# awslabs/crowd-coachable-recommendations

Hardware: AMD Instinct MI355X
Metric: queries/sec, exhaustive inner-product top-100 retrieval (NQ-shaped 2,681,468 x 768 bf16 corpus) (higher is better)
Workload: dtype bf16

## Files before the change

crowd-coachable-recommendations_amd/ccrec_amd/_lib.py:

```python
import ctypes
import os

_HERE = os.path.dirname(os.path.abspath(__file__))
LIB_PATH = os.path.join(os.path.dirname(_HERE), "lib", "libccr_hip.so")

CCR_OK = 0
CCR_ERR_INVALID, CCR_ERR_HIP, CCR_ERR_WORKSPACE, CCR_ERR_BLOCK_ID = -1, -2, -3, -4
DTYPE_F32, DTYPE_F16, DTYPE_BF16 = 0, 1, 2
SEARCH_DEFAULT, SEARCH_FORCE_DENSE, SEARCH_FORCE_FUSED, SEARCH_ASYNC = 0, 1, 2, 4
SCORES_CANONICAL, SCORES_MFMA = 0, 1

EXPORTS = [
    "ccr_last_error", "ccr_version", "ccr_pack_bf16", "ccr_pack_bf16_ex", "ccr_meanpool_pack_bf16", "ccr_meanpool_pack_bf16_ex", "ccr_index_create",
    "ccr_index_create_with_norms", "ccr_index_destroy",
    "ccr_index_rows", "ccr_index_dim", "ccr_search_workspace_bytes", "ccr_search", "ccr_search_last_stats",
    "ccr_merge_topk", "ccr_merge_topk_strided", "ccr_apply_block", "ccr_inbatch_ce_workspace_bytes", "ccr_inbatch_ce_fwd", "ccr_inbatch_ce_bwd", "ccr_inbatch_ce_bwd_dev", "ccr_rank_metrics",
    "ccr_search_finish", "ccr_scores", "ccr_search_blocked_workspace_bytes", "ccr_search_blocked",
    "ccr_search_sparse_prior_workspace_bytes", "ccr_search_sparse_prior", "ccr_colsum_bf16", "ccr_meanpool_bwd", "ccr_bm25_index_create", "ccr_bm25_index_destroy", "ccr_bm25_search_workspace_bytes",
    "ccr_bm25_search", "ccr_pack_bf16_padded", "ccr_shard_message_bytes", "ccr_search_shard", "ccr_shard_message_fill", "ccr_merge_shard_messages",
    "ccr_attention_bf16", "ccr_add_layernorm", "ccr_meanpool_pack_bf16_packed", "ccr_embed_layernorm", "ccr_gelu_bf16",
    "ccr_attention_half", "ccr_add_layernorm_half", "ccr_embed_layernorm_half", "ccr_gelu_half", "ccr_merge_short_lists",
    "ccr_bm25_search_workspace_bytes_k", "ccr_bm25_search_last_stats", "ccr_bm25_index_set_idf", "ccr_inbatch_pack3_bf16", "ccr_inbatch_ce_fwd_f32",
    "ccr_search_stream_wait_main_pass",
]

SHARD_HEADER_BYTES = 32
SHARD_MAGIC = 0x4D524343


class ShardHeader(ctypes.Structure):
    _fields_ = [("magic", ctypes.c_uint32), ("n_flagged", ctypes.c_uint32), ("k_valid", ctypes.c_uint32),
                ("n_covered", ctypes.c_uint32), ("row_offset", ctypes.c_int64), ("n_rows", ctypes.c_int64)]


class SearchStats(ctypes.Structure):
    _fields_ = [("path", ctypes.c_int32), ("n_fallback", ctypes.c_int32), ("sample_tiles", ctypes.c_int32),
                ("ranges", ctypes.c_int32), ("cap", ctypes.c_int32), ("sublists", ctypes.c_int32),
                ("n_candidates", ctypes.c_int64), ("ms_sample", ctypes.c_float), ("ms_threshold", ctypes.c_float),
                ("ms_main", ctypes.c_float), ("ms_select", ctypes.c_float), ("ms_fallback", ctypes.c_float),
                ("ms_total", ctypes.c_float), ("n_retried", ctypes.c_int32), ("n_dense", ctypes.c_int32),
                ("main_launches", ctypes.c_int32), ("opt_rank", ctypes.c_int32), ("main_tile_queries", ctypes.c_int32),
                ("reserved0", ctypes.c_int32)]


class CcrError(RuntimeError):
    pass


_lib = None


def load():
    global _lib
    if _lib is not None:
        return _lib
    if not os.path.isfile(LIB_PATH):
        raise CcrError(f"{LIB_PATH} not built: run `python -c 'import __graft_entry__ as g; g.build()'` "
                       f"(or make -C crowd-coachable-recommendations_amd/csrc)")
    lib = ctypes.CDLL(LIB_PATH)
    vp, i32, i64, f32, sz = ctypes.c_void_p, ctypes.c_int, ctypes.c_int64, ctypes.c_float, ctypes.c_size_t
    lib.ccr_last_error.restype = ctypes.c_char_p
    lib.ccr_last_error.argtypes = []
    lib.ccr_version.restype = i32
    lib.ccr_pack_bf16.argtypes = [vp, vp, vp, i64, i32, i32, vp]
    lib.ccr_pack_bf16_ex.argtypes = [vp, vp, vp, vp, i64, i32, i32, vp]
    lib.ccr_index_create_with_norms.argtypes = [vp, i64, i32, i64, vp, vp, ctypes.POINTER(vp)]
    lib.ccr_meanpool_pack_bf16.argtypes = [vp, i32, vp, vp, vp, i32, i32, i32, i32, vp]
    lib.ccr_meanpool_pack_bf16_ex.argtypes = [vp, i32, vp, vp, vp, vp, vp, i32, i32, i32, i32, vp]
    lib.ccr_index_create.argtypes = [vp, i64, i32, i64, vp, ctypes.POINTER(vp)]
    lib.ccr_index_destroy.argtypes = [vp]
    lib.ccr_index_rows.argtypes = [vp]
    lib.ccr_index_rows.restype = i64
    lib.ccr_index_dim.argtypes = [vp]
    lib.ccr_search_workspace_bytes.argtypes = [vp, i32, i32]
    lib.ccr_search_workspace_bytes.restype = sz
    lib.ccr_search.argtypes = [vp, vp, i32, i32, vp, vp, vp, sz, i32, vp]
    lib.ccr_search_last_stats.argtypes = [vp, ctypes.POINTER(SearchStats)]
    lib.ccr_merge_topk.argtypes = [vp, vp, i32, i32, i32, vp, vp, vp]
    lib.ccr_merge_topk_strided.argtypes = [vp, vp, i64, i64, i32, i32, i32, vp, vp, vp]
    lib.ccr_apply_block.argtypes = [vp, vp, i32, i32, vp, vp, i64, vp, vp, i32, vp]
    lib.ccr_inbatch_ce_workspace_bytes.argtypes = [i32, i32]
    lib.ccr_inbatch_ce_workspace_bytes.restype = sz
    lib.ccr_inbatch_ce_fwd.argtypes = [vp, vp, vp, i32, i32, f32, vp, vp, vp, sz, vp]
    lib.ccr_inbatch_ce_bwd.argtypes = [vp, vp, vp, vp, i32, i32, f32, f32, vp, vp, vp, vp, sz, vp]
    lib.ccr_inbatch_ce_bwd_dev.argtypes = [vp, vp, vp, vp, i32, i32, f32, vp, vp, vp, vp, vp, sz, vp]
    lib.ccr_inbatch_pack3_bf16.argtypes = [vp, vp, vp, i32, i32, vp, vp]
    lib.ccr_inbatch_ce_fwd_f32.argtypes = [vp, vp, vp, i32, i32, f32, vp, vp, vp, vp, sz, vp]
    lib.ccr_rank_metrics.argtypes = [vp, i32, i32, vp, vp, vp, i32, vp, vp, vp]
    lib.ccr_search_finish.argtypes = [vp]
    lib.ccr_search_stream_wait_main_pass.argtypes = [vp, vp]
    lib.ccr_scores.argtypes = [vp, vp, i32, i32, vp, vp]
    lib.ccr_search_blocked_workspace_bytes.argtypes = [vp, i32, i32, vp]
    lib.ccr_search_blocked_workspace_bytes.restype = sz
    lib.ccr_search_blocked.argtypes = [vp, vp, i32, i32, vp, vp, vp, vp, vp, sz, i32, vp]
    lib.ccr_search_sparse_prior_workspace_bytes.argtypes = [vp, i32, i32, vp]
    lib.ccr_search_sparse_prior_workspace_bytes.restype = sz
    lib.ccr_search_sparse_prior.argtypes = [vp, vp, i32, i32, vp, vp, vp, vp, vp, vp, sz, i32, vp]
    lib.ccr_colsum_bf16.argtypes = [vp, i64, i32, vp, vp]
    lib.ccr_meanpool_bwd.argtypes = [vp, vp, vp, i32, i32, i32, i32, vp]
    lib.ccr_bm25_index_create.argtypes = [vp, vp, vp, vp, i64, i64, ctypes.c_double, ctypes.POINTER(vp)]
    lib.ccr_bm25_index_destroy.argtypes = [vp]
    lib.ccr_bm25_search_workspace_bytes.argtypes = [vp, i32, i32]
    lib.ccr_bm25_search_workspace_bytes.restype = sz
    lib.ccr_bm25_search_workspace_bytes_k.argtypes = [vp, i32, i32, i32]
    lib.ccr_bm25_search_workspace_bytes_k.restype = sz
    lib.ccr_bm25_search_last_stats.argtypes = [vp, vp]
    lib.ccr_bm25_index_set_idf.argtypes = [vp, vp, vp, vp]
    lib.ccr_bm25_search.argtypes = [vp, vp, vp, vp, i32, i32, vp, vp, vp, sz, vp]
    lib.ccr_pack_bf16_padded.argtypes = [vp, i64, i32, vp, i32, vp, vp, i32, vp]
    lib.ccr_attention_bf16.argtypes = [vp, vp, vp, vp, i32, i32, i32, i32, ctypes.c_float, vp]
    lib.ccr_add_layernorm.argtypes = [vp, vp, vp, vp, ctypes.c_float, vp, vp, i64, i32, vp]
    lib.ccr_embed_layernorm.argtypes = [vp, i64, vp, i64, vp, i64, vp, vp, vp, vp, vp, ctypes.c_float, vp, vp, i64, i32, vp]
    lib.ccr_gelu_bf16.argtypes = [vp, vp, i64, vp]
    lib.ccr_attention_half.argtypes = [vp, vp, vp, vp, i32, i32, i32, i32, ctypes.c_float, i32, vp]
    lib.ccr_add_layernorm_half.argtypes = [vp, vp, vp, vp, ctypes.c_float, vp, vp, i64, i32, i32, vp]
    lib.ccr_embed_layernorm_half.argtypes = [vp, i64, vp, i64, vp, i64, vp, vp, vp, vp, vp, ctypes.c_float, vp, vp, i64, i32, i32, vp]
    lib.ccr_gelu_half.argtypes = [vp, vp, i64, i32, vp]
    lib.ccr_meanpool_pack_bf16_packed.argtypes = [vp, i32, vp, vp, vp, vp, vp, vp, i32, i32, i32, vp]
    lib.ccr_shard_message_bytes.argtypes = [i32, i32]
    lib.ccr_shard_message_bytes.restype = sz
    lib.ccr_search_shard.argtypes = [vp, vp, i32, i32, vp, vp, sz, i32, vp]
    lib.ccr_shard_message_fill.argtypes = [vp, i32, i32, i32, vp, vp, i64, i64, vp]
    lib.ccr_merge_shard_messages.argtypes = [vp, i64, i32, i32, i32, vp, vp, vp]
    lib.ccr_merge_short_lists.argtypes = [vp, i64, i32, i32, i32, i32, vp, vp, vp, vp, vp]
    for name in EXPORTS:
        fn = getattr(lib, name)
        if fn.restype is ctypes.c_int and name not in ("ccr_version", "ccr_index_dim"):
            fn.restype = i32
    _lib = lib
    return lib


def check(rc, what=""):
    if rc != CCR_OK:
        msg = load().ccr_last_error().decode("utf-8", "replace")
        if rc == CCR_ERR_BLOCK_ID:
            raise AssertionError("block id not found")
        raise CcrError(f"{what} failed ({rc}): {msg}")
```

crowd-coachable-recommendations_amd/csrc/ccr_api.hip:

```cpp
#include <stdarg.h>
#include <stdlib.h>
#include <string.h>

#include <math.h>

#include <algorithm>
#include <mutex>
#include <vector>

#include "ccr_index.h"
#include "ccr_narrow.h"
#include "ccr_topk_device.h"

namespace ccr {

static thread_local char g_err[512] = "";
void set_error(const char *fmt, ...) {
    va_list ap;
    va_start(ap, fmt);
    vsnprintf(g_err, sizeof(g_err), fmt, ap);
    va_end(ap);
}

static int env_int(const char *name, int dflt) {
    const char *e = getenv(name);
    return e ? atoi(e) : dflt;
}

Knobs read_knobs() {
    Knobs kn;
    kn.qgroups = env_int("CCR_QGROUPS", 0);
    kn.progressive = env_int("CCR_PROGRESSIVE", 1);
    kn.max_phases = env_int("CCR_PHASES", 3);
    kn.mfma16 = env_int("CCR_MFMA16", -1);
    kn.sample_div = env_int("CCR_SAMPLE_DIV", 0);
    kn.max_lists = env_int("CCR_MAX_LISTS", 0);
    kn.ranges = env_int("CCR_RANGES", 0);
    kn.optimistic = env_int("CCR_OPTIMISTIC", -1);
    kn.opt_rank = env_int("CCR_OPT_RANK", 0);
    kn.narrow = env_int("CCR_NARROW", -1);
    kn.wide = env_int("CCR_WIDE", -1);
    kn.narrow_grid = env_int("CCR_NARROW_GRID", 0);
    kn.narrow_groups = env_int("CCR_NARROW_GROUPS", NARROW_MAX_GROUPS);
    return kn;
}

static int pick_qgroups(int qblocks, int dim, const Knobs &kn, int tile_q = TILE_Q) {
    {
        const int v = kn.qgroups;
        if ((v == 1 || v == 2 || v == 4 || v == 8) && qblocks % v == 0) return v;
    }
    const size_t block_bytes = (size_t)tile_q * dim * 2;
    int best = 1;
    for (int gq = 1; gq <= NUM_XCD; gq *= 2) {
        if (qblocks % gq) continue;
        best = gq;
        if ((size_t)(qblocks / gq) * block_bytes <= (size_t)3 << 20) break;
    }
    return best;
}

static inline int64_t round_up(int64_t v, int64_t m) { return (v + m - 1) / m * m; }

static int best_sample_ranges(int64_t n_vt, int qblocks, int qgroups, int grid) {
    const int nrc = NUM_XCD / qgroups, qb_per = qblocks / qgroups, per_x = std::max(1, grid / NUM_XCD);
    int best_r = NUM_XCD;
    double best = 1e300;
    const int64_t r_max = round_up(std::min<int64_t>(n_vt, 1024), NUM_XCD);
    std::vector<double> load((size_t)per_x);
    for (int64_t R = NUM_XCD; R <= r_max; R += NUM_XCD) {
        double worst = 0.0;
        for (int rc = 0; rc < nrc; ++rc) {
            std::fill(load.begin(), load.end(), 0.0);
            const int64_t items = R / nrc * qb_per;
            for (int64_t item = 0; item < items; ++item) {
                const int64_t r = rc + nrc * (item / qb_per);
                const int64_t ntile = (n_vt - r + R - 1) / R;
                if (ntile > 0) load[(size_t)(item % per_x)] += (double)ntile + 0.15;
            }
            worst = std::max(worst, *std::max_element(load.begin(), load.end()));
        }
        if (worst < best - 1e-9) {
            best = worst;
            best_r = (int)R;
        }
    }
    return best_r;
}

constexpr size_t DENSE_SCRATCH_TARGET = (size_t)1 << 30;

struct MainPassChoice {
    int64_t sample, ranges;
    int item_a, item_b;
    int opt_rank;
};

static int optimistic_rank(int k, int64_t sample, int64_t tiles, const Knobs &kn) {
    if (kn.opt_rank > 0) return kn.opt_rank;
    const double need = (double)k * (double)sample / (double)tiles;
    int r = 40;
    for (; r < 1 << 20; ++r) {
        const double a = 1.0 / (9.0 * r), t = 1.0 - a - 5.2 * sqrt(a);
        if (t > 0.0 && (double)r * t * t * t >= need) break;
    }
    return r;
}

static MainPassChoice choose_main_pass(const Plan &p, int k, int64_t sample_a, int64_t sample_b, int64_t sample_c, const Knobs &kn,
                                       bool single_only = false) {
    const int nrc = NUM_XCD / p.main_qgroups, qb_per = p.main_qblocks / p.main_qgroups, per_x = p.grid / NUM_XCD;
    const double tile_cost = p.tile_q == WIDE_Q ? 1.37 : 1.0;
    int64_t max_lists = p.rescore_cap > 512 ? 2048 : 1024;
    if ((max_lists / p.sublists) * p.main_qblocks < p.grid) max_lists = 2048;
    if (kn.max_lists >= 64 && kn.max_lists < max_lists) max_lists = kn.max_lists;
    const int64_t r_hi = std::min<int64_t>(max_lists / p.sublists, round_up(std::max<int64_t>(1, p.tiles / 8), NUM_XCD));
    const int64_t target = std::min<int64_t>(r_hi, round_up(std::max<int64_t>(NUM_XCD, (int64_t)p.grid * 6 / p.main_qblocks), NUM_XCD));
    const bool prog_on = kn.progressive != 0 && !single_only;
    const int max_phases = kn.max_phases;
    const double qscale = (double)p.nq_pad / 3584.0;
    const double select_per_range = 0.1 * qscale, hit_w = 0.014 * qscale, phase_w = 3.0;
    auto sample_cost = [&](int64_t smp) -> double {
        return (double)((smp * p.qblocks + p.grid - 1) / p.grid) + 0.015 * (double)smp * std::max(1.0, qscale);
    };

    MainPassChoice best_choice = {sample_a, target, 0, 0, 0};
    double best = 1e300;
    for (int pass = 0; pass < 3; ++pass) {
        const int64_t smp = pass == 0 ? sample_a : (pass == 1 ? sample_b : sample_c);
        if ((pass >= 1 && smp == sample_a) || (pass == 2 && smp == sample_b)) continue;
        const double fs = (double)smp / (double)p.tiles;
        const double smp_cost = sample_cost(smp);
        auto survivors = [&](double fa, double fb) -> double {
            if (fa <= 0.0) return (double)k / fs;
            if (fb <= 0.0) return (double)k * (fa / fs + (1.0 - fa) / fa);
            return (double)k * (fa / fs + fb / fa + (1.0 - fa - fb) / (fa + fb));
        };
        const int64_t r_lo = std::max<int64_t>(NUM_XCD, target / 2 / NUM_XCD * NUM_XCD);
        for (int64_t R = r_lo; R <= std::min(r_hi, target * 2); R += NUM_XCD) {
            if (kn.ranges > 0 && R != std::min<int64_t>(r_hi, std::max<int64_t>(r_lo, round_up(kn.ranges, NUM_XCD)))) continue;
            const int64_t items = R / nrc * qb_per;
            const double item_cost = ((double)((p.tiles + R - 1) / R) + 0.15) * tile_cost;
            auto rounds = [&](int64_t n) { return (double)((n + per_x - 1) / per_x); };
            const double common = smp_cost + select_per_range * (double)R + 1e-3 * std::abs((double)(R - target));
            const double single = rounds(items) * item_cost + hit_w * survivors(0.0, 0.0) + common;
            if (single < best && kn.optimistic != 1) {
                best = single;
                best_choice = {smp, R, 0, 0, 0};
            }
            if (kn.optimistic != 0 && smp * GROUPS_PER_TILE >= 4 * 40) {
                const int rank = optimistic_rank(k, smp, p.tiles, kn);
                if ((int64_t)rank * 4 <= smp * GROUPS_PER_TILE) {
                    const double pass = std::max((double)rank / fs, (double)k);
                    const double opt = rounds(items) * item_cost + hit_w * pass + common - (kn.optimistic == 1 ? 1e9 : 0.0);
                    if (opt < best) {
                        best = opt;
                        best_choice = {smp, R, 0, 0, rank};
                    }
                }
            }
            if (!(prog_on && items > per_x && (double)p.tiles / (double)R >= 8.0)) continue;
            const double fa = (double)per_x / (double)items;
            const double two = (1.0 + rounds(items - per_x)) * item_cost + phase_w + hit_w * survivors(fa, 0.0) + common;
            if (two < best) {
                best = two;
                best_choice = {smp, R, per_x, 0, 0};
            }
            if (max_phases < 3) continue;
            for (int m = 1; m <= 3; ++m) {
                const int64_t ib = (int64_t)per_x * (1 + m);
                if (ib >= items) break;
                const double fb = (double)m * per_x / (double)items;
                const double three = (1.0 + m + rounds(items - ib)) * item_cost + 2.0 * phase_w + hit_w * survivors(fa, fb) + common;
                if (three < best) {
                    best = three;
                    best_choice = {smp, R, per_x, (int)ib, 0};
                }
            }
        }
    }
    return best_choice;
}

static CandLayout one_segment(int cap) {
    CandLayout L;
    memset(&L, 0, sizeof(L));
    L.nseg = 1;
    L.seg_end[0] = L.seg_end[1] = L.seg_end[2] = INT32_MAX;
    L.cap[0] = L.cap[1] = L.cap[2] = cap;
    return L;
}

static Plan make_plan_for(int64_t n_rows, int dim, int n_q, int k, int flags, int num_cu, const Knobs &kn, int mfma16) {
    Plan p;
    memset(&p, 0, sizeof(p));
    p.nq_pad = (int)round_up(n_q, TILE_Q);
    p.qblocks = p.nq_pad / TILE_Q;
    p.tile_q = TILE_Q;
    p.main_qblocks = p.qblocks;
    p.main_qgroups = 1;
    p.tiles = (n_rows + TILE_DOCS - 1) / TILE_DOCS;
    p.full_tiles = n_rows / TILE_DOCS;
    p.grid = std::max(NUM_XCD, num_cu / NUM_XCD * NUM_XCD);
    {
        p.mfma16 = mfma16;
        p.sublists = p.mfma16 ? 8 : 4;
    }
    p.rescore_cap = std::min(8192, std::max(256, 2 * pow2_ceil(k)));

    const int64_t min_sample = (2 * (int64_t)k + GROUPS_PER_TILE - 1) / GROUPS_PER_TILE;
    int64_t sample_div = 32;
    bool sample_div_forced = false;
    {
        if (kn.sample_div >= 4 && kn.sample_div <= 256) {
            sample_div = kn.sample_div;
            sample_div_forced = true;
        }
    }
    auto sample_for = [&](int64_t div) { return std::max<int64_t>({(p.tiles + div - 1) / div, min_sample, 4}); };
    int64_t sample = sample_for(sample_div);
    bool fused = (dim % 8 == 0) && dim >= 8 && (sample * 4 <= p.full_tiles) && k <= MAX_K;
    if ((flags & CCR_SEARCH_FORCE_FUSED) && (dim % 8 == 0) && p.full_tiles >= 1) {
        if (!fused) sample = std::min<int64_t>(std::max<int64_t>(sample, 1), p.full_tiles);
        fused = sample * GROUPS_PER_TILE >= k;
    }
    if (flags & CCR_SEARCH_FORCE_DENSE) fused = false;
    p.fused = fused ? 1 : 0;

    if (p.fused) {
        p.qgroups = pick_qgroups(p.qblocks, dim, kn);
        const bool pinned = sample_div_forced || (flags & CCR_SEARCH_FORCE_FUSED);
        const int64_t sample_alt = pinned ? sample : sample_for(2 * sample_div);
        int64_t sample_big = pinned ? sample : sample_for(sample_div / 2);
        if (sample_big * 4 > p.full_tiles) sample_big = sample;
        int nqt = n_q <= 16 ? 1 : (n_q <= 32 ? 2 : 4);
        int ngroups = n_q <= NARROW_MAX_Q ? 1 : 2;
        if (n_q > NARROW_MAX_Q && n_q <= 96 && kn.narrow_groups >= 2 && dim % TILE_K == 0 && narrow_lds_bytes(6, dim) <= (size_t)160 * 1024)
            nqt = 6, ngroups = 1;
        const bool narrow = kn.narrow != 0 && n_q <= NARROW_MAX_Q * std::min(std::max(kn.narrow_groups, 1), NARROW_MAX_GROUPS) && dim % TILE_K == 0 &&
                            narrow_lds_bytes(nqt, dim) <= (size_t)160 * 1024 && (ngroups == 1 || num_cu >= 16);
        p.narrow = narrow ? nqt : 0;
        p.narrow_groups = narrow ? ngroups : 1;
        p.tile_q = TILE_Q;
        p.main_qblocks = p.qblocks;
        if (!narrow && p.mfma16 && dim % 32 == 0 && kn.wide != 0) {
            const int wb = (n_q + WIDE_Q - 1) / WIDE_Q;
            const double per_xcd = (double)(wb / pick_qgroups(wb, dim, kn, WIDE_Q)) * WIDE_Q * dim * 2.0;
            const double per_flop = per_xcd <= 3.2 * 1048576.0 ? 0.95 : (per_xcd <= 5.5 * 1048576.0 ? 0.97 : 1.04);
            if (kn.wide == 1 || (double)wb * WIDE_Q * per_flop < (double)p.qblocks * TILE_Q) {
                p.tile_q = WIDE_Q;
                p.main_qblocks = wb;
                p.nq_pad = (int)round_up(std::max<int64_t>(n_q, (int64_t)wb * WIDE_Q), TILE_Q);
                p.qblocks = p.nq_pad / TILE_Q;
                p.qgroups = pick_qgroups(p.qblocks, dim, kn);
            }
        }
        p.main_qgroups = pick_qgroups(p.main_qblocks, dim, kn, p.tile_q);
        const MainPassChoice choice = choose_main_pass(p, k, sample, sample_alt, sample_big, kn, narrow);
        sample = choice.sample;
        const int64_t R = choice.ranges;
        p.sample_tiles = (int)sample;
        p.sample_stride = std::max<int64_t>(1, p.full_tiles / sample);
        p.sample_ranges = best_sample_ranges(sample, p.qblocks, p.qgroups, p.grid);
        p.ranges = (int)R;
        p.item_a = choice.item_a;
        p.item_b = choice.item_b;
        p.opt_rank = choice.opt_rank;
        const int nrc_p = NUM_XCD / p.main_qgroups, qb_per_p = p.main_qblocks / p.main_qgroups;
        const int64_t RA = p.item_a ? std::min<int64_t>(R, (int64_t)nrc_p * ((p.item_a + qb_per_p - 1) / qb_per_p)) : 0;
        const int64_t RB = p.item_b ? std::min<int64_t>(R, (int64_t)nrc_p * ((p.item_b + qb_per_p - 1) / qb_per_p)) : 0;
        const double ratio = (double)p.tiles / (double)sample;
        const double expect = (double)k * ratio * 1.3 + 64.0;
        const double fs = 1.0 / ratio, nlists = (double)R * p.sublists;
        const double xk = 1.25 * ((double)k + 4.75 * sqrt((double)k) + 8.0) / (double)k;
        const int64_t tile_rows = TILE_DOCS / p.sublists;
        const double xr = p.opt_rank ? 1.25 * ((double)p.opt_rank + 4.75 * sqrt((double)p.opt_rank) + 8.0) / (double)p.opt_rank : 0.0;
        auto cap_for = [&](double g) -> int {
            const double mean = p.opt_rank ? xr * std::max((double)p.opt_rank / fs, (double)k) / nlists : xk * (double)k / (g * nlists);
            const int64_t c = (int64_t)(mean + 6.0 * sqrt(mean)) + 16 + tile_rows;
            return (int)round_up(std::min<int64_t>(std::max<int64_t>(c, 16), 8192), 4);
        };
        const double fa = p.item_a ? (double)(p.item_a / qb_per_p) * nrc_p / (double)R : 0.0;
        const double fb = p.item_b ? std::max(0.0, (double)(p.item_b / qb_per_p) * nrc_p / (double)R - fa) : 0.0;
        const double upd_compact = std::min(32768.0, std::max(4096.0, 8.0 * pow2_ceil(k)));
        auto seen = [&](double g, double found) { return found > upd_compact ? g * upd_compact / found : g; };
        const double found_a = (double)k * fa / fs;
        CandLayout &L = p.cand;
        memset(&L, 0, sizeof(L));
        const int seg_end_v[3] = {RA ? (int)RA : (int)R, RB > RA ? (int)RB : (int)R, (int)R};
        int64_t recs = 0;
        L.nseg = 0;
        int prev_end = 0;
        for (int g = 0; g < 3; ++g) {
            L.seg_end[g] = INT32_MAX;
            L.cap[g] = 16;
            L.base[g] = recs;
        }
        for (int g = 0; g < 3; ++g) {
            if (seg_end_v[g] <= prev_end) continue;
            const int sg = L.nseg++;
            double frac_seen = fs;
            if (sg == 1) frac_seen = fa >= 2.0 * fs ? seen(fa, found_a) : fs;
            if (sg == 2) frac_seen = fa >= 2.0 * fs ? seen(fa + fb, found_a + (double)k * fb / fa) : fs;
            L.seg_end[sg] = seg_end_v[g];
            L.cap[sg] = cap_for(std::min(1.0, std::max(frac_seen, fs)));
            L.base[sg] = recs;
            recs += (int64_t)(seg_end_v[g] - prev_end) * p.nq_pad * p.sublists * L.cap[sg];
            recs = round_up(recs, 32);
            prev_end = seg_end_v[g];
        }
        L.seg_end[L.nseg - 1] = INT32_MAX;
        p.cap = L.cap[0];
        const double want_opt = std::max(xr * std::max((double)p.opt_rank / fs, (double)k) + 512.0, k > 256 ? 18.0 * k : 0.0);
        p.select_compact = select_compact_entries(dim, p.ranges * p.sublists, p.rescore_cap,
                                                  (int64_t)((p.opt_rank ? want_opt : (RA ? 16.0 * k + 512.0 : expect)) * 1.25));
        p.first_nsub = p.ranges * p.sublists;
        p.first_sp = p.sublists;
        p.first_lay = p.cand;
        if (p.narrow) {
            const double pass = p.opt_rank ? xr * std::max((double)p.opt_rank / fs, (double)k) : expect;
            int64_t capn = std::max<int64_t>(recs / ((int64_t)NARROW_SUBLISTS * std::max(1, n_q)), (int64_t)(8.0 * pass) + 4096);
            capn = std::min<int64_t>(capn, (int64_t)1 << 22) / 4 * 4;
            recs = std::max<int64_t>(recs, capn * NARROW_SUBLISTS * n_q);
            p.first_lay = one_segment((int)capn);
            p.first_nsub = NARROW_SUBLISTS;
            p.first_sp = NARROW_SUBLISTS;
        }
        p.cand_recs = recs;
        p.dense_rows_per_chunk = FALLBACK_ROWS;
    } else {
        int64_t rows = (int64_t)(DENSE_SCRATCH_TARGET / ((size_t)n_rows * 4));
        rows = std::min<int64_t>(std::max<int64_t>(rows, 1), n_q);
        if (rows >= 64) rows = rows / 64 * 64;
        p.dense_rows_per_chunk = rows;
    }
    const SearchWs w = search_ws(p, n_rows, dim, n_q, k, nullptr);
    p.off_qnorm = (size_t)w.qnorm, p.off_thr = (size_t)w.thr, p.off_gmax = (size_t)w.gmax, p.off_cnt = (size_t)w.cnt, p.off_cand = (size_t)w.cand;
    p.off_flag = (size_t)w.flag_count, p.off_dense = (size_t)w.dense, p.off_retry = (size_t)w.Q2, p.off_top = (size_t)w.top, p.off_safe = (size_t)w.thr_safe;
    p.total = w.total;
    return p;
}

SearchWs search_ws(const Plan &p, int64_t n_rows, int dim, int n_q, int k, char *base) {
    SearchWs w;
    memset(&w, 0, sizeof(w));
    Bump b = {0};
    auto at = [&](size_t off) { return (char *)((uintptr_t)base + off); };
    auto take = [&](size_t bytes) { return at(b.take(bytes)); };
    if (!p.fused) {
        w.flag_count = (uint32_t *)take(64 + (size_t)n_q * 4);
        w.flag_list = w.flag_count + 16;
        w.dense_bytes = (size_t)p.dense_rows_per_chunk * (n_rows + 3) * 4;
        w.dense = (float *)take(w.dense_bytes);
        w.total = b.off;
        return w;
    }
    const size_t nq_pad = p.nq_pad;
    w.qnorm = (float *)take(nq_pad * 4);
    w.thr = (float *)take(nq_pad * 8);
    w.cq = w.thr + nq_pad;
    w.gmax = (float *)take((size_t)p.sample_tiles * GROUPS_PER_TILE * nq_pad * 4);
    w.cnt = (uint32_t *)take((size_t)p.ranges * nq_pad * p.sublists * 4);
    w.cand = (uint2 *)take((size_t)p.cand_recs * 8);
    w.flag_count = (uint32_t *)take(64 + (size_t)n_q * 4);
    w.stat_cand = (unsigned long long *)(w.flag_count + 2);
    w.flag_list = w.flag_count + 16;
    w.cand_bytes = (char *)w.flag_count - (char *)w.cand;
    w.top = (uint32_t *)take(p.item_b ? (nq_pad + (size_t)n_q * k) * 4 : 0);
    w.thr_safe = (float *)take(p.opt_rank ? nq_pad * 8 : 0);
    w.cq_safe = w.thr_safe + nq_pad;
    w.dense_bytes = (size_t)p.dense_rows_per_chunk * n_rows * 4;
    w.dense = (float *)take(w.dense_bytes);
    w.retry_bytes = nq_pad * dim * 2 + nq_pad * 8 + (size_t)n_q * 16 + 64 + 64 + (size_t)n_q * 4 + 256 * 10;
    Bump r = {b.take(w.retry_bytes)};
    w.Q2 = (uint16_t *)at(r.take(nq_pad * dim * 2));
    w.thr2 = (float *)at(r.take(nq_pad * 4));
    w.cq2 = (float *)at(r.take(nq_pad * 4));
    w.retry_list = (uint32_t *)at(r.take((size_t)n_q * 4));
    w.dense_list = (uint32_t *)at(r.take((size_t)n_q * 4));
    w.counts = (uint32_t *)at(r.take(64));
    w.flag2 = (uint32_t *)at(r.take(64 + (size_t)n_q * 4));
    w.list_b = (uint32_t *)at(r.take((size_t)n_q * 4));
    w.list_c = (uint32_t *)at(r.take((size_t)n_q * 4));
    w.total = b.off;
    return w;
}

Plan make_plan(int64_t n_rows, int dim, int n_q, int k, int flags, int num_cu, const Knobs &kn) {
    if (kn.mfma16 >= 0) return make_plan_for(n_rows, dim, n_q, k, flags, num_cu, kn, kn.mfma16 ? 1 : 0);
    if (k <= 512) return make_plan_for(n_rows, dim, n_q, k, flags, num_cu, kn, 1);
    const Plan p32 = make_plan_for(n_rows, dim, n_q, k, flags, num_cu, kn, 0);
    if (p32.fused && p32.ranges * 8 <= 2048) return make_plan_for(n_rows, dim, n_q, k, flags, num_cu, kn, 1);
    return p32;
}

}

using namespace ccr;

namespace {
constexpr int SLAB_SLOTS = 1024, SLAB_SLOT_BYTES = 256, MAX_DEVICES = 64;
struct Slab {
    char *base = nullptr;
    char *host = nullptr;
    std::vector<int> free_slots;
};
constexpr int SLAB_HOST_BYTES = 64;
std::mutex g_slab_mutex;
Slab g_slabs[MAX_DEVICES];

int slab_take(int device, uint32_t **out, volatile uint32_t **host_out) {
    std::lock_guard<std::mutex> lock(g_slab_mutex);
    CCR_REQUIRE(device >= 0 && device < MAX_DEVICES, "device ordinal %d out of range", device);
    Slab &sl = g_slabs[device];
    if (!sl.base) {
        CCR_HIP_CHECK(hipMalloc((void **)&sl.base, (size_t)SLAB_SLOTS * SLAB_SLOT_BYTES));
        if (hipHostMalloc((void **)&sl.host, (size_t)SLAB_SLOTS * SLAB_HOST_BYTES, hipHostMallocDefault) != hipSuccess) {
            (void)hipFree(sl.base);
            sl.base = nullptr;
            set_error("ccr_index_create: hipHostMalloc of the pinned flag lines failed");
            return CCR_ERR_HIP;
        }
        for (int i = SLAB_SLOTS - 1; i >= 0; --i) sl.free_slots.push_back(i);
    }
    if (sl.free_slots.empty()) {
        set_error("ccr_index_create: more than %d live indices on device %d", SLAB_SLOTS, device);
        return CCR_ERR_INVALID;
    }
    *out = reinterpret_cast<uint32_t *>(sl.base + (size_t)sl.free_slots.back() * SLAB_SLOT_BYTES);
    *host_out = reinterpret_cast<volatile uint32_t *>(sl.host + (size_t)sl.free_slots.back() * SLAB_HOST_BYTES);
    sl.free_slots.pop_back();
    return CCR_OK;
}

void slab_give(int device, uint32_t *p) {
    if (!p || device < 0 || device >= MAX_DEVICES) return;
    std::lock_guard<std::mutex> lock(g_slab_mutex);
    Slab &sl = g_slabs[device];
    sl.free_slots.push_back((int)((reinterpret_cast<char *>(p) - sl.base) / SLAB_SLOT_BYTES));
}
}

extern "C" const char *ccr_last_error(void) { return g_err; }
extern "C" int ccr_version(void) { return 100; }

extern "C" int ccr_index_destroy(ccr_index *ix);

namespace {
struct CachedBlock {
    void *p;
    size_t bytes;
};
std::vector<CachedBlock> g_blocks[MAX_DEVICES];
constexpr size_t BLOCK_CACHE_ENTRIES = 8;

int block_take(int device, size_t bytes, void **out, size_t *got) {
    CCR_REQUIRE(device >= 0 && device < MAX_DEVICES, "device ordinal %d out of range", device);
    bytes = (bytes + 4095) / 4096 * 4096;
    {
        std::lock_guard<std::mutex> lock(g_slab_mutex);
        auto &v = g_blocks[device];
        for (size_t i = 0; i < v.size(); ++i)
            if (v[i].bytes >= bytes && v[i].bytes <= 2 * bytes) {
                *out = v[i].p;
                *got = v[i].bytes;
                v.erase(v.begin() + i);
                return CCR_OK;
            }
    }
    CCR_HIP_CHECK(hipMalloc(out, bytes));
    *got = bytes;
    return CCR_OK;
}

void block_give(int device, void *p, size_t bytes) {
    if (!p) return;
    void *drop = nullptr;
    if (device >= 0 && device < MAX_DEVICES && bytes <= ((size_t)64 << 20)) {
        std::lock_guard<std::mutex> lock(g_slab_mutex);
        auto &v = g_blocks[device];
        v.push_back({p, bytes});
        if (v.size() > BLOCK_CACHE_ENTRIES) {
            drop = v.front().p;
            v.erase(v.begin());
        }
    } else {
        drop = p;
    }
    if (drop) (void)hipFree(drop);
}
}

static int index_create_impl(const uint16_t *D_bf16, int64_t n_rows, int dim, int64_t global_row_offset, const float *row_bounds,
                             void *stream, ccr_index **out) {
    CCR_REQUIRE(D_bf16 && out, "ccr_index_create: null pointer");
    CCR_REQUIRE(n_rows >= 1 && n_rows < ((int64_t)1 << 32), "ccr_index_create: n_rows=%lld out of range [1, 2^32)",
                (long long)n_rows);
    CCR_REQUIRE(dim >= 8 && dim % 8 == 0 && dim <= 4096, "ccr_index_create: dim=%d must be a multiple of 8 in [8, 4096]", dim);
    CCR_REQUIRE((uintptr_t)D_bf16 % 16 == 0, "ccr_index_create: corpus pointer must be 16-byte aligned");
    hipStream_t s = (hipStream_t)stream;
    ccr_index *ix = new ccr_index();
    memset(ix, 0, sizeof(*ix));
    ix->D = D_bf16;
    ix->n_rows = n_rows;
    ix->dim = dim;
    ix->offset = ix->id_out = global_row_offset;
    ix->knobs = read_knobs();
    auto build = [&]() -> int {
        CCR_HIP_CHECK(hipGetDevice(&ix->device));
        CCR_HIP_CHECK(hipDeviceGetAttribute(&ix->num_cu, hipDeviceAttributeMultiprocessorCount, ix->device));
        int rc = slab_take(ix->device, &ix->dmax_bits, &ix->host_flags);
        if (rc != CCR_OK) return rc;
        const int64_t tiles = (n_rows + TILE_DOCS - 1) / TILE_DOCS;
        void *tn = nullptr;
        rc = block_take(ix->device, (size_t)tiles * 4, &tn, &ix->tile_bytes);
        if (rc != CCR_OK) return rc;
        ix->tile_norm = (float *)tn;
        uint32_t *tile_bits = reinterpret_cast<uint32_t *>(ix->tile_norm);
        if (row_bounds) {
            ix->row_norm = row_bounds;
            rc = launch_tile_norms(row_bounds, n_rows, tile_bits, ix->dmax_bits, s);
            if (rc != CCR_OK) return rc;
        } else {
            void *rn = nullptr;
            rc = block_take(ix->device, (size_t)n_rows * 4, &rn, &ix->row_bytes);
            if (rc != CCR_OK) return rc;
            ix->row_norm = ix->row_norm_own = (float *)rn;
            CCR_HIP_CHECK(hipMemsetAsync(ix->dmax_bits, 0, 4, s));
            CCR_HIP_CHECK(hipMemsetAsync(tile_bits, 0, (size_t)tiles * 4, s));
            rc = launch_row_norms_bf16(D_bf16, n_rows, dim, ix->row_norm_own, ix->dmax_bits, tile_bits, s);
            if (rc != CCR_OK) return rc;
            CCR_HIP_CHECK(hipStreamSynchronize(s));
        }
        return CCR_OK;
    };
    const int rc = build();
    if (rc != CCR_OK) {
        ccr_index_destroy(ix);
        return rc;
    }
    *out = ix;
    return CCR_OK;
}

extern "C" int ccr_index_create(const uint16_t *D_bf16, int64_t n_rows, int dim, int64_t global_row_offset, void *stream,
                                ccr_index **out) {
    return index_create_impl(D_bf16, n_rows, dim, global_row_offset, nullptr, stream, out);
}

extern "C" int ccr_index_create_with_norms(const uint16_t *D_bf16, int64_t n_rows, int dim, int64_t global_row_offset,
                                           const float *row_norm_bounds, void *stream, ccr_index **out) {
    CCR_REQUIRE(row_norm_bounds, "ccr_index_create_with_norms: null row_norm_bounds");
    return index_create_impl(D_bf16, n_rows, dim, global_row_offset, row_norm_bounds, stream, out);
}

extern "C" int ccr_index_destroy(ccr_index *ix) {
    if (!ix) return CCR_OK;
    if (ix->pending.active && ix->have_events) (void)hipEventSynchronize(ix->ev[EV_ASYNC_END]);
    ix->pending.active = false;
    slab_give(ix->device, ix->dmax_bits);
    block_give(ix->device, ix->tile_norm, ix->tile_bytes);
    block_give(ix->device, ix->row_norm_own, ix->row_bytes);
    if (ix->have_events)
        for (int i = 0; i < EV_COUNT; ++i)
            if (ix->ev[i]) (void)hipEventDestroy(ix->ev[i]);
    delete ix;
    return CCR_OK;
}

extern "C" int64_t ccr_index_rows(const ccr_index *ix) { return ix ? ix->n_rows : -1; }
extern "C" int ccr_index_dim(const ccr_index *ix) { return ix ? ix->dim : -1; }

extern "C" size_t ccr_search_workspace_bytes(const ccr_index *ix, int n_q, int k) {
    if (!ix || n_q <= 0 || k <= 0) return 0;
    Plan a = make_plan(ix->n_rows, ix->dim, n_q, k, CCR_SEARCH_DEFAULT, ix->num_cu, ix->knobs);
    Plan b = make_plan(ix->n_rows, ix->dim, n_q, k, CCR_SEARCH_FORCE_DENSE, ix->num_cu, ix->knobs);
    Plan c = make_plan(ix->n_rows, ix->dim, n_q, k, CCR_SEARCH_FORCE_FUSED, ix->num_cu, ix->knobs);
    return std::max({a.total, b.total, c.total}) + 256;
}

extern "C" int ccr_search_stream_wait_main_pass(const ccr_index *ix, void *stream) {
    CCR_REQUIRE(ix, "ccr_search_stream_wait_main_pass: null index");
    if (!ix->main_pass_recorded) return CCR_OK;
    CCR_HIP_CHECK(hipStreamWaitEvent((hipStream_t)stream, ix->ev[EV_MAIN_END], 0));
    return CCR_OK;
}

extern "C" int ccr_search_last_stats(const ccr_index *ix, ccr_search_stats *stats) {
    CCR_REQUIRE(ix && stats, "ccr_search_last_stats: null pointer");
    CCR_REQUIRE(!ix->pending.active, "ccr_search_last_stats: an asynchronous search is pending (call ccr_search_finish first)");
    *stats = ix->stats;
    return CCR_OK;
}

static int dense_for_list(const ccr_index *ix, const uint16_t *Q, const uint32_t *d_qlist, int n, int k, float *scratch, int64_t rows_per_chunk,
                          float *out_scores, int64_t *out_ids, hipStream_t s) {
    for (int lo = 0; lo < n; lo += (int)rows_per_chunk) {
        const int m = std::min<int64_t>(rows_per_chunk, n - lo);
        int rc = launch_dense_scores(ix->D, ix->n_rows, ix->dim, Q, d_qlist ? d_qlist + lo : nullptr, lo, m, nullptr, scratch, s);
        if (rc != CCR_OK) return rc;
        rc = launch_dense_select(scratch, ix->n_rows, k, d_qlist ? d_qlist + lo : nullptr, lo, m, nullptr, ix->id_out, out_scores, out_ids, s);
        if (rc != CCR_OK) return rc;
    }
    return CCR_OK;
}

static bool margin_path_ok(const ccr_index *ix, int k) { return ix->dim % 8 == 0 && k <= MAX_K; }
static int64_t tiles_of(const ccr_index *ix) { return (ix->n_rows + TILE_DOCS - 1) / TILE_DOCS; }

static GemmArgs gemm_args(const ccr_index *ix, const uint16_t *Q, int n_q, int nq_pad) {
    GemmArgs g;
    memset(&g, 0, sizeof(g));
    g.D = ix->D;
    g.n_rows = ix->n_rows;
    g.dim = ix->dim;
    g.Q = Q;
    g.n_q = n_q;
    g.nq_pad = nq_pad;
    g.qblocks = nq_pad / TILE_Q;
    g.item_end = INT32_MAX;
    return g;
}

static GemmArgs filter_args(const ccr_index *ix, const Plan &p, const SearchWs &w, const uint16_t *Q, int n_q, int nq_pad, int qblocks,
                            int qgroups, const float *thr, const float *cq, const CandLayout &lay) {
    GemmArgs g = gemm_args(ix, Q, n_q, nq_pad);
    g.qblocks = qblocks;
    g.qgroups = qgroups;
    g.n_vt = p.tiles;
    g.tile_stride = 1;
    g.ranges = p.ranges;
    g.thr = thr;
    g.cq = cq;
    g.tile_norm = ix->tile_norm;
    g.cnt = w.cnt;
    g.cand = w.cand;
    g.lay = lay;
    return g;
}

static int store_scores(const ccr_index *ix, const uint16_t *Q, int n_q, int ranges, float *out, int64_t pitch, hipStream_t s) {
    GemmArgs g = gemm_args(ix, Q, n_q, (int)round_up(n_q, TILE_Q));
    g.n_vt = tiles_of(ix);
    g.tile_stride = 1;
    g.ranges = ranges;
    g.qgroups = 1;
    g.store = out;
    g.store_pitch = pitch;
    return launch_gemm(g, ix->knobs.mfma16 != 0 ? MAIN_16X16 : MAIN_32X32, EPI_STORE, std::max(NUM_XCD, ix->num_cu / NUM_XCD * NUM_XCD), s);
}

static int margin_for_rows(const ccr_index *ix, const uint16_t *Qc, const float *hint, const uint32_t *out_rows, int n, int k, float *scratch,
                           size_t scratch_bytes, float *out_scores, int64_t *out_ids, uint32_t *flag_count, uint32_t *flag_list, hipStream_t s) {
    const int64_t pitch = round_up(ix->n_rows, 4);
    int64_t chunk = (int64_t)(scratch_bytes / ((size_t)pitch * 4));
    CCR_REQUIRE(chunk >= 1, "margin path: no room for one score row");
    if (chunk > TILE_Q) chunk = chunk / TILE_Q * TILE_Q;
    const int ranges = (int)round_up(std::min<int64_t>(std::max<int64_t>(1, tiles_of(ix) / 4), 1024), NUM_XCD);
    for (int lo = 0; lo < n; lo += (int)chunk) {
        const int m = std::min<int64_t>(chunk, n - lo);
        const uint16_t *Q = Qc + (int64_t)lo * ix->dim;
        int rc = store_scores(ix, Q, m, ranges, scratch, pitch, s);
        if (rc != CCR_OK) return rc;
        rc = launch_margin_select(scratch, pitch, ix->n_rows, k, ix->dim, Q, ix->D, ix->tile_norm, ix->row_norm, ix->dmax_bits,
                                  hint ? hint + lo : nullptr, out_rows ? out_rows + lo : nullptr, lo, m, ix->id_out, out_scores, out_ids, flag_count, flag_list, s);
        if (rc != CCR_OK) return rc;
    }
    return CCR_OK;
}

static int run_main_pass(const ccr_index *ix, const Plan &p, const SearchWs &w, const uint16_t *Q, int n_q, int k, hipStream_t s) {
    GemmArgs gm = filter_args(ix, p, w, Q, n_q, p.nq_pad, p.main_qblocks, p.main_qgroups, w.thr, w.cq, p.cand);
    const int nrc = NUM_XCD / gm.qgroups, qb_per = gm.qblocks / gm.qgroups, items = p.ranges / nrc * qb_per;
    const int bounds[4] = {0, p.item_a, p.item_b, items};
    int done = 0, updates = 0, prev_full = 0, prev_part = 0, prev_blocks = 0;
    for (int ph = 1; ph < 4; ++ph) {
        if (bounds[ph] <= done) continue;
        if (done > 0) {
            const int rl_full = done / qb_per, part = done % qb_per;
            const int full = rl_full * nrc * p.sublists, partial = part ? (rl_full + 1) * nrc * p.sublists : 0;
            const bool more = bounds[ph] < items && ph < 3;
            const int rc = launch_threshold_update(w.cand, w.cnt, full, partial, part, prev_full, prev_part, prev_blocks, qb_per, p.sublists, n_q,
                                                   p.nq_pad, p.cand, k, w.cq, ix->tile_norm, p.item_b ? w.top : nullptr, updates > 0, more, w.thr, s, p.tile_q);
            if (rc != CCR_OK) return rc;
            prev_full = full;
            prev_part = partial;
            prev_blocks = part;
            ++updates;
        }
        gm.item_begin = done;
        gm.item_end = bounds[ph];
        const MainKernel kind = p.tile_q == WIDE_Q ? MAIN_WIDE : p.mfma16 ? MAIN_16X16 : MAIN_32X32;
        const int rc = launch_gemm(gm, kind, EPI_FILTER, p.grid, s);
        if (rc != CCR_OK) return rc;
        done = bounds[ph];
    }
    return CCR_OK;
}

static int run_narrow_pass(const ccr_index *ix, const Plan &p, const SearchWs &w, const uint16_t *Q, int n_q, hipStream_t s) {
    NarrowArgs na;
    memset(&na, 0, sizeof(na));
    na.D = ix->D;
    na.n_rows = ix->n_rows;
    na.dim = ix->dim;
    na.Q = Q;
    na.n_q = n_q;
    na.q_stride = narrow_query_stride(ix->dim);
    na.thr = w.thr;
    na.cq = w.cq;
    na.tile_norm = ix->tile_norm;
    na.cand = w.cand;
    na.cnt = w.cnt;
    na.cap = p.first_lay.cap[0];
    na.groups = p.narrow_groups;
    int ngrid = ix->knobs.narrow_grid > 0 ? ix->knobs.narrow_grid : ix->num_cu;
    const int64_t blocks = (ix->n_rows + 16 * NARROW_WAVES - 1) / (16 * NARROW_WAVES);
    if ((int64_t)ngrid > blocks) ngrid = (int)std::max<int64_t>(1, blocks);
    if (p.narrow_groups == 2) ngrid = std::max(16, ngrid / 16 * 16);
    return launch_narrow_filter(na, p.narrow, ngrid, s);
}

static int read_words(void *host, const void *dev, int n, hipStream_t s) {
    CCR_HIP_CHECK(hipMemcpyAsync(host, dev, (size_t)n * 4, hipMemcpyDeviceToHost, s));
    CCR_HIP_CHECK(hipStreamSynchronize(s));
    return CCR_OK;
}


static int fused_stats(ccr_index *ix, uint32_t nflag, unsigned long long ncand) {
    const Plan &p = ix->plan;
    ccr_search_stats &st = ix->stats;
    float a = 0, b = 0;
    CCR_HIP_CHECK(hipEventElapsedTime(&st.ms_sample, ix->ev[EV_SAMPLE_BEGIN], ix->ev[EV_SAMPLE_END]));
    CCR_HIP_CHECK(hipEventElapsedTime(&a, ix->ev[EV_BEGIN], ix->ev[EV_SAMPLE_BEGIN]));
    CCR_HIP_CHECK(hipEventElapsedTime(&b, ix->ev[EV_SAMPLE_END], ix->ev[EV_MAIN_BEGIN]));
    st.ms_threshold = a + b;
    CCR_HIP_CHECK(hipEventElapsedTime(&st.ms_main, ix->ev[EV_MAIN_BEGIN], ix->ev[EV_MAIN_END]));
    CCR_HIP_CHECK(hipEventElapsedTime(&st.ms_select, ix->ev[EV_MAIN_END], ix->ev[EV_SELECT_END]));
    CCR_HIP_CHECK(hipEventElapsedTime(&st.ms_total, ix->ev[EV_BEGIN], ix->ev[EV_SELECT_END]));
    st.path = 1;
    st.n_fallback = (int32_t)nflag;
    st.sample_tiles = p.sample_tiles;
    st.ranges = p.narrow ? 1 : p.ranges;
    st.cap = p.narrow ? p.first_lay.cap[0] : p.cap;
    st.sublists = p.narrow ? p.first_sp : p.sublists;
    st.main_launches = 1 + (p.item_a ? 1 : 0) + (p.item_b ? 1 : 0);
    st.opt_rank = p.opt_rank;
    st.main_tile_queries = p.narrow ? 0 : p.tile_q;
    st.n_candidates = (int64_t)ncand;
    return CCR_OK;
}

static int recover_thresholds(const ccr_index *ix, const SearchWs &w, int nflag) {
    const auto &pd = ix->pending;
    const int rc = launch_threshold(w.gmax, (int64_t)ix->plan.sample_tiles * GROUPS_PER_TILE, pd.n_q, ix->plan.nq_pad, pd.k, w.qnorm, ix->dmax_bits,
                                    ix->dim, ix->tile_norm, ix->plan.sample_stride, w.thr_safe, w.cq_safe, pd.stream);
    if (rc != CCR_OK) return rc;
    return launch_underfilled_to_retry(w.flag_list, 0, nflag, w.thr_safe, w.thr, pd.stream);
}

static int to_dense(const SearchWs &w, const uint32_t *list, int n, int &n_dense, hipStream_t s) {
    CCR_HIP_CHECK(hipMemcpyAsync(w.dense_list + n_dense, list, (size_t)n * 4, hipMemcpyDeviceToDevice, s));
    n_dense += n;
    return CCR_OK;
}

static int retry_group(ccr_index *ix, const SearchWs &w, const uint32_t *cur, int n_cur, int &n_dense) {
    const Plan &p = ix->plan;
    const auto &pd = ix->pending;
    hipStream_t s = pd.stream;
    const int nsub_all = p.ranges * p.sublists;
    for (int round = 0;; ++round) {
        int rc = launch_gather_queries(pd.Q, ix->dim, cur, n_cur, w.thr, w.cq, w.Q2, w.thr2, w.cq2, s);
        if (rc != CCR_OK) return rc;
        const int pad2 = (int)round_up(n_cur, TILE_Q);
        const int64_t cap2 = std::min<int64_t>(8192, (int64_t)(w.cand_bytes / 8) / ((int64_t)nsub_all * pad2) / 4 * 4);
        if (cap2 < 16) break;
        const CandLayout lay2 = one_segment((int)cap2);
        CCR_HIP_CHECK(hipMemsetAsync(w.cnt, 0, (size_t)nsub_all * pad2 * 4, s));
        CCR_HIP_CHECK(hipMemsetAsync(w.flag2, 0, 64, s));
        const GemmArgs g = filter_args(ix, p, w, w.Q2, n_cur, pad2, pad2 / TILE_Q, pick_qgroups(pad2 / TILE_Q, ix->dim, ix->knobs), w.thr2, w.cq2, lay2);
        rc = launch_gemm(g, p.mfma16 ? MAIN_16X16 : MAIN_32X32, EPI_FILTER, p.grid, s);
        if (rc != CCR_OK) return rc;
        rc = launch_select_rescore(w.cand, w.cnt, nsub_all, p.sublists, n_cur, pad2, lay2, pd.k, p.rescore_cap, p.select_compact, ix->n_rows,
                                   w.thr2, w.cq2, ix->tile_norm, ix->row_norm, ix->dmax_bits, w.Q2, ix->D, ix->dim, ix->id_out, pd.out_scores, pd.out_ids,
                                   w.flag2, w.flag2 + 16, nullptr, cur, s);
        if (rc != CCR_OK) return rc;
        ix->stats.n_retried += n_cur;
        uint32_t again = 0;
        rc = read_words(&again, w.flag2, 1, s);
        if (rc != CCR_OK || again == 0) return rc;
        uint32_t *next = (cur == w.list_b) ? w.list_c : w.list_b;
        rc = launch_partition_flags(w.flag2 + 16, 0, (int)again, next, w.dense_list + n_dense, w.counts, s);
        if (rc != CCR_OK) return rc;
        uint32_t hc[2] = {0, 0};
        rc = read_words(hc, w.counts, 2, s);
        if (rc != CCR_OK) return rc;
        n_dense += (int)hc[1];
        const uint32_t *list = cur;
        const int n = n_cur;
        cur = next;
        n_cur = (int)hc[0];
        if (n_cur == 0 || round == 2 || n_cur >= n) break;
        rc = launch_threshold_update(w.cand, w.cnt, nsub_all, 0, 0, 0, 0, 0, 1, p.sublists, n, pad2, lay2, pd.k, w.cq2, ix->tile_norm, nullptr,
                                     false, false, w.thr2, s);
        if (rc != CCR_OK) return rc;
        rc = launch_scatter_thresholds(list, n, w.thr2, w.thr, s);
        if (rc != CCR_OK) return rc;
    }
    return n_cur > 0 ? to_dense(w, cur, n_cur, n_dense, s) : CCR_OK;
}

static int retry_flagged(ccr_index *ix, const SearchWs &w, int n_retry, int &n_dense) {
    const Plan &p = ix->plan;
    const auto &pd = ix->pending;
    const int nsub_all = p.ranges * p.sublists;
    if (nsub_all > 2048) return to_dense(w, w.retry_list, n_retry, n_dense, pd.stream);
    int rc = launch_threshold_update(w.cand, w.cnt, p.first_nsub, 0, 0, 0, 0, 0, 1, p.first_sp, pd.n_q, p.nq_pad, p.first_lay, pd.k, w.cq,
                                     ix->tile_norm, nullptr, false, false, w.thr, pd.stream);
    if (rc != CCR_OK) return rc;
    const int64_t want_cap = std::min<int64_t>(8192, 4 * (int64_t)p.cap);
    int64_t group = (int64_t)(w.cand_bytes / 8) / ((int64_t)nsub_all * want_cap) / TILE_Q * TILE_Q;
    group = std::max<int64_t>(TILE_Q, std::min<int64_t>(group, round_up(n_retry, TILE_Q)));
    for (int g0 = 0; g0 < n_retry && rc == CCR_OK; g0 += (int)group)
        rc = retry_group(ix, w, w.retry_list + g0, std::min<int>((int)group, n_retry - g0), n_dense);
    return rc;
}

static int complete_dense(ccr_index *ix, const SearchWs &w, int n_dense) {
    const Plan &p = ix->plan;
    const auto &pd = ix->pending;
    hipStream_t s = pd.stream;
    const bool margin_in_cand = w.cand_bytes > w.dense_bytes;
    const int64_t fit = (int64_t)(w.cand_bytes / ((size_t)ix->n_rows * 4)) / 64 * 64;
    const bool fp64_in_cand = n_dense > p.dense_rows_per_chunk && fit >= 64;
    const int64_t chunk = fp64_in_cand ? std::min<int64_t>(fit, 256) : p.dense_rows_per_chunk;
    float *fp64_scr = fp64_in_cand ? (float *)w.cand : w.dense;
    if (!margin_path_ok(ix, pd.k))
        return dense_for_list(ix, pd.Q, w.dense_list, n_dense, pd.k, fp64_scr, chunk, pd.out_scores, pd.out_ids, s);
    CCR_HIP_CHECK(hipMemsetAsync(w.flag2, 0, 64, s));
    for (int lo = 0; lo < n_dense; lo += p.nq_pad) {
        const int m = std::min(p.nq_pad, n_dense - lo);
        int rc = launch_gather_queries(pd.Q, ix->dim, w.dense_list + lo, m, w.thr, w.cq, w.Q2, w.thr2, w.cq2, s);
        if (rc != CCR_OK) return rc;
        rc = margin_for_rows(ix, w.Q2, w.thr2, w.dense_list + lo, m, pd.k, margin_in_cand ? (float *)w.cand : w.dense,
                             margin_in_cand ? w.cand_bytes : w.dense_bytes, pd.out_scores, pd.out_ids, w.flag2, w.flag2 + 16, s);
        if (rc != CCR_OK) return rc;
    }
    uint32_t left = 0;
    const int rc = read_words(&left, w.flag2, 1, s);
    if (rc != CCR_OK || left == 0) return rc;
    return dense_for_list(ix, pd.Q, w.flag2 + 16, (int)left, pd.k, fp64_scr, chunk, pd.out_scores, pd.out_ids, s);
}

static int search_complete(ccr_index *ix) {
    auto &pd = ix->pending;
    hipStream_t s = pd.stream;
    const bool was_async = pd.active;
    pd.active = false;
    const SearchWs w = search_ws(ix->plan, ix->n_rows, ix->dim, pd.n_q, pd.k, pd.ws);
    struct { uint32_t nflag, pad; unsigned long long ncand; } host;
    int rc = CCR_OK;
    if (was_async) {
        CCR_HIP_CHECK(hipEventSynchronize(ix->ev[EV_ASYNC_END]));
        host.nflag = ix->host_flags[0];
        host.ncand = *reinterpret_cast<volatile unsigned long long *>(ix->host_flags + 2);
    } else {
        rc = read_words(&host, w.flag_count, 4, s);
        if (rc != CCR_OK) return rc;
    }
    rc = fused_stats(ix, host.nflag, host.ncand);
    if (rc != CCR_OK || host.nflag == 0) return rc;
    rc = ix->plan.opt_rank ? recover_thresholds(ix, w, (int)host.nflag) : CCR_OK;
    if (rc != CCR_OK) return rc;
    rc = launch_partition_flags(w.flag_list, 0, (int)host.nflag, w.retry_list, w.dense_list, w.counts, s);
    if (rc != CCR_OK) return rc;
    uint32_t hc[2] = {0, 0};
    rc = read_words(hc, w.counts, 2, s);
    if (rc != CCR_OK) return rc;
    int n_dense = (int)hc[1];
    if (hc[0] > 0) rc = retry_flagged(ix, w, (int)hc[0], n_dense);
    if (rc == CCR_OK && n_dense > 0) rc = complete_dense(ix, w, n_dense);
    if (rc != CCR_OK) return rc;
    ix->stats.n_dense += n_dense;
    CCR_HIP_CHECK(hipEventRecord(ix->ev[EV_DONE], s));
    CCR_HIP_CHECK(hipStreamSynchronize(s));
    CCR_HIP_CHECK(hipEventElapsedTime(&ix->stats.ms_fallback, ix->ev[EV_SELECT_END], ix->ev[EV_DONE]));
    ix->stats.ms_total += ix->stats.ms_fallback;
    return CCR_OK;
}

extern "C" int ccr_search_finish(ccr_index *ix) {
    CCR_REQUIRE(ix, "ccr_search_finish: null index");
    return ix->pending.active ? search_complete(ix) : CCR_OK;
}

static int search_dense(ccr_index *ix, const SearchWs &w, const uint16_t *Q, int n_q, int k, float *out_scores, int64_t *out_ids,
                        int flags, hipStream_t s) {
    const bool async = (flags & CCR_SEARCH_ASYNC) != 0;
    const int64_t chunk = ix->plan.dense_rows_per_chunk;
    int rc;
    if (!async && !(flags & CCR_SEARCH_FORCE_DENSE) && margin_path_ok(ix, k)) {
        CCR_HIP_CHECK(hipMemsetAsync(w.flag_count, 0, 64, s));
        rc = margin_for_rows(ix, Q, nullptr, nullptr, n_q, k, w.dense, w.dense_bytes, out_scores, out_ids, w.flag_count, w.flag_list, s);
        if (rc != CCR_OK) return rc;
        uint32_t nf = 0;
        rc = read_words(&nf, w.flag_count, 1, s);
        if (rc != CCR_OK) return rc;
        ix->stats.n_fallback = ix->stats.n_dense = (int32_t)nf;
        if (nf > 0) rc = dense_for_list(ix, Q, w.flag_list, (int)nf, k, w.dense, chunk, out_scores, out_ids, s);
    } else {
        rc = dense_for_list(ix, Q, nullptr, n_q, k, w.dense, chunk, out_scores, out_ids, s);
    }
    if (rc != CCR_OK) return rc;
    CCR_HIP_CHECK(hipEventRecord(ix->ev[EV_DONE], s));
    if (async) return CCR_OK;
    CCR_HIP_CHECK(hipStreamSynchronize(s));
    CCR_HIP_CHECK(hipEventElapsedTime(&ix->stats.ms_total, ix->ev[EV_BEGIN], ix->ev[EV_DONE]));
    ix->stats.ms_fallback = ix->stats.ms_total;
    return CCR_OK;
}

static int search_impl(ccr_index *ix, const uint16_t *Q_bf16, int n_q, int k, float *out_scores, int64_t *out_ids, int64_t id_out,
                       uint32_t *flagged_out, void *workspace, size_t ws_bytes, int flags, void *stream) {
    CCR_REQUIRE(ix && Q_bf16 && out_scores && out_ids, "ccr_search: null pointer");
    CCR_REQUIRE(n_q >= 0, "ccr_search: n_q=%d", n_q);
    CCR_REQUIRE(k >= 1 && k <= MAX_K && (int64_t)k <= ix->n_rows, "ccr_search: k=%d must be in [1, min(n_rows=%lld, %d)]", k,
                (long long)ix->n_rows, MAX_K);
    CCR_REQUIRE((uintptr_t)Q_bf16 % 16 == 0, "ccr_search: query pointer must be 16-byte aligned");
    CCR_REQUIRE(!ix->pending.active, "ccr_search: an asynchronous search is pending on this index (call ccr_search_finish first)");
    memset(&ix->stats, 0, sizeof(ix->stats));
    ix->main_pass_recorded = false;
    if (n_q == 0) return CCR_OK;
    hipStream_t s = (hipStream_t)stream;
    ix->id_out = id_out;
    const bool async = (flags & CCR_SEARCH_ASYNC) != 0;
    const int plan_flags = flags & ~CCR_SEARCH_ASYNC;
    if (!(ix->plan_nq == n_q && ix->plan_k == k && ix->plan_flags == plan_flags)) {
        ix->plan = make_plan(ix->n_rows, ix->dim, n_q, k, plan_flags, ix->num_cu, ix->knobs);
        ix->plan_nq = n_q;
        ix->plan_k = k;
        ix->plan_flags = plan_flags;
    }
    const Plan p = ix->plan;
    if (!workspace || ws_bytes < p.total || (uintptr_t)workspace % 256 != 0) {
        set_error("ccr_search: workspace %zu bytes (256-byte aligned) required, got %zu at %p", p.total, ws_bytes, workspace);
        return CCR_ERR_WORKSPACE;
    }
    const SearchWs w = search_ws(p, ix->n_rows, ix->dim, n_q, k, (char *)workspace);

    if (!ix->have_events) {
        for (int i = 0; i < EV_COUNT; ++i) CCR_HIP_CHECK(hipEventCreate(&ix->ev[i]));
        ix->have_events = true;
    }
    CCR_HIP_CHECK(hipEventRecord(ix->ev[EV_BEGIN], s));
    if (!p.fused) return search_dense(ix, w, Q_bf16, n_q, k, out_scores, out_ids, flags, s);

    CCR_HIP_CHECK(hipMemsetAsync(w.flag_count, 0, 64, s));
    if ((int64_t)p.ranges > p.tiles) CCR_HIP_CHECK(hipMemsetAsync(w.cnt, 0, (size_t)p.ranges * p.nq_pad * p.sublists * 4, s));
    int rc = launch_row_norms_bf16(Q_bf16, n_q, ix->dim, w.qnorm, nullptr, nullptr, s);
    if (rc != CCR_OK) return rc;

    GemmArgs gs = gemm_args(ix, Q_bf16, n_q, p.nq_pad);
    gs.qgroups = p.qgroups;
    gs.n_vt = p.sample_tiles;
    gs.tile_stride = p.sample_stride;
    gs.ranges = p.sample_ranges;
    gs.gmax = w.gmax;
    CCR_HIP_CHECK(hipEventRecord(ix->ev[EV_SAMPLE_BEGIN], s));
    rc = launch_gemm(gs, MAIN_32X32, EPI_GMAX, p.grid, s);
    if (rc != CCR_OK) return rc;
    CCR_HIP_CHECK(hipEventRecord(ix->ev[EV_SAMPLE_END], s));
    rc = launch_threshold(w.gmax, (int64_t)p.sample_tiles * GROUPS_PER_TILE, n_q, p.nq_pad, p.opt_rank ? p.opt_rank : k, w.qnorm, ix->dmax_bits,
                          ix->dim, ix->tile_norm, p.sample_stride, w.thr, w.cq, s, p.narrow ? w.cnt : nullptr, p.narrow ? NARROW_SUBLISTS : 0);
    if (rc != CCR_OK) return rc;

    CCR_HIP_CHECK(hipEventRecord(ix->ev[EV_MAIN_BEGIN], s));
    rc = p.narrow ? run_narrow_pass(ix, p, w, Q_bf16, n_q, s) : run_main_pass(ix, p, w, Q_bf16, n_q, k, s);
    if (rc != CCR_OK) return rc;
    CCR_HIP_CHECK(hipEventRecord(ix->ev[EV_MAIN_END], s));
    ix->main_pass_recorded = true;
    rc = launch_select_rescore(w.cand, w.cnt, p.first_nsub, p.first_sp, n_q, p.nq_pad, p.first_lay, k, p.rescore_cap, p.select_compact, ix->n_rows, w.thr,
                               w.cq, ix->tile_norm, ix->row_norm, ix->dmax_bits, Q_bf16, ix->D, ix->dim, ix->id_out, out_scores, out_ids,
                               w.flag_count, w.flag_list, w.stat_cand, nullptr, s);
    if (rc != CCR_OK) return rc;
    CCR_HIP_CHECK(hipEventRecord(ix->ev[EV_SELECT_END], s));

    ix->pending = {false, Q_bf16, n_q, k, out_scores, out_ids, (char *)workspace, s};
    if (!async) return search_complete(ix);
    if (flagged_out) CCR_HIP_CHECK(hipMemcpyAsync(flagged_out, w.flag_count, 4, hipMemcpyDeviceToDevice, s));
    CCR_HIP_CHECK(hipMemcpyAsync((void *)ix->host_flags, w.flag_count, 16, hipMemcpyDeviceToHost, s));
    CCR_HIP_CHECK(hipEventRecord(ix->ev[EV_ASYNC_END], s));
    ix->pending.active = true;
    return CCR_OK;
}

extern "C" int ccr_search(ccr_index *ix, const uint16_t *Q_bf16, int n_q, int k, float *out_scores, int64_t *out_ids,
                          void *workspace, size_t ws_bytes, int flags, void *stream) {
    CCR_REQUIRE(ix, "ccr_search: null index");
    return search_impl(ix, Q_bf16, n_q, k, out_scores, out_ids, ix->offset, nullptr, workspace, ws_bytes, flags, stream);
}

static inline size_t shard_rows_at(int n_q, int k) { return (sizeof(ccr_shard_header) + (size_t)n_q * k * 4 + 15) / 16 * 16; }

extern "C" size_t ccr_shard_message_bytes(int n_q, int k) {
    if (n_q < 0 || k < 1) return 0;
    return (shard_rows_at(n_q, k) + (size_t)n_q * k * 4 + 15) / 16 * 16;
}

extern "C" int ccr_search_shard(ccr_index *ix, const uint16_t *Q_bf16, int n_q, int k, void *message, void *workspace, size_t ws_bytes,
                                int flags, void *stream) {
    CCR_REQUIRE(ix && message, "ccr_search_shard: null pointer");
    CCR_REQUIRE((uintptr_t)message % 16 == 0, "ccr_search_shard: message must be 16-byte aligned");
    CCR_REQUIRE(n_q >= 0 && k >= 1, "ccr_search_shard: bad shape n_q=%d k=%d", n_q, k);
    hipStream_t s = (hipStream_t)stream;
    ccr_shard_header h;
    memset(&h, 0, sizeof(h));
    h.magic = CCR_SHARD_MAGIC;
    h.k_valid = (uint32_t)k;
    h.n_covered = 0u;
    h.row_offset = ix->offset;
    h.n_rows = ix->n_rows;
    int rc = launch_shard_header(h, message, s);
    if (rc != CCR_OK) return rc;
    if (n_q == 0) return CCR_OK;
    char *m = (char *)message;
    uint32_t *flagged = reinterpret_cast<uint32_t *>(m + offsetof(ccr_shard_header, n_flagged));
    return search_impl(ix, Q_bf16, n_q, k, reinterpret_cast<float *>(m + sizeof(ccr_shard_header)),
                       reinterpret_cast<int64_t *>(m + shard_rows_at(n_q, k)), ID_LOCAL_U32, flagged, workspace, ws_bytes, flags, stream);
}

extern "C" int ccr_scores(const ccr_index *ix, const uint16_t *Q_bf16, int n_q, int mode, float *out, void *stream) {
    CCR_REQUIRE(ix && Q_bf16 && out && n_q > 0, "ccr_scores: bad argument");
    CCR_REQUIRE((uintptr_t)Q_bf16 % 16 == 0, "ccr_scores: query pointer must be 16-byte aligned");
    if (mode == CCR_SCORES_CANONICAL)
        return launch_dense_scores(ix->D, ix->n_rows, ix->dim, Q_bf16, nullptr, 0, n_q, nullptr, out, (hipStream_t)stream);
    CCR_REQUIRE(mode == CCR_SCORES_MFMA, "ccr_scores: unknown mode %d", mode);
    CCR_REQUIRE(ix->dim % 8 == 0, "ccr_scores: CCR_SCORES_MFMA needs dim %% 8 == 0 (dim=%d)", ix->dim);
    return store_scores(ix, Q_bf16, n_q, (int)round_up(std::min<int64_t>(64, tiles_of(ix)), NUM_XCD), out, 0, (hipStream_t)stream);
}
```

crowd-coachable-recommendations_amd/csrc/ccr_common.h:

```cpp
#pragma once
#include <hip/hip_runtime.h>
#include <stdint.h>
#include <stdio.h>

#include "ccr_retrieval.h"

namespace ccr {

void set_error(const char *fmt, ...);

#define CCR_HIP_CHECK(expr)                                                                   \
    do {                                                                                      \
        hipError_t _e = (expr);                                                               \
        if (_e != hipSuccess) {                                                               \
            ccr::set_error("%s failed: %s (%s:%d)", #expr, hipGetErrorString(_e), __FILE__, __LINE__); \
            return CCR_ERR_HIP;                                                               \
        }                                                                                     \
    } while (0)

#define CCR_REQUIRE(cond, ...)            \
    do {                                  \
        if (!(cond)) {                    \
            ccr::set_error(__VA_ARGS__);  \
            return CCR_ERR_INVALID;       \
        }                                 \
    } while (0)

#define CCR_LAUNCH_CHECK()                                                              \
    do {                                                                                \
        hipError_t _e = hipGetLastError();                                              \
        if (_e != hipSuccess) {                                                         \
            ccr::set_error("kernel launch failed: %s (%s:%d)", hipGetErrorString(_e), __FILE__, __LINE__); \
            return CCR_ERR_HIP;                                                         \
        }                                                                               \
    } while (0)

constexpr int TILE_DOCS = 256;
constexpr int TILE_Q = 256;
constexpr int WIDE_Q = 384;
constexpr int TILE_K = 32;
constexpr int GEMM_THREADS = 512;
constexpr int GROUPS_PER_TILE = 16;
constexpr int MAX_K = 4096;
constexpr uint32_t FLAG_DENSE = 0x80000000u;
constexpr int NUM_XCD = 8;

struct CandLayout {
    int nseg;
    int seg_end[3];
    int cap[3];
    long long base[3];
};
__host__ __device__ __forceinline__ void cand_segment(const CandLayout &L, int r, int &cap, int &r0, long long &base) {
    const int g = (r >= L.seg_end[0] ? 1 : 0) + (r >= L.seg_end[1] ? 1 : 0);
    r0 = g ? L.seg_end[g - 1] : 0;
    cap = L.cap[g];
    base = L.base[g];
}
__host__ __device__ __forceinline__ long long cand_sublist(const CandLayout &L, int r, int q, int s, int nq_pad, int sp, int &cap) {
    const int g = (r >= L.seg_end[0] ? 1 : 0) + (r >= L.seg_end[1] ? 1 : 0);
    const int r0 = g ? L.seg_end[g - 1] : 0;
    cap = L.cap[g];
    return L.base[g] + (((long long)(r - r0) * nq_pad + q) * sp) * (long long)cap + s;
}

struct Plan {
    int fused;
    int nq_pad;
    int qblocks;
    int tile_q;
    int main_qblocks;
    int main_qgroups;
    int64_t tiles;
    int64_t full_tiles;
    int sample_tiles;
    int64_t sample_stride;
    int sample_ranges;
    int ranges;
    int item_a;
    int item_b;
    int opt_rank;
    int qgroups;
    int cap;
    CandLayout cand;
    int grid;
    int rescore_cap;
    int select_compact;
    int mfma16;
    int sublists;
    int narrow;
    int narrow_groups;
    int first_nsub;
    int first_sp;
    CandLayout first_lay;
    int64_t cand_recs;
    size_t off_qnorm, off_thr, off_gmax, off_cnt, off_cand, off_flag, off_dense, off_retry, off_top, off_safe, total;
    int64_t dense_rows_per_chunk;
};

enum { EPI_FILTER = 0, EPI_GMAX = 1, EPI_STORE = 2 };

struct GemmArgs {
    const uint16_t *D;
    int64_t n_rows;
    int dim;
    const uint16_t *Q;
    int n_q;
    int nq_pad;
    int qblocks;
    int64_t n_vt;
    int64_t tile_stride;
    int ranges;
    int qgroups;
    int item_begin, item_end;
    const float *thr;
    const float *cq;
    const float *tile_norm;
    uint2 *cand;
    uint32_t *cnt;
    CandLayout lay;
    float *gmax;
    float *store;
    int64_t store_pitch;
};


__device__ __forceinline__ float bf16_bits_to_f32(uint16_t h) { return __uint_as_float(((uint32_t)h) << 16); }

__device__ __forceinline__ uint32_t f32_orderable(float f) {
    uint32_t u = __float_as_uint(f);
    return (u & 0x80000000u) ? ~u : (u | 0x80000000u);
}
__device__ __forceinline__ float orderable_to_f32(uint32_t u) {
    return __uint_as_float((u & 0x80000000u) ? (u & 0x7fffffffu) : ~u);
}

constexpr int64_t ID_LOCAL_U32 = INT64_MIN;
__device__ __forceinline__ void store_id(int64_t *out_ids, int64_t pos, int64_t id_offset, uint32_t row) {
    if (id_offset == ID_LOCAL_U32)
        reinterpret_cast<uint32_t *>(out_ids)[pos] = row;
    else
        out_ids[pos] = id_offset + (int64_t)row;
}

__host__ __device__ __forceinline__ float mfma_gamma(int dim) { return (float)dim * 1.1920929e-7f * 1.02f; }

}
```

crowd-coachable-recommendations_amd/csrc/ccr_fused.hip:

```cpp
#include <stdlib.h>

#include <mutex>
#include <set>
#include <type_traits>
#include <utility>

#include "ccr_gemm_common.h"
#include "ccr_index.h"
#include "ccr_topk_device.h"

namespace ccr {

__device__ __attribute__((aligned(16))) uint32_t g_zero_chunk[4];

__device__ __forceinline__ float load_uniform_f32(const float *p) {
    float v;
    asm volatile("s_load_dword %0, %1, 0x0\n\ts_waitcnt lgkmcnt(0)" : "=s"(v) : "s"(p) : "memory");
    return v;
}

template <int N>
__device__ __forceinline__ void wait_vm() {
    asm volatile("s_waitcnt vmcnt(%0)" ::"n"(N) : "memory");
}

typedef float f32x4v __attribute__((ext_vector_type(4)));

__device__ __forceinline__ float max4_asm(const f32x4v &c) {
    float m;
    asm("v_max3_f32 %0, %1, %2, %3\n\tv_max_f32 %0, %0, %4" : "=&v"(m) : "v"(c[0]), "v"(c[1]), "v"(c[2]), "v"(c[3]));
    return m;
}
__device__ __forceinline__ float max3_asm(float a, float b, float c) {
    float m;
    asm("v_max3_f32 %0, %1, %2, %3" : "=v"(m) : "v"(a), "v"(b), "v"(c));
    return m;
}

struct ItemWalk {
    int jx, step, qg, rc, nrc, qb_per, end;
    __device__ __forceinline__ explicit ItemWalk(const GemmArgs &a) {
        const int xcd = blockIdx.x & (NUM_XCD - 1);
        jx = blockIdx.x >> 3;
        step = gridDim.x >> 3;
        qg = xcd % a.qgroups;
        rc = xcd / a.qgroups;
        nrc = NUM_XCD / a.qgroups;
        qb_per = a.qblocks / a.qgroups;
        const int count_x = (a.ranges / nrc) * qb_per;
        end = a.item_end < count_x ? a.item_end : count_x;
    }
    __device__ __forceinline__ int first(const GemmArgs &a) const { return a.item_begin + jx; }
    __device__ __forceinline__ int64_t item(const GemmArgs &a, int i, int &r, int &qb) const {
        const int rl = i / qb_per;
        const int b = qg * qb_per + i % qb_per;
        const int ri = rc + nrc * rl;
        const int64_t ntile = (a.n_vt - ri + a.ranges - 1) / a.ranges;
        r = ri;
        qb = b;
        return ntile;
    }
};


struct Mfma32 {
    typedef f32x16 Acc;
    static constexpr int TILE = 32, REGS = 16, DT = 4, QT = 2, SUBLISTS = 4;
    struct Frags { bf16x8 a[2][4], b[2][2]; };

    static __device__ __forceinline__ int src_swizzle(int row) { return (row >> 2) & 3; }

    int a_base, b_base, cofs[2];
    __device__ __forceinline__ Mfma32(int lane, int wd, int wq) {
        const int swz = (lane >> 2) & 3;
#pragma unroll
        for (int ks = 0; ks < 2; ++ks) cofs[ks] = (((2 * ks + (lane >> 5)) ^ swz) << 4);
        a_base = (wd * 128 + (lane & 31)) * 64;
        b_base = SUB_Q_REGION + (wq * 64 + (lane & 31)) * 64;
    }
    __device__ __forceinline__ void read(const char *buf, Frags &f) const {
#pragma unroll
        for (int ks = 0; ks < 2; ++ks) {
#pragma unroll
            for (int dt = 0; dt < 4; ++dt) f.a[ks][dt] = *reinterpret_cast<const bf16x8 *>(buf + a_base + dt * 2048 + cofs[ks]);
#pragma unroll
            for (int qt = 0; qt < 2; ++qt) f.b[ks][qt] = *reinterpret_cast<const bf16x8 *>(buf + b_base + qt * 2048 + cofs[ks]);
        }
    }
    static __device__ __forceinline__ void mma(Acc (&acc)[4][2], const Frags &f, bool first) {
        if (first) {
            const f32x16 z = {0.f, 0.f, 0.f, 0.f, 0.f, 0.f, 0.f, 0.f, 0.f, 0.f, 0.f, 0.f, 0.f, 0.f, 0.f, 0.f};
#pragma unroll
            for (int dt = 0; dt < 4; ++dt)
#pragma unroll
                for (int qt = 0; qt < 2; ++qt) acc[dt][qt] = __builtin_amdgcn_mfma_f32_32x32x16_bf16(f.a[0][dt], f.b[0][qt], z, 0, 0, 0);
        } else {
#pragma unroll
            for (int dt = 0; dt < 4; ++dt)
#pragma unroll
                for (int qt = 0; qt < 2; ++qt) acc[dt][qt] = __builtin_amdgcn_mfma_f32_32x32x16_bf16(f.a[0][dt], f.b[0][qt], acc[dt][qt], 0, 0, 0);
        }
#pragma unroll
        for (int dt = 0; dt < 4; ++dt)
#pragma unroll
            for (int qt = 0; qt < 2; ++qt) acc[dt][qt] = __builtin_amdgcn_mfma_f32_32x32x16_bf16(f.a[1][dt], f.b[1][qt], acc[dt][qt], 0, 0, 0);
    }

    static __device__ __forceinline__ void tile_max(const Acc (&acc)[4][2], int qt, float (&sub)[4][4], float (&mdt)[4]) {
#pragma unroll
        for (int dt = 0; dt < 4; ++dt) {
#pragma unroll
            for (int g = 0; g < 4; ++g)
                sub[dt][g] = fmaxf(fmaxf(acc[dt][qt][4 * g], acc[dt][qt][4 * g + 1]), fmaxf(acc[dt][qt][4 * g + 2], acc[dt][qt][4 * g + 3]));
            mdt[dt] = fmaxf(fmaxf(sub[dt][0], sub[dt][1]), fmaxf(sub[dt][2], sub[dt][3]));
        }
    }
    static __device__ __forceinline__ void gmax(const Acc (&acc)[4][2], const GemmArgs &a, int64_t vt, int q0, int wd, int wq, int lane) {
        const int h = lane >> 5;
#pragma unroll
        for (int qt = 0; qt < 2; ++qt) {
            float sub[4][4], mdt[4];
            tile_max(acc, qt, sub, mdt);
            const int ql = wq * 64 + qt * 32 + (lane & 31);
#pragma unroll
            for (int dt = 0; dt < 4; ++dt) a.gmax[(vt * GROUPS_PER_TILE + wd * 8 + dt * 2 + h) * a.nq_pad + q0 + ql] = mdt[dt];
        }
    }
    static __device__ __forceinline__ void filter(const Acc (&acc)[4][2], const float (&thr)[2], const float (&cqv)[2], float nt,
                                                  int64_t row_base, const GemmArgs &a, uint2 *const (&clist)[2], uint32_t (&ncand)[2],
                                                  int cap) {
        const uint32_t row32 = (uint32_t)row_base;
        const int64_t left = a.n_rows - row_base;
        const uint32_t rows_left = left <= 0 ? 0u : (left > 128 ? 128u : (uint32_t)left);
#pragma unroll
        for (int qt = 0; qt < 2; ++qt) {
            float sub[4][4], mdt[4];
            tile_max(acc, qt, sub, mdt);
            const float t = fmaf(-cqv[qt], nt, thr[qt]);
            const float mall = fmaxf(fmaxf(mdt[0], mdt[1]), fmaxf(mdt[2], mdt[3]));
            if (__ballot(mall >= t) == 0ull) continue;
#pragma unroll
            for (int dt = 0; dt < 4; ++dt) {
                if (__ballot(mdt[dt] >= t) == 0ull) continue;
#pragma unroll
                for (int g = 0; g < 4; ++g) {
                    if (sub[dt][g] >= t) {
#pragma unroll
                        for (int e2 = 0; e2 < 4; ++e2) {
                            const float v = acc[dt][qt][4 * g + e2];
                            const uint32_t off = (uint32_t)(dt * 32 + 8 * g + e2);
                            if (v >= t && off < rows_left) {
                                if (ncand[qt] < (uint32_t)cap) clist[qt][ncand[qt] * 4] = make_uint2(__float_as_uint(v), row32 + off);
                                ++ncand[qt];
                            }
                        }
                    }
                }
            }
        }
    }
};

struct Mfma16 {
    typedef f32x4v Acc;
    static constexpr int TILE = 16, REGS = 4, DT = 8, QT = 4, SUBLISTS = 8;
    struct Frags { bf16x8 a[8], b[4]; };

    static __device__ __forceinline__ int src_swizzle(int row) { return ((row >> 2) & 1) << 1; }

    int a_base, b_base;
    __device__ __forceinline__ Mfma16(int lane, int wd, int wq) {
        const int cofs = (((lane >> 4) ^ (((lane >> 2) & 1) << 1)) << 4);
        a_base = (wd * 128 + (lane & 15)) * 64 + cofs;
        b_base = SUB_Q_REGION + (wq * 64 + (lane & 15)) * 64 + cofs;
    }
    __device__ __forceinline__ void read(const char *buf, Frags &f) const {
#pragma unroll
        for (int dt = 0; dt < 8; ++dt) f.a[dt] = *reinterpret_cast<const bf16x8 *>(buf + a_base + dt * 1024);
#pragma unroll
        for (int qt = 0; qt < 4; ++qt) f.b[qt] = *reinterpret_cast<const bf16x8 *>(buf + b_base + qt * 1024);
    }
    static __device__ __forceinline__ void mma(Acc (&acc)[8][4], const Frags &f, bool first) {
        if (first) {
            const f32x4v z = {0.f, 0.f, 0.f, 0.f};
#pragma unroll
            for (int dt = 0; dt < 8; ++dt)
#pragma unroll
                for (int qt = 0; qt < 4; ++qt) acc[dt][qt] = __builtin_amdgcn_mfma_f32_16x16x32_bf16(f.a[dt], f.b[qt], z, 0, 0, 0);
            return;
        }
#pragma unroll
        for (int dt = 0; dt < 8; ++dt)
#pragma unroll
            for (int qt = 0; qt < 4; ++qt) acc[dt][qt] = __builtin_amdgcn_mfma_f32_16x16x32_bf16(f.a[dt], f.b[qt], acc[dt][qt], 0, 0, 0);
    }

    static __device__ __forceinline__ void filter(const Acc (&acc)[8][4], const float (&thr)[4], const float (&cqv)[4], float nt,
                                                  int64_t row_base, const GemmArgs &a, uint2 *const (&clist)[4], uint32_t (&ncand)[4],
                                                  int cap) {
#pragma unroll
        for (int qt = 0; qt < 4; ++qt) {
            float sub[8];
#pragma unroll
            for (int dt = 0; dt < 8; ++dt) sub[dt] = max4_asm(acc[dt][qt]);
            const float t = fmaf(-cqv[qt], nt, thr[qt]);
            float mall = max3_asm(sub[0], sub[1], sub[2]);
            mall = max3_asm(mall, sub[3], sub[4]);
            mall = max3_asm(mall, sub[5], sub[6]);
            mall = fmaxf(mall, sub[7]);
            if (__ballot(mall >= t) == 0ull) continue;
#pragma unroll
            for (int dt = 0; dt < 8; ++dt) {
                if (sub[dt] >= t) {
#pragma unroll
                    for (int e = 0; e < 4; ++e) {
                        const float v = acc[dt][qt][e];
                        const int64_t doc = row_base + dt * 16 + e;
                        if (v >= t && doc < a.n_rows) {
                            if (ncand[qt] < (uint32_t)cap) clist[qt][ncand[qt] * 8] = make_uint2(__float_as_uint(v), (uint32_t)doc);
                            ++ncand[qt];
                        }
                    }
                }
            }
        }
    }
};

template <class S, int EPI, bool TAIL>
__device__ __forceinline__ void main_pass_256(const GemmArgs &a) {
    static_assert(EPI != EPI_GMAX || std::is_same<S, Mfma32>::value, "EPI_GMAX exists on the 32x32 shape only");
    extern __shared__ __attribute__((aligned(16))) char smem[];

    const int tid = threadIdx.x & (GEMM_THREADS - 1);
    const int lane = tid & 63;
    const int wv = __builtin_amdgcn_readfirstlane(tid >> 6);
    const int wd = wv >> 2;
    const int wq = wv & 3;
    const int lc = lane & (S::TILE - 1);
    const int lh = lane / S::TILE;
    const int cell = wd * (S::SUBLISTS / 2) + lh;
    const bool g1 = (wv >= 4);
    const int KS2 = TAIL ? (a.dim + SUB_K - 1) / SUB_K : a.dim / SUB_K;

    const int srow = wv * 16 + (lane >> 2);
    const int schunk = (lane & 3) ^ S::src_swizzle(srow);
    const S mfma(lane, wd, wq);

    const ItemWalk walk(a);
    for (int item = walk.first(a); item < walk.end; item += walk.step) {
        int r, qb;
        const int64_t ntile = walk.item(a, item, r, qb);
        if (ntile <= 0) continue;
        const int q0 = qb * TILE_Q;

        float thr[S::QT] = {}, cqv[S::QT] = {};
        uint32_t ncand[S::QT] = {};
        uint2 *clist[S::QT] = {};
        int cap = 0;
        if (EPI == EPI_FILTER) {
            int seg_r0;
            long long seg_base;
            cand_segment(a.lay, r, cap, seg_r0, seg_base);
#pragma unroll
            for (int qt = 0; qt < S::QT; ++qt) {
                const int q = q0 + wq * 64 + qt * S::TILE + lc;
                thr[qt] = (q < a.n_q) ? a.thr[q] : __builtin_nanf("");
                cqv[qt] = (q < a.n_q) ? a.cq[q] : 0.f;
                clist[qt] = a.cand + seg_base + ((int64_t)(r - seg_r0) * a.nq_pad + q) * S::SUBLISTS * cap + cell;
            }
#pragma unroll
            for (int qt = 0; qt < S::QT; ++qt) asm volatile("" : "+v"(thr[qt]), "+v"(cqv[qt]));
        }
        float *dst[S::QT] = {};
        if (EPI == EPI_STORE) {
            const int64_t pitch = a.store_pitch ? a.store_pitch : a.n_rows;
#pragma unroll
            for (int qt = 0; qt < S::QT; ++qt) {
                const int q = q0 + wq * 64 + qt * S::TILE + lc;
                if (q < a.n_q) dst[qt] = a.store + (int64_t)q * pitch;
            }
        }
        const uint16_t *qsrc[2];
#pragma unroll
        for (int i = 0; i < 2; ++i) {
            int qrow = q0 + i * 128 + srow;
            if (qrow > a.n_q - 1) qrow = a.n_q - 1;
            qsrc[i] = a.Q + (int64_t)qrow * a.dim + schunk * 8;
        }

        typename S::Acc acc[S::DT][S::QT];
        const int64_t U = ntile * KS2;

        int64_t iu = 0, it = 0;
        int iks = 0;
        const uint16_t *dsrc[2];
        auto tile_ptrs = [&]() {
            const int64_t row0 = (r + it * a.ranges) * a.tile_stride * TILE_DOCS;
#pragma unroll
            for (int i = 0; i < 2; ++i) {
                int64_t drow = row0 + (i * 128 + srow);
                if (drow > a.n_rows - 1) drow = a.n_rows - 1;
                dsrc[i] = a.D + drow * a.dim + schunk * 8;
            }
        };
        tile_ptrs();
        auto issue = [&]() {
            char *buf = smem + (int)(iu & (RING - 1)) * SUB_BYTES;
            const int k0 = iks * SUB_K;
            if (TAIL && iks == KS2 - 1) {
                const bool in = k0 + schunk * 8 < a.dim;
#pragma unroll
                for (int i = 0; i < 2; ++i)
                    glds16(in ? (const void *)(dsrc[i] + k0) : (const void *)g_zero_chunk, buf + (i * 512 + wv * 64) * 16);
#pragma unroll
                for (int i = 0; i < 2; ++i)
                    glds16(in ? (const void *)(qsrc[i] + k0) : (const void *)g_zero_chunk, buf + SUB_Q_REGION + (i * 512 + wv * 64) * 16);
            } else {
#pragma unroll
                for (int i = 0; i < 2; ++i) glds16(dsrc[i] + k0, buf + (i * 512 + wv * 64) * 16);
#pragma unroll
                for (int i = 0; i < 2; ++i) glds16(qsrc[i] + k0, buf + SUB_Q_REGION + (i * 512 + wv * 64) * 16);
            }
            ++iu;
            if (++iks == KS2) {
                iks = 0;
                ++it;
                tile_ptrs();
            }
        };

        auto epilogue = [&](int64_t vt, float nt) {
            const int64_t row_base = vt * a.tile_stride * TILE_DOCS + wd * 128 + 4 * lh;
            if constexpr (EPI == EPI_GMAX) {
                S::gmax(acc, a, vt, q0, wd, wq, lane);
            } else if constexpr (EPI == EPI_FILTER) {
                S::filter(acc, thr, cqv, nt, row_base, a, clist, ncand, cap);
            } else {
                const int64_t pitch = a.store_pitch ? a.store_pitch : a.n_rows;
#pragma unroll
                for (int qt = 0; qt < S::QT; ++qt) {
                    if (!dst[qt]) continue;
#pragma unroll
                    for (int dt = 0; dt < S::DT; ++dt)
#pragma unroll
                        for (int g = 0; g < S::REGS / 4; ++g) {
                            const int64_t doc = row_base + dt * S::TILE + 8 * g;
                            if ((pitch & 3) == 0 && doc + 3 < a.n_rows) {
                                *reinterpret_cast<float4 *>(dst[qt] + doc) = make_float4(acc[dt][qt][4 * g], acc[dt][qt][4 * g + 1],
                                                                                             acc[dt][qt][4 * g + 2], acc[dt][qt][4 * g + 3]);
                            } else {
#pragma unroll
                                for (int e2 = 0; e2 < 4; ++e2)
                                    if (doc + e2 < a.n_rows) dst[qt][doc + e2] = acc[dt][qt][4 * g + e2];
                            }
                        }
                }
            }
        };

        const int npro = U < 3 ? (int)U : 3;
        for (int i = 0; i < npro; ++i) issue();
        if (npro == 3)
            CCR_WAIT_VM(8);
        else if (npro == 2)
            CCR_WAIT_VM(4);
        else
            CCR_WAIT_VM(0);
        CCR_BARRIER();
        if (g1) CCR_BARRIER();

        int cks = 0;
        int64_t ct = 0;
        bool pending = false;
        int64_t pending_vt = 0;
        float pending_nt = 0.f;
        for (int64_t u = 0; u < U; ++u) {
            if (pending) {
                epilogue(pending_vt, pending_nt);
                pending = false;
            }
            if (u + 1 < U) {
                if (u + 2 < U)
                    CCR_WAIT_VM(4);
                else
                    CCR_WAIT_VM(0);
            }
            typename S::Frags f;
            mfma.read(smem + (int)(u & (RING - 1)) * SUB_BYTES, f);
            if (u + 3 < U) issue();
            CCR_WAIT_LGKM0();
            CCR_BARRIER();
            S::mma(acc, f, cks == 0);
            if (++cks == KS2) {
                cks = 0;
                const int64_t vt_done = r + ct * a.ranges;
                const float nt_done = EPI == EPI_FILTER ? load_uniform_f32(a.tile_norm + vt_done * a.tile_stride) : 0.f;
                if (g1) {
                    epilogue(vt_done, nt_done);
                } else {
                    pending = true;
                    pending_vt = vt_done;
                    pending_nt = nt_done;
                }
                ++ct;
            }
            CCR_BARRIER();
        }
        if (pending) epilogue(pending_vt, pending_nt);
        if (!g1) CCR_BARRIER();

        if (EPI == EPI_FILTER) {
#pragma unroll
            for (int qt = 0; qt < S::QT; ++qt)
                a.cnt[((int64_t)r * a.nq_pad + q0 + wq * 64 + qt * S::TILE + lc) * S::SUBLISTS + cell] = ncand[qt];
        }
        __syncthreads();
    }
}

template <int EPI, bool TAIL = false>
__global__ __launch_bounds__(GEMM_THREADS, 2) void gemm_topk_kernel(const GemmArgs a) { main_pass_256<Mfma32, EPI, TAIL>(a); }
template <int EPI, bool TAIL = false>
__global__ __launch_bounds__(GEMM_THREADS, 2) void gemm_topk16_kernel(const GemmArgs a) { main_pass_256<Mfma16, EPI, TAIL>(a); }


__device__ __forceinline__ int fresh_lane() {
    int l;
    asm volatile("v_mbcnt_lo_u32_b32 %0, -1, 0\n\tv_mbcnt_hi_u32_b32 %0, -1, %0" : "=v"(l));
    return l;
}
__device__ __forceinline__ uint32_t lds_offset(const void *p) {
    return (uint32_t)(uintptr_t)(const __attribute__((address_space(3))) void *)p;
}
__device__ __forceinline__ float2 lds_read_f2(uint32_t addr) {
    uint64_t v;
    asm volatile("ds_read_b64 %0, %1\n\ts_waitcnt lgkmcnt(0)" : "=v"(v) : "v"(addr) : "memory");
    return make_float2(__uint_as_float((uint32_t)v), __uint_as_float((uint32_t)(v >> 32)));
}
__device__ __forceinline__ uint32_t lds_add_rtn(uint32_t addr, uint32_t x) {
    uint32_t r;
    asm volatile("ds_add_rtn_u32 %0, %1, %2\n\ts_waitcnt lgkmcnt(0)" : "=v"(r) : "v"(addr), "v"(x) : "memory");
    return r;
}
constexpr int WIDE_SUB_BYTES = (TILE_DOCS + WIDE_Q) * SUB_K * 2;
constexpr int WIDE_Q_REGION = TILE_DOCS * SUB_K * 2;
constexpr int WIDE_RING = 3;
constexpr int WIDE_PIECES = 5;
constexpr int WIDE_QT = 6;
#ifndef WIDE_BFR
#define WIDE_BFR 6
#endif
constexpr int WIDE_RING_BYTES = WIDE_RING * WIDE_SUB_BYTES;
constexpr size_t WIDE_LDS = (size_t)WIDE_RING_BYTES + WIDE_Q * 8 + (size_t)(GEMM_THREADS / 64) * WIDE_QT * 64 * 4;

__global__ __launch_bounds__(GEMM_THREADS, 2) void gemm_topk16w_kernel(const GemmArgs a) {
    extern __shared__ __attribute__((aligned(16))) char smem[];
    float2 *s_tc = reinterpret_cast<float2 *>(smem + WIDE_RING_BYTES);
    uint32_t *s_cnt = reinterpret_cast<uint32_t *>(smem + WIDE_RING_BYTES + WIDE_Q * 8);
    const int wv = __builtin_amdgcn_readfirstlane((int)threadIdx.x >> 6);
    const int wd = wv >> 2;
    const int wq = wv & 3;
    const bool g1 = (wv >= 4);
    const int KS2 = a.dim / SUB_K;
    const uint32_t pitch = (uint32_t)a.dim * 2u;
    uint32_t lane_src, lane_lds;
    {
        const int ln = fresh_lane();
        const int pr = ln >> 2;
        lane_src = (uint32_t)pr * pitch + (uint32_t)(((ln & 3) ^ (((pr >> 2) & 1) << 1)) << 4);
        lane_lds = (uint32_t)((ln & 15) * 64 + (((ln >> 4) ^ (((ln >> 2) & 1) << 1)) << 4));
    }

    const ItemWalk walk(a);
    for (int item = walk.first(a); item < walk.end; item += walk.step) {
        int r, qb;
        const int64_t ntile = walk.item(a, item, r, qb);
        if (ntile <= 0) continue;
        const int q0 = qb * WIDE_Q;

        int cap, seg_r0;
        long long seg_base;
        cand_segment(a.lay, r, cap, seg_r0, seg_base);
        {
            const int ln = fresh_lane();
            const int tid = wv * 64 + ln;
            if (tid < WIDE_Q) {
                const int q = q0 + tid;
                s_tc[tid] = make_float2((q < a.n_q) ? a.thr[q] : __builtin_nanf(""), (q < a.n_q) ? a.cq[q] : 0.f);
            }
#pragma unroll
            for (int qt = 0; qt < WIDE_QT; ++qt) s_cnt[(wv * WIDE_QT + qt) * 64 + ln] = 0u;
        }
        CCR_WAIT_VM(0);

        const int qlimit = (a.n_q - 1 - q0 < WIDE_Q - 1) ? a.n_q - 1 - q0 : WIDE_Q - 1;
        const char *qblk = reinterpret_cast<const char *>(a.Q) + (int64_t)q0 * pitch;

        f32x4v acc[8][WIDE_QT];
        const int U = (int)(ntile * KS2);
        int islot = 0, iks = 0;
        int64_t it = 0;
        const char *dtile = nullptr;
        int dlimit = 0;
        auto tile_base = [&]() __attribute__((always_inline)) {
            const int64_t row0 = (r + it * a.ranges) * a.tile_stride * TILE_DOCS;
            dlimit = (a.n_rows - 1 - row0 < TILE_DOCS - 1) ? (int)(a.n_rows - 1 - row0) : TILE_DOCS - 1;
            dtile = reinterpret_cast<const char *>(a.D) + row0 * pitch;
        };
        tile_base();
        const bool q_whole = g1 ? ((wv - 4) * 96 + 95 <= qlimit) : (wv * 96 + 15 <= qlimit);
        auto issue = [&]() __attribute__((always_inline)) {
            char *buf = smem + islot * WIDE_SUB_BYTES;
            const uint32_t kb = (uint32_t)iks * (SUB_K * 2);
            if (q_whole && (g1 || dlimit == TILE_DOCS - 1)) {
                const uint32_t voff = lane_src + kb;
                if (!g1) {
                    const char *rows = dtile + (size_t)(wv * 64) * pitch;
#pragma unroll
                    for (int i = 0; i < 4; ++i) glds16(rows + (size_t)(i * 16) * pitch + voff, buf + (wv * 4 + i) * 1024);
                    glds16(qblk + (size_t)(wv * 96) * pitch + voff, buf + WIDE_Q_REGION + wv * 96 * 64);
                } else {
                    const char *rows = qblk + (size_t)((wv - 4) * 96 + 16) * pitch;
                    char *dst = buf + WIDE_Q_REGION + ((wv - 4) * 96 + 16) * 64;
#pragma unroll
                    for (int i = 0; i < WIDE_PIECES; ++i) glds16(rows + (size_t)(i * 16) * pitch + voff, dst + i * 1024);
                }
            } else {
                const int iln = fresh_lane();
                const int pr = iln >> 2;
                const uint32_t co = (uint32_t)(((iln & 3) ^ (((pr >> 2) & 1) << 1)) << 4) + kb;
                auto piece = [&](const char *rows, int row0, int limit, char *dst) __attribute__((always_inline)) {
                    int row = row0 + pr;
                    row = row < limit ? row : limit;
                    glds16(rows + ((uint32_t)row * pitch + co), dst);
                };
                if (!g1) {
#pragma unroll
                    for (int i = 0; i < 4; ++i) piece(dtile, (wv * 4 + i) * 16, dlimit, buf + (wv * 4 + i) * 1024);
                    piece(qblk, wv * 96, qlimit, buf + WIDE_Q_REGION + wv * 96 * 64);
                } else {
#pragma unroll
                    for (int i = 0; i < WIDE_PIECES; ++i)
                        piece(qblk, (wv - 4) * 96 + 16 * (1 + i), qlimit, buf + WIDE_Q_REGION + ((wv - 4) * 96 + 16 * (1 + i)) * 64);
                }
            }
            islot = islot == WIDE_RING - 1 ? 0 : islot + 1;
            if (++iks == KS2) {
                iks = 0;
                ++it;
                if (!g1) tile_base();
            }
        };

        auto epilogue = [&](int64_t vt, float nt) __attribute__((always_inline)) {
            const int eln = fresh_lane();
            const int l15o = eln & 15, lqo = eln >> 4;
            char *const cbase = reinterpret_cast<char *>(a.cand + seg_base + ((int64_t)(r - seg_r0) * a.nq_pad + q0) * 8 * cap + wd * 4);
            const uint32_t row_lo = (uint32_t)(wd * 128 + 4 * lqo);
            const uint32_t tc_addr = lds_offset(s_tc) + (uint32_t)l15o * 8u;
            const uint32_t cnt_addr = lds_offset(s_cnt) + (uint32_t)(lqo * 16 + l15o) * 4u;
            const int64_t tile_row0 = vt * a.tile_stride * TILE_DOCS;
            const uint32_t rows_left = a.n_rows - tile_row0 < TILE_DOCS ? (uint32_t)(a.n_rows - tile_row0) : (uint32_t)TILE_DOCS;
#pragma unroll
            for (int qt = 0; qt < WIDE_QT; ++qt) {
                float sub[8];
#pragma unroll
                for (int dt = 0; dt < 8; ++dt) sub[dt] = max4_asm(acc[dt][qt]);
                const float2 tc = lds_read_f2(tc_addr + (uint32_t)(wq * 96 + qt * 16) * 8u);
                const float t = fmaf(-tc.y, nt, tc.x);
                float mall = max3_asm(sub[0], sub[1], sub[2]);
                mall = max3_asm(mall, sub[3], sub[4]);
                mall = max3_asm(mall, sub[5], sub[6]);
                mall = fmaxf(mall, sub[7]);
                if (__ballot(mall >= t) != 0ull) {
                    const uint32_t ql = (uint32_t)(wq * 96 + qt * 16 + l15o);
                    const uint32_t cell = (ql * 8u * (uint32_t)cap + (uint32_t)lqo) * 8u;
                    const uint32_t cn = cnt_addr + (uint32_t)((wv * WIDE_QT + qt) * 64) * 4u;
#pragma unroll
                    for (int dt = 0; dt < 8; ++dt) {
                        if (sub[dt] >= t) {
#pragma unroll
                            for (int e = 0; e < 4; ++e) {
                                const float v = acc[dt][qt][e];
                                const uint32_t row = row_lo + dt * 16 + e;
                                if (v >= t && row < rows_left) {
                                    const uint32_t n = lds_add_rtn(cn, 1u);
                                    if (n < (uint32_t)cap)
                                        *reinterpret_cast<uint2 *>(cbase + (cell + n * 64u)) = make_uint2(__float_as_uint(v), (uint32_t)tile_row0 + row);
                                }
                            }
                        }
                    }
                }
            }
        };

        const int npro = U < 2 ? U : 2;
        for (int i = 0; i < npro; ++i) issue();
        if (npro == 2)
            wait_vm<WIDE_PIECES>();
        else
            CCR_WAIT_VM(0);
        CCR_BARRIER();
        if (g1) CCR_BARRIER();

        int cks = 0;
        int64_t ct = 0;
        bool pending = false;
        int64_t pending_vt = 0;
        float pending_nt = 0.f;
        int uslot = 0;
        for (int u = 0; u < U; ++u) {
            if (u + 2 < U) issue();
            __builtin_amdgcn_sched_barrier(0);
            if (pending) {
                epilogue(pending_vt, pending_nt);
                pending = false;
            }
            const char *abuf = smem + uslot * WIDE_SUB_BYTES;
            const char *bbuf = abuf + WIDE_Q_REGION;
            uslot = uslot == WIDE_RING - 1 ? 0 : uslot + 1;
            const int a_base = wd * 128 * 64 + (int)lane_lds;
            const int b_base = wq * 96 * 64 + (int)lane_lds;
            bf16x8 af[8], bfr[WIDE_BFR];
#pragma unroll
            for (int dt = 0; dt < 8; ++dt) af[dt] = *reinterpret_cast<const bf16x8 *>(abuf + a_base + dt * 1024);
#pragma unroll
            for (int qt = 0; qt < WIDE_BFR; ++qt) bfr[qt] = *reinterpret_cast<const bf16x8 *>(bbuf + b_base + qt * 1024);
            if (u + 2 < U)
                wait_vm<WIDE_PIECES>();
            else
                CCR_WAIT_VM(0);
            CCR_WAIT_LGKM0();
            CCR_BARRIER();
            if (cks == 0) {
                const f32x4v z = {0.f, 0.f, 0.f, 0.f};
#pragma unroll
                for (int qt = 0; qt < WIDE_QT; ++qt) {
#pragma unroll
                    for (int dt = 0; dt < 8; ++dt) acc[dt][qt] = __builtin_amdgcn_mfma_f32_16x16x32_bf16(af[dt], bfr[qt % WIDE_BFR], z, 0, 0, 0);
                    if (WIDE_BFR == 3 && qt < 3) {
                        __builtin_amdgcn_sched_barrier(0);
                        bfr[qt] = *reinterpret_cast<const bf16x8 *>(bbuf + b_base + (qt + 3) * 1024);
                        __builtin_amdgcn_sched_barrier(0);
                    }
                }
            } else {
#pragma unroll
                for (int qt = 0; qt < WIDE_QT; ++qt) {
#pragma unroll
                    for (int dt = 0; dt < 8; ++dt)
                        acc[dt][qt] = __builtin_amdgcn_mfma_f32_16x16x32_bf16(af[dt], bfr[qt % WIDE_BFR], acc[dt][qt], 0, 0, 0);
                    if (WIDE_BFR == 3 && qt < 3) {
                        __builtin_amdgcn_sched_barrier(0);
                        bfr[qt] = *reinterpret_cast<const bf16x8 *>(bbuf + b_base + (qt + 3) * 1024);
                        __builtin_amdgcn_sched_barrier(0);
                    }
                }
            }
            if (++cks == KS2) {
                cks = 0;
                const int64_t vt_done = r + ct * a.ranges;
                const float nt_done = load_uniform_f32(a.tile_norm + vt_done * a.tile_stride);
                if (g1) {
                    epilogue(vt_done, nt_done);
                } else {
                    pending = true;
                    pending_vt = vt_done;
                    pending_nt = nt_done;
                }
                ++ct;
            }
            CCR_WAIT_LGKM0();
            CCR_BARRIER();
        }
        if (pending) epilogue(pending_vt, pending_nt);
        if (!g1) CCR_BARRIER();

        {
            const int ln = fresh_lane();
#pragma unroll
            for (int qt = 0; qt < WIDE_QT; ++qt)
                a.cnt[((int64_t)r * a.nq_pad + q0 + wq * 96 + qt * 16 + (ln & 15)) * 8 + wd * 4 + (ln >> 4)] = s_cnt[(wv * WIDE_QT + qt) * 64 + ln];
        }
        __syncthreads();
    }
}

__global__ __launch_bounds__(256) void row_norms_bf16_kernel(const uint16_t *__restrict__ X, int64_t rows, int dim,
                                                            float *__restrict__ norms, uint32_t *__restrict__ max_bits,
                                                            uint32_t *__restrict__ tile_bits) {
    const int lane = threadIdx.x & 63;
    const int64_t wave = ((int64_t)blockIdx.x * blockDim.x + threadIdx.x) >> 6;
    const int64_t nwaves = ((int64_t)gridDim.x * blockDim.x) >> 6;
    const int chunk = tile_bits ? 64 : 1;
    uint32_t wbits = 0u;
    for (int64_t r0 = wave * chunk; r0 < rows; r0 += nwaves * chunk) {
        uint32_t cbits = 0u;
        const int64_t r1 = r0 + chunk < rows ? r0 + chunk : rows;
        for (int64_t r = r0; r < r1; ++r) {
            const uint16_t *x = X + r * dim;
            float s = 0.f;
            for (int c = lane * 8; c < dim; c += 64 * 8) {
                const uint4 v = *reinterpret_cast<const uint4 *>(x + c);
                const uint32_t w[4] = {v.x, v.y, v.z, v.w};
#pragma unroll
                for (int e = 0; e < 4; ++e) {
                    const float lo = __uint_as_float(w[e] << 16), hi = __uint_as_float(w[e] & 0xffff0000u);
                    s = fmaf(lo, lo, s);
                    s = fmaf(hi, hi, s);
                }
            }
#pragma unroll
            for (int off = 32; off >= 1; off >>= 1) s += __shfl_xor(s, off, 64);
            const float n = sqrtf(s);
            if (norms && lane == 0) norms[r] = n;
            const uint32_t nb = __float_as_uint(n) & 0x7fffffffu;
            cbits = nb > cbits ? nb : cbits;
        }
        if (tile_bits && lane == 0) atomicMax(tile_bits + r0 / TILE_DOCS, cbits);
        wbits = cbits > wbits ? cbits : wbits;
    }
    if (max_bits && lane == 0 && wbits > __hip_atomic_load(max_bits, __ATOMIC_RELAXED, __HIP_MEMORY_SCOPE_AGENT)) atomicMax(max_bits, wbits);
}

__global__ __launch_bounds__(256) void tile_norms_kernel(const float *__restrict__ row_bounds, int64_t rows,
                                                        uint32_t *__restrict__ tile_bits) {
    __shared__ uint32_t s_w[4];
    const int64_t r = (int64_t)blockIdx.x * TILE_DOCS + threadIdx.x;
    uint32_t b = r < rows ? (__float_as_uint(row_bounds[r]) & 0x7fffffffu) : 0u;
#pragma unroll
    for (int off = 32; off >= 1; off >>= 1) {
        const uint32_t o = __shfl_xor(b, off, 64);
        b = o > b ? o : b;
    }
    if ((threadIdx.x & 63) == 0) s_w[threadIdx.x >> 6] = b;
    __syncthreads();
    if (threadIdx.x == 0) {
        const uint32_t m01 = s_w[0] > s_w[1] ? s_w[0] : s_w[1], m23 = s_w[2] > s_w[3] ? s_w[2] : s_w[3];
        tile_bits[blockIdx.x] = m01 > m23 ? m01 : m23;
    }
}

__global__ __launch_bounds__(1024) void max_tile_norm_kernel(const uint32_t *__restrict__ tile_bits, int64_t tiles,
                                                            uint32_t *__restrict__ max_bits) {
    __shared__ uint32_t s_w[16];
    uint32_t b = 0u;
    for (int64_t t = threadIdx.x; t < tiles; t += 1024) {
        const uint32_t v = tile_bits[t];
        b = v > b ? v : b;
    }
#pragma unroll
    for (int off = 32; off >= 1; off >>= 1) {
        const uint32_t o = __shfl_xor(b, off, 64);
        b = o > b ? o : b;
    }
    if ((threadIdx.x & 63) == 0) s_w[threadIdx.x >> 6] = b;
    __syncthreads();
    if (threadIdx.x == 0) {
        uint32_t m = 0u;
        for (int w = 0; w < 16; ++w) m = s_w[w] > m ? s_w[w] : m;
        *max_bits = m;
    }
}

__global__ __launch_bounds__(256) void threshold_kernel(const float *__restrict__ gmax, int64_t n_groups, int n_q, int nq_pad,
                                                       int k, const float *__restrict__ qnorm,
                                                       const uint32_t *__restrict__ dmax_bits, float gamma,
                                                       const float *__restrict__ tile_norm, int64_t sample_stride,
                                                       float *__restrict__ thr, float *__restrict__ cq) {
    __shared__ uint32_t s_hist[16][256];
    __shared__ uint32_t s_prefix[16], s_remaining[16];
    const int tid = threadIdx.x;
    const int ql = tid & 15, ph = tid >> 4;
    const int q = blockIdx.x * 16 + ql;
    if (tid < 16) {
        s_prefix[tid] = 0;
        s_remaining[tid] = (uint32_t)k;
    }
    const float dmax = __uint_as_float(*dmax_bits);
    const float c = (q < n_q) ? ((dmax < INFINITY) ? gamma * (qnorm[q] * 1.001f) * 1.001f : __builtin_nanf("")) : 0.f;
    auto tile_of = [&](int64_t g) { return tile_norm[(g / GROUPS_PER_TILE) * sample_stride]; };
    uint32_t mask = 0;
    for (int shift = 24; shift >= 0; shift -= 8) {
        for (int b = tid; b < 16 * 256; b += 256) (&s_hist[0][0])[b] = 0;
        __syncthreads();
        const uint32_t prefix = s_prefix[ql];
        int64_t i = ph;
        for (; i + 240 < n_groups; i += 256) {
            float v[16], tn[16];
#pragma unroll
            for (int j = 0; j < 16; ++j) {
                v[j] = gmax[(i + 16 * j) * nq_pad + q];
                tn[j] = tile_of(i + 16 * j);
            }
#pragma unroll
            for (int j = 0; j < 16; ++j) {
                const uint32_t o = f32_orderable(fmaf(-c, tn[j], v[j]));
                if ((o & mask) == prefix) atomicAdd(&s_hist[ql][(o >> shift) & 255u], 1u);
            }
        }
        for (; i < n_groups; i += 16) {
            const uint32_t o = f32_orderable(fmaf(-c, tile_of(i), gmax[i * nq_pad + q]));
            if ((o & mask) == prefix) atomicAdd(&s_hist[ql][(o >> shift) & 255u], 1u);
        }
        __syncthreads();
        {
            const int qi = tid >> 4, part = tid & 15;
            const uint32_t remaining = s_remaining[qi];
            uint32_t hb[16];
            uint32_t own = 0;
#pragma unroll
            for (int j = 0; j < 16; ++j) {
                hb[j] = s_hist[qi][16 * part + j];
                own += hb[j];
            }
            uint32_t incl = own;
#pragma unroll
            for (int off = 1; off < 16; off <<= 1) {
                const uint32_t t = __shfl_down(incl, off, 16);
                if (part + off < 16) incl += t;
            }
            const uint32_t above = incl - own;
            const uint32_t total = __shfl(incl, 0, 16);
            __syncthreads();
            if (above < remaining && remaining <= incl) {
                uint32_t cum = above;
                int d = 16 * part;
#pragma unroll
                for (int j = 15; j >= 1; --j) {
                    if (cum + hb[j] >= remaining) {
                        d = 16 * part + j;
                        break;
                    }
                    cum += hb[j];
                }
                s_prefix[qi] |= (uint32_t)d << shift;
                s_remaining[qi] = remaining - cum;
            } else if (part == 0 && total < remaining) {
                s_remaining[qi] = remaining - (total - hb[0]);
            }
        }
        mask |= 0xffu << shift;
        __syncthreads();
    }
    if (tid < 16) {
        const int qq = blockIdx.x * 16 + tid;
        if (qq < n_q) {
            const float tau = orderable_to_f32(s_prefix[tid]);
            cq[qq] = c;
            thr[qq] = (c < INFINITY) ? tau : __builtin_nanf("");
        }
    }
}


template <int THREADS, int BATCH, class At, class Want, class Put>
__device__ __forceinline__ void sweep_sublists(int tid, int n_lists, int first, int longest, const uint32_t *s_cnt, At at,
                                               Want want, Put put) {
    if (longest <= first) return;
    int lw = 0;
    while ((1 << lw) < longest - first) ++lw;
    const int sweep = n_lists << lw;
    for (int i0 = tid; i0 < sweep; i0 += THREADS * BATCH) {
        uint2 e[BATCH];
        int jj[BATCH], ss[BATCH];
#pragma unroll
        for (int u = 0; u < BATCH; ++u) {
            const int i = i0 + u * THREADS;
            const int j = i >> lw, sl = first + (i & ((1 << lw) - 1));
            jj[u] = -1;
            ss[u] = sl;
            if (i < sweep && (uint32_t)sl < s_cnt[j] && want(j, sl)) {
                jj[u] = j;
                e[u] = at(j, sl);
            }
        }
#pragma unroll
        for (int u = 0; u < BATCH; ++u)
            if (jj[u] >= 0) put(jj[u], ss[u], e[u]);
    }
}

__global__ __launch_bounds__(256) void threshold_update_kernel(const uint2 *__restrict__ cand, const uint32_t *__restrict__ cnt,
                                                              int nsub_full, int nsub_part, int part_blocks, int prev_full,
                                                              int prev_part, int prev_blocks, int qb_per, int sp, int nq_pad,
                                                              const CandLayout lay, int k, int compact,
                                                              const float *__restrict__ cq, const float *__restrict__ tile_norm,
                                                              uint32_t *__restrict__ top, int top_in, int top_out,
                                                              float *__restrict__ thr, int tile_q) {
    extern __shared__ __attribute__((aligned(16))) uint32_t s_val[];
    __shared__ uint32_t s_hist[256];
    __shared__ uint32_t s_ctl[4];
    __shared__ uint32_t s_cnt[2048];
    __shared__ uint32_t s_total, s_maxc, s_fill, s_eq;
    const int tid = threadIdx.x;
    const int q = blockIdx.x;
    const int qpos = (q / tile_q) % qb_per;
    const int nsub = qpos < part_blocks ? nsub_part : nsub_full;
    uint32_t *top_n = top;
    uint32_t *top_v = top ? top + nq_pad + (int64_t)q * k : nullptr;
    const bool have_prev = top_in && top_n[q] == (uint32_t)k;
    const int j0 = have_prev ? (qpos < prev_blocks ? prev_part : prev_full) : 0;
    if (tid == 0) {
        s_total = have_prev ? (uint32_t)k : 0u;
        s_maxc = 0;
        s_fill = 0;
    }
    __syncthreads();
    uint32_t my = 0, mymax = 0;
    for (int j = j0 + tid; j < nsub; j += blockDim.x) {
        uint32_t c = cnt[((int64_t)(j / sp) * nq_pad + q) * sp + (j % sp)];
        int cap;
        (void)cand_sublist(lay, j / sp, q, j % sp, nq_pad, sp, cap);
        if (c > (uint32_t)cap) c = (uint32_t)cap;
        s_cnt[j - j0] = c;
        my += c;
        mymax = c > mymax ? c : mymax;
    }
    if (my) {
        atomicAdd(&s_total, my);
        atomicMax(&s_maxc, mymax);
    }
    __syncthreads();
    if (s_total < (uint32_t)k) {
        if (top_out && tid == 0) top_n[q] = 0u;
        return;
    }
    auto sub_base = [&](int j) -> int64_t {
        int cap;
        return cand_sublist(lay, (j0 + j) / sp, q, (j0 + j) % sp, nq_pad, sp, cap);
    };
    uint32_t kth = 0;
    int need_eq = 0, M = 0;
    bool selected = false;
    {
        const int maxc = (int)s_maxc;
        const float c = cq[q];
        uint32_t keep = 0u;
        auto append = [&](uint32_t o) {
            if (o >= keep) {
                const uint32_t p = atomicAdd(&s_fill, 1u);
                if (p < (uint32_t)compact) s_val[p] = o;
            }
        };
        for (int round = 0; round < 4; ++round) {
            __syncthreads();
            if (tid == 0) s_fill = 0;
            __syncthreads();
            selected = false;
            if (have_prev)
                for (int i = tid; i < k; i += blockDim.x) append(top_v[i]);
            sweep_sublists<256, 8>(
                tid, nsub - j0, 0, maxc, s_cnt, [&](int j, int sl) -> uint2 { return cand[sub_base(j) + (int64_t)sl * sp]; },
                [](int, int) { return true; },
                [&](int, int, uint2 e) { append(f32_orderable(fmaf(-c, tile_norm[e.y / TILE_DOCS], __uint_as_float(e.x)))); });
            __syncthreads();
            const uint32_t filled = s_fill;
            M = (int)(filled < (uint32_t)compact ? filled : (uint32_t)compact);
            if (M < k) break;
            block_radix_select(
                [&](int64_t i, bool &skip) -> uint32_t {
                    (void)skip;
                    return s_val[i];
                },
                (int64_t)M, k, s_hist, s_ctl, kth, need_eq);
            selected = true;
            if (filled <= (uint32_t)compact || kth <= keep) break;
            keep = kth;
        }
    }
    if (top_out) {
        if (!selected) {
            if (tid == 0) top_n[q] = 0u;
        } else {
            __syncthreads();
            if (tid == 0) s_fill = s_eq = 0u;
            __syncthreads();
            for (int i = tid; i < M; i += blockDim.x) {
                const uint32_t v = s_val[i];
                bool take = v > kth;
                if (v == kth) take = atomicAdd(&s_eq, 1u) < (uint32_t)need_eq;
                if (take) top_v[atomicAdd(&s_fill, 1u)] = v;
            }
            if (tid == 0) top_n[q] = (uint32_t)k;
        }
    }
    if (tid == 0) {
        const float t1 = orderable_to_f32(kth);
        if (t1 > thr[q]) thr[q] = t1;
    }
}

template <int THREADS>
__global__ __launch_bounds__(THREADS) void select_rescore_kernel(const uint2 *__restrict__ cand, const uint32_t *__restrict__ cnt,
                                                            int ranges, int sp, int nq_pad, const CandLayout lay, int k, int rescore_cap, int compact,
                                                            int64_t n_rows, float *__restrict__ thr, const float *__restrict__ cq,
                                                            const float *__restrict__ tile_norm, const float *__restrict__ row_norm,
                                                            const uint32_t *__restrict__ dmax_bits,
                                                            const uint16_t *__restrict__ Q, const uint16_t *__restrict__ D,
                                                            int dim, int64_t id_offset, float *__restrict__ out_scores,
                                                            int64_t *__restrict__ out_ids, uint32_t *__restrict__ flag_count,
                                                            uint32_t *__restrict__ flag_list,
                                                            unsigned long long *__restrict__ stat_cand,
                                                            const uint32_t *__restrict__ out_rows) {
    extern __shared__ __attribute__((aligned(16))) char sm[];
    const size_t cnt_bytes = ((size_t)(ranges + 1) * 4 + 15) & ~(size_t)15;
    uint16_t *s_q = reinterpret_cast<uint16_t *>(sm);
    uint32_t *s_cnt = reinterpret_cast<uint32_t *>(sm + (((size_t)dim * 2 + 15) & ~(size_t)15));
    uint32_t *s_off = reinterpret_cast<uint32_t *>(reinterpret_cast<char *>(s_cnt) + cnt_bytes);
    unsigned long long *s_keys = reinterpret_cast<unsigned long long *>(reinterpret_cast<char *>(s_off) + cnt_bytes);
    uint2 *s_comp = reinterpret_cast<uint2 *>(s_keys + rescore_cap);
    __shared__ uint32_t s_hist[256];
    __shared__ uint32_t s_ctl[4];
    __shared__ uint32_t s_wsum[THREADS / 64];
    __shared__ int s_flag;
    __shared__ uint32_t s_total, s_maxc, s_fill;
    __shared__ uint32_t s_ncoll;

    const int tid = threadIdx.x;
    const int q = blockIdx.x;
    if (tid == 0) {
        s_flag = 0;
        s_total = 0;
        s_ncoll = 0;
        s_maxc = 0;
        s_fill = 0;
    }
    __syncthreads();
    const int per = (ranges + THREADS - 1) / THREADS;
    uint32_t my = 0, mymax = 0;
    for (int j = tid * per; j < min(ranges, tid * per + per); ++j) {
        uint32_t c = cnt[((int64_t)(j / sp) * nq_pad + q) * sp + (j % sp)];
        int cap;
        (void)cand_sublist(lay, j / sp, q, j % sp, nq_pad, sp, cap);
        if (c > (uint32_t)cap) {
            s_flag = 1;
            c = (uint32_t)cap;
        }
        s_cnt[j] = c;
        my += c;
        mymax = c > mymax ? c : mymax;
    }
    {
        const int lane = tid & 63, wid = tid >> 6;
        uint32_t incl = my;
#pragma unroll
        for (int off = 1; off < 64; off <<= 1) {
            const uint32_t t = __shfl_up(incl, off, 64);
            if (lane >= off) incl += t;
        }
        if (lane == 63) s_wsum[wid] = incl;
        if (my) atomicMax(&s_maxc, mymax);
        for (int c = tid; c < dim / 8; c += THREADS)
            reinterpret_cast<uint4 *>(s_q)[c] = reinterpret_cast<const uint4 *>(Q + (int64_t)q * dim)[c];
        __syncthreads();
        uint32_t base = incl - my;
        for (int w = 0; w < wid; ++w) base += s_wsum[w];
        for (int j = tid * per; j < min(ranges, tid * per + per); ++j) {
            s_off[j] = base;
            base += s_cnt[j];
        }
        if (tid == THREADS - 1) s_total = base;
        __syncthreads();
    }
    if (tid == 0 && stat_cand) atomicAdd(stat_cand, (unsigned long long)s_total);
    bool bad = (s_flag != 0) || (s_total < (uint32_t)k);
    bool dense_only = (s_flag == 0) && bad;
    if (dense_only && thr && tid == 0) thr[q] = -INFINITY;

    auto sub_base = [&](int j) -> int64_t {
        int cap;
        return cand_sublist(lay, j / sp, q, j % sp, nq_pad, sp, cap);
    };
    auto at = [&](int j, int sl) -> uint2 { return cand[sub_base(j) + (int64_t)sl * sp]; };
    const int coll_cap = rescore_cap;
    uint32_t kth = 0;
    int need_eq = 0;
    int n_lds = 0;
    const float c = cq[q];
    bool row_lb = false;

    if (!bad && s_total <= (uint32_t)compact) {
        constexpr int FIRST = THREADS >= 1024 ? 8 : 4, MAXL = 8;
        {
            const int per_cell = FIRST * sp / 2;
            const int nload = (ranges / sp) * per_cell;
            uint4 v[MAXL];
#pragma unroll
            for (int t = 0; t < MAXL; ++t) {
                const int x = tid + t * THREADS;
                if (x < nload) {
                    const int cell = x / per_cell, w = x - cell * per_cell;
                    int cap;
                    v[t] = *reinterpret_cast<const uint4 *>(cand + cand_sublist(lay, cell, q, 0, nq_pad, sp, cap) + 2 * w);
                }
            }
#pragma unroll
            for (int t = 0; t < MAXL; ++t) {
                const int x = tid + t * THREADS;
                if (x < nload) {
                    const int cell = x / per_cell, w = x - cell * per_cell;
                    const int slot = (2 * w) / sp, part = (2 * w) % sp;
                    const int j = cell * sp + part;
                    if ((uint32_t)slot < s_cnt[j]) s_comp[s_off[j] + slot] = make_uint2(v[t].x, v[t].y);
                    if ((uint32_t)slot < s_cnt[j + 1]) s_comp[s_off[j + 1] + slot] = make_uint2(v[t].z, v[t].w);
                }
            }
        }
        sweep_sublists<THREADS, 8>(tid, ranges, FIRST, (int)s_maxc, s_cnt, at, [](int, int) { return true; },
                                   [&](int j, int sl, uint2 e) { s_comp[s_off[j] + sl] = e; });
        __syncthreads();
        n_lds = (int)s_total;
        for (int i0 = tid; i0 < n_lds; i0 += 4 * THREADS) {
            uint2 e[4];
            float rn[4];
#pragma unroll
            for (int u = 0; u < 4; ++u) {
                const int i = i0 + u * THREADS;
                e[u] = s_comp[i < n_lds ? i : i0];
                rn[u] = tile_norm[e[u].y / TILE_DOCS];
            }
#pragma unroll
            for (int u = 0; u < 4; ++u) {
                const int i = i0 + u * THREADS;
                if (i < n_lds) s_comp[i] = make_uint2(__float_as_uint(fmaf(-c, rn[u], __uint_as_float(e[u].x))), e[u].y);
            }
        }
        __syncthreads();
    } else if (!bad && compact < k) {
        bad = dense_only = true;
    } else if (!bad) {
        float keep = -INFINITY;
        bool fits = false;
        row_lb = true;
        for (int round = 0; round < 4 && !fits; ++round) {
            __syncthreads();
            if (tid == 0) s_fill = 0u;
            __syncthreads();
            sweep_sublists<THREADS, 8>(tid, ranges, 0, (int)s_maxc, s_cnt, at, [](int, int) { return true; },
                                       [&](int, int, uint2 e) {
                                           const float cn = c * row_norm[e.y];
                                           if (__uint_as_float(e.x) + cn >= keep) {
                                               const uint32_t p = atomicAdd(&s_fill, 1u);
                                               if (p < (uint32_t)compact) s_comp[p] = make_uint2(__float_as_uint(__uint_as_float(e.x) - cn), e.y);
                                           }
                                       });
            __syncthreads();
            if (s_fill <= (uint32_t)compact) {
                fits = true;
            } else {
                uint32_t kth0 = 0;
                int eq0 = 0;
                block_radix_select(
                    [&](int64_t i, bool &skip) -> uint32_t {
                        (void)skip;
                        return f32_orderable(__uint_as_float(s_comp[i].x));
                    },
                    compact, k, s_hist, s_ctl, kth0, eq0);
                keep = orderable_to_f32(kth0);
            }
        }
        if (fits)
            n_lds = (int)s_fill;
        else
            bad = dense_only = true;
    }
    if (!bad) {
        const int M = n_lds;
        block_radix_select(
            [&](int64_t i, bool &skip) -> uint32_t {
                (void)skip;
                return f32_orderable(__uint_as_float(s_comp[i].x));
            },
            M, k, s_hist, s_ctl, kth, need_eq);
        const float low = orderable_to_f32(kth);
        if (thr && low < thr[q]) {
            __syncthreads();
            if (tid == 0) {
                thr[q] = low;
                const uint32_t p = atomicAdd(flag_count, 1u);
                flag_list[p] = (out_rows ? out_rows[q] : (uint32_t)q);
            }
            return;
        }
        const float loose = fmaf(-2.f * c, __uint_as_float(*dmax_bits), low);
        for (int i = tid; i < M; i += THREADS) {
            const uint2 e = s_comp[i];
            const float lb = __uint_as_float(e.x);
            if (lb >= loose && fmaf(c, row_norm[e.y], fmaf(c, row_lb ? row_norm[e.y] : tile_norm[e.y / TILE_DOCS], lb)) >= low) {
                const uint32_t p = atomicAdd(&s_ncoll, 1u);
                if (p < (uint32_t)coll_cap) s_keys[p] = (unsigned long long)e.y;
            }
        }
        __syncthreads();
        if (s_ncoll > (uint32_t)coll_cap) bad = dense_only = true;
    }
    if (bad) {
        if (tid == 0) {
            const uint32_t p = atomicAdd(flag_count, 1u);
            flag_list[p] = (out_rows ? out_rows[q] : (uint32_t)q) | (dense_only ? FLAG_DENSE : 0u);
        }
        return;
    }
    const int ncoll = (int)s_ncoll;
    const int np2 = pow2_ceil(ncoll);
    const size_t stage_bytes = (size_t)compact * 8;
    int SB = (size_t)ncoll * 144 <= stage_bytes ? 128 : ((size_t)ncoll * 80 <= stage_bytes ? 64 : 0);
    constexpr int PRE = 8;
    if (SB == 128 && ncoll * 8 > PRE * THREADS) SB = 64;
    if (SB != 0 && ncoll <= 2 * THREADS && ncoll * (SB / 16) <= PRE * THREADS) {
        char *stage = reinterpret_cast<char *>(s_comp);
        const int stride = SB + 16;
        const int lpr = SB / 16;
        const int row_bytes = dim * 2;
        const char *Dbytes = reinterpret_cast<const char *>(D);
        const int col = (tid % lpr) * 16;
#define CCR_PIECES(X) X(0) X(1) X(2) X(3) X(4) X(5) X(6) X(7)
        const int acol = col < row_bytes ? col : 0;
        const char *Dcol = Dbytes + acol;
        const int npiece = ncoll * lpr;
#define CCR_DECL(j)                                                                                              \
    const int idx##j = tid + j * THREADS;                                                                        \
    const char *src##j = Dcol + (int64_t)(uint32_t)s_keys[idx##j < npiece ? idx##j / lpr : 0] * row_bytes;      \
    uint4 pre##j = *reinterpret_cast<const uint4 *>(src##j);
        CCR_PIECES(CCR_DECL)
#undef CCR_DECL
        double acc[2] = {0.0, 0.0};
        for (int k0 = 0; k0 < row_bytes; k0 += SB) {
            __syncthreads();
            const bool col_in = k0 + col < row_bytes;
#define CCR_PUT(j) \
    if (col_in && idx##j < npiece) *reinterpret_cast<uint4 *>(stage + (idx##j / lpr) * stride + col) = pre##j;
            CCR_PIECES(CCR_PUT)
#undef CCR_PUT
            __syncthreads();
            {
                const int kn = (k0 + SB + col < row_bytes) ? k0 + SB : -acol;
#define CCR_GET(j) pre##j = *reinterpret_cast<const uint4 *>(src##j + kn);
                CCR_PIECES(CCR_GET)
#undef CCR_GET
            }
#undef CCR_PIECES
#pragma unroll
            for (int j = 0; j < 2; ++j) {
                const int i = tid + j * THREADS;
                if (i < ncoll) {
                    double a = acc[j];
                    for (int c = 0; c < lpr && k0 + c * 16 < row_bytes; ++c) {
                        const uint4 dv = *reinterpret_cast<const uint4 *>(stage + (size_t)i * stride + c * 16);
                        const uint4 qv = *reinterpret_cast<const uint4 *>(reinterpret_cast<const char *>(s_q) + k0 + c * 16);
                        const uint32_t dw[4] = {dv.x, dv.y, dv.z, dv.w};
                        const uint32_t qw[4] = {qv.x, qv.y, qv.z, qv.w};
#pragma unroll
                        for (int e = 0; e < 4; ++e) {
                            a = fma((double)__uint_as_float(qw[e] << 16), (double)__uint_as_float(dw[e] << 16), a);
                            a = fma((double)__uint_as_float(qw[e] & 0xffff0000u), (double)__uint_as_float(dw[e] & 0xffff0000u), a);
                        }
                    }
                    acc[j] = a;
                }
            }
        }
        __syncthreads();
#pragma unroll
        for (int j = 0; j < 2; ++j) {
            const int i = tid + j * THREADS;
            if (i < np2) s_keys[i] = i < ncoll ? make_key((float)acc[j], (uint32_t)s_keys[i]) : 0ull;
        }
    } else {
        for (int i = tid; i < np2; i += blockDim.x) {
            unsigned long long key = 0ull;
            if (i < ncoll) {
                const uint32_t row = (uint32_t)s_keys[i];
                key = make_key(canonical_dot(s_q, D + (int64_t)row * dim, dim), row);
            }
            s_keys[i] = key;
        }
    }
    block_bitonic_sort_desc(s_keys, np2);
    const int64_t orow = out_rows ? (int64_t)out_rows[q] : (int64_t)q;
    for (int i = tid; i < k; i += blockDim.x) {
        const unsigned long long key = s_keys[i];
        out_scores[orow * k + i] = key_score(key);
        store_id(out_ids, orow * k + i, id_offset, key_idx(key));
    }
}

__global__ __launch_bounds__(256) void partition_flags_kernel(const uint32_t *__restrict__ flags, int begin, int n,
                                                             uint32_t *__restrict__ retry_list, uint32_t *__restrict__ dense_list,
                                                             uint32_t *__restrict__ counts) {
    __shared__ uint32_t s_n[2];
    if (threadIdx.x == 0) s_n[0] = s_n[1] = 0;
    __syncthreads();
    for (int i = begin + threadIdx.x; i < n; i += blockDim.x) {
        const uint32_t f = flags[i];
        if (f & FLAG_DENSE)
            dense_list[atomicAdd(&s_n[1], 1u)] = f & ~FLAG_DENSE;
        else
            retry_list[atomicAdd(&s_n[0], 1u)] = f;
    }
    __syncthreads();
    if (threadIdx.x < 2) counts[threadIdx.x] = s_n[threadIdx.x];
}

__global__ __launch_bounds__(256) void underfilled_to_retry_kernel(uint32_t *__restrict__ flags, int begin, int n,
                                                                  const float *__restrict__ thr_safe, float *__restrict__ thr) {
    const int i = begin + blockIdx.x * blockDim.x + threadIdx.x;
    if (i >= n) return;
    const uint32_t f = flags[i];
    const uint32_t q = f & ~FLAG_DENSE;
    if ((f & FLAG_DENSE) && thr[q] == -INFINITY && thr_safe[q] > -INFINITY) {
        thr[q] = thr_safe[q];
        flags[i] = q;
    }
}

__global__ __launch_bounds__(256) void scatter_thresholds_kernel(const uint32_t *__restrict__ list, int n, const float *__restrict__ thr2,
                                                                float *__restrict__ thr) {
    const int i = blockIdx.x * blockDim.x + threadIdx.x;
    if (i < n) thr[list[i]] = thr2[i];
}

__global__ __launch_bounds__(256) void gather_queries_kernel(const uint16_t *__restrict__ Q, int dim, const uint32_t *__restrict__ list,
                                                            int n, const float *__restrict__ thr, const float *__restrict__ delta,
                                                            uint16_t *__restrict__ Q2, float *__restrict__ thr2,
                                                            float *__restrict__ delta2) {
    const int i = blockIdx.x;
    if (i >= n) return;
    const uint32_t q = list[i];
    for (int c = threadIdx.x; c < dim / 8; c += blockDim.x)
        reinterpret_cast<uint4 *>(Q2 + (int64_t)i * dim)[c] = reinterpret_cast<const uint4 *>(Q + (int64_t)q * dim)[c];
    if (threadIdx.x == 0) {
        thr2[i] = thr[q];
        delta2[i] = delta[q];
    }
}

int ensure_dynamic_lds(const void *kernel, size_t lds) {
    static std::mutex mu;
    static std::set<std::pair<const void *, int>> done;
    int dev = 0;
    CCR_HIP_CHECK(hipGetDevice(&dev));
    std::lock_guard<std::mutex> lock(mu);
    if (done.count({kernel, dev})) return CCR_OK;
    CCR_HIP_CHECK(hipFuncSetAttribute(kernel, hipFuncAttributeMaxDynamicSharedMemorySize, (int)lds));
    done.insert({kernel, dev});
    return CCR_OK;
}

template <class K>
static int launch_kernel(K kernel, size_t lds, const GemmArgs &a, int grid, hipStream_t s) {
    const int rc = ensure_dynamic_lds(reinterpret_cast<const void *>(kernel), lds);
    if (rc != CCR_OK) return rc;
    hipLaunchKernelGGL(kernel, dim3(grid), dim3(GEMM_THREADS), lds, s, a);
    CCR_LAUNCH_CHECK();
    return CCR_OK;
}

int launch_gemm(const GemmArgs &a, MainKernel kind, int epi, int grid, hipStream_t s) {
    if (epi != EPI_FILTER && epi != EPI_GMAX && epi != EPI_STORE) {
        set_error("launch_gemm: unknown epilogue %d", epi);
        return CCR_ERR_INVALID;
    }
    if (kind == MAIN_WIDE) {
        if (epi != EPI_FILTER || a.dim % SUB_K != 0 || a.dim < SUB_K) {
            set_error("launch_gemm: the 256 x 384 kernel takes EPI_FILTER and dim %% %d == 0 only (epi %d, dim %d)", SUB_K, epi, a.dim);
            return CCR_ERR_INVALID;
        }
        return launch_kernel(&gemm_topk16w_kernel, WIDE_LDS, a, grid, s);
    }
    typedef void (*Kernel)(const GemmArgs);
    static const Kernel k256[2][3][2] = {
        {{gemm_topk_kernel<EPI_FILTER>, gemm_topk_kernel<EPI_FILTER, true>},
         {gemm_topk_kernel<EPI_GMAX>, gemm_topk_kernel<EPI_GMAX, true>},
         {gemm_topk_kernel<EPI_STORE>, gemm_topk_kernel<EPI_STORE, true>}},
        {{gemm_topk16_kernel<EPI_FILTER>, gemm_topk16_kernel<EPI_FILTER, true>},
         {nullptr, nullptr},
         {gemm_topk16_kernel<EPI_STORE>, gemm_topk16_kernel<EPI_STORE, true>}},
    };
    const Kernel k = k256[kind == MAIN_16X16][epi][a.dim % SUB_K != 0];
    if (!k) {
        set_error("launch_gemm: the 16x16x32 kernel has no EPI_GMAX");
        return CCR_ERR_INVALID;
    }
    return launch_kernel(k, RING * (size_t)SUB_BYTES, a, grid, s);
}

int launch_row_norms_bf16(const uint16_t *X, int64_t rows, int dim, float *norms, uint32_t *max_bits, uint32_t *tile_bits,
                          hipStream_t s) {
    if (rows <= 0) return CCR_OK;
    int64_t blocks = tile_bits ? (rows + 255) / 256 : (rows + 3) / 4;
    if (blocks > 2048) blocks = 2048;
    hipLaunchKernelGGL(row_norms_bf16_kernel, dim3((unsigned)blocks), dim3(256), 0, s, X, rows, dim, norms, max_bits, tile_bits);
    CCR_LAUNCH_CHECK();
    return CCR_OK;
}

int launch_tile_norms(const float *row_bounds, int64_t rows, uint32_t *tile_bits, uint32_t *max_bits, hipStream_t s) {
    if (rows <= 0) return CCR_OK;
    const int64_t tiles = (rows + TILE_DOCS - 1) / TILE_DOCS;
    hipLaunchKernelGGL(tile_norms_kernel, dim3((unsigned)tiles), dim3(256), 0, s, row_bounds, rows, tile_bits);
    hipLaunchKernelGGL(max_tile_norm_kernel, dim3(1), dim3(1024), 0, s, tile_bits, tiles, max_bits);
    CCR_LAUNCH_CHECK();
    return CCR_OK;
}

__global__ __launch_bounds__(256) void threshold_small_kernel(const float *__restrict__ gmax, int n_groups, int nq_pad, int k,
                                                             const float *__restrict__ qnorm, const uint32_t *__restrict__ dmax_bits,
                                                             float gamma, const float *__restrict__ tile_norm, int64_t sample_stride,
                                                             float *__restrict__ thr, float *__restrict__ cq, uint32_t *__restrict__ zero_cnt,
                                                             int zero_per_query) {
    extern __shared__ __attribute__((aligned(16))) uint32_t s_low[];
    __shared__ uint32_t s_hist[256];
    __shared__ uint32_t s_ctl[4];
    const int tid = threadIdx.x, q = blockIdx.x;
    const float dmax = __uint_as_float(*dmax_bits);
    const float c = (dmax < INFINITY) ? gamma * (qnorm[q] * 1.001f) * 1.001f : __builtin_nanf("");
    for (int g = tid; g < n_groups; g += 256)
        s_low[g] = f32_orderable(fmaf(-c, tile_norm[(int64_t)(g / GROUPS_PER_TILE) * sample_stride], gmax[(int64_t)g * nq_pad + q]));
    if (zero_cnt && tid < zero_per_query) zero_cnt[q * zero_per_query + tid] = 0u;
    __syncthreads();
    uint32_t kth = 0;
    int need_eq = 0;
    block_radix_select<true>(
        [&](int64_t i, bool &skip) -> uint32_t {
            (void)skip;
            return s_low[i];
        },
        n_groups, k, s_hist, s_ctl, kth, need_eq);
    if (tid == 0) {
        cq[q] = c;
        thr[q] = (c < INFINITY) ? orderable_to_f32(kth) : __builtin_nanf("");
    }
}

int launch_threshold(const float *gmax, int64_t n_groups, int n_q, int nq_pad, int k, const float *qnorm,
                     const uint32_t *dmax_bits, int dim, const float *tile_norm, int64_t sample_stride, float *thr, float *cq,
                     hipStream_t s, uint32_t *zero_cnt, int zero_per_query) {
    if (n_q <= 128 && n_groups >= k && n_groups <= 16384 && zero_per_query <= 256) {
        if (n_groups * 4 > 32 * 1024) {
            const int rc = ensure_dynamic_lds(reinterpret_cast<const void *>(&threshold_small_kernel), 72 * 1024);
            if (rc != CCR_OK) return rc;
        }
        hipLaunchKernelGGL(threshold_small_kernel, dim3(n_q), dim3(256), (size_t)n_groups * 4, s, gmax, (int)n_groups, nq_pad, k, qnorm, dmax_bits,
                           mfma_gamma(dim), tile_norm, sample_stride, thr, cq, zero_cnt, zero_per_query);
        CCR_LAUNCH_CHECK();
        return CCR_OK;
    }
    if (zero_cnt) CCR_HIP_CHECK(hipMemsetAsync(zero_cnt, 0, (size_t)n_q * zero_per_query * 4, s));
    hipLaunchKernelGGL(threshold_kernel, dim3(nq_pad / 16), dim3(256), 0, s, gmax, n_groups, n_q, nq_pad, k, qnorm, dmax_bits,
                       mfma_gamma(dim), tile_norm, sample_stride, thr, cq);
    CCR_LAUNCH_CHECK();
    return CCR_OK;
}

int launch_threshold_update(const uint2 *cand, const uint32_t *cnt, int nsub, int nsub_part, int part_blocks, int prev_nsub, int prev_part,
                            int prev_blocks, int qb_per, int sp, int n_q, int nq_pad, const CandLayout &lay, int k, const float *cq,
                            const float *tile_norm, uint32_t *top, bool top_in, bool top_out, float *thr, hipStream_t s, int tile_q) {
    if (nsub_part < nsub) nsub_part = nsub;
    if (prev_part < prev_nsub) prev_part = prev_nsub;
    if (nsub_part > 2048) {
        set_error("threshold_update: %d sub-lists exceed 2048", nsub_part);
        return CCR_ERR_INVALID;
    }
    if (!top) top_in = top_out = false;
    int compact = std::max(4096, 8 * pow2_ceil(k));
    if (compact > 32768) compact = 32768;
    const size_t lds = (size_t)compact * 4;
    if (lds > 48 * 1024) {
        const int rc = ensure_dynamic_lds(reinterpret_cast<const void *>(&threshold_update_kernel), 128 * 1024);
        if (rc != CCR_OK) return rc;
    }
    hipLaunchKernelGGL(threshold_update_kernel, dim3(n_q), dim3(256), lds, s, cand, cnt, nsub, nsub_part, part_blocks, prev_nsub, prev_part,
                       prev_blocks, qb_per > 0 ? qb_per : 1, sp, nq_pad, lay, k, compact, cq, tile_norm, top, top_in ? 1 : 0, top_out ? 1 : 0,
                       thr, tile_q > 0 ? tile_q : TILE_Q);
    CCR_LAUNCH_CHECK();
    return CCR_OK;
}

constexpr size_t SELECT_LDS_BUDGET = 150 * 1024;

static size_t select_fixed_lds(int dim, int ranges, int rescore_cap) {
    const size_t cnt_bytes = ((size_t)(ranges + 1) * 4 + 15) & ~(size_t)15;
    return (((size_t)dim * 2 + 15) & ~(size_t)15) + 2 * cnt_bytes + (size_t)rescore_cap * 8;
}

int select_compact_entries(int dim, int ranges, int rescore_cap, int64_t want) {
    const size_t fixed = select_fixed_lds(dim, ranges, rescore_cap);
    const int64_t fit = fixed + 2048 < SELECT_LDS_BUDGET ? (int64_t)((SELECT_LDS_BUDGET - fixed) / 8) : 256;
    return (int)std::min<int64_t>(std::max<int64_t>(want, 2048), fit) / 256 * 256;
}

int launch_partition_flags(const uint32_t *flags, int begin, int n, uint32_t *retry_list, uint32_t *dense_list, uint32_t *counts,
                           hipStream_t s) {
    hipLaunchKernelGGL(partition_flags_kernel, dim3(1), dim3(256), 0, s, flags, begin, n, retry_list, dense_list, counts);
    CCR_LAUNCH_CHECK();
    return CCR_OK;
}

int launch_underfilled_to_retry(uint32_t *flags, int begin, int n, const float *thr_safe, float *thr, hipStream_t s) {
    if (n <= begin) return CCR_OK;
    hipLaunchKernelGGL(underfilled_to_retry_kernel, dim3((n - begin + 255) / 256), dim3(256), 0, s, flags, begin, n, thr_safe, thr);
    CCR_LAUNCH_CHECK();
    return CCR_OK;
}

int launch_scatter_thresholds(const uint32_t *list, int n, const float *thr2, float *thr, hipStream_t s) {
    if (n <= 0) return CCR_OK;
    hipLaunchKernelGGL(scatter_thresholds_kernel, dim3((n + 255) / 256), dim3(256), 0, s, list, n, thr2, thr);
    CCR_LAUNCH_CHECK();
    return CCR_OK;
}

int launch_gather_queries(const uint16_t *Q, int dim, const uint32_t *list, int n, const float *thr, const float *delta, uint16_t *Q2,
                          float *thr2, float *delta2, hipStream_t s) {
    if (n <= 0) return CCR_OK;
    hipLaunchKernelGGL(gather_queries_kernel, dim3(n), dim3(256), 0, s, Q, dim, list, n, thr, delta, Q2, thr2, delta2);
    CCR_LAUNCH_CHECK();
    return CCR_OK;
}

int launch_select_rescore(const uint2 *cand, const uint32_t *cnt, int ranges, int sp, int n_q, int nq_pad, const CandLayout &lay, int k,
                          int rescore_cap, int compact, int64_t n_rows, float *thr, const float *cq, const float *tile_norm, const float *row_norm,
                          const uint32_t *dmax_bits, const uint16_t *Q,
                          const uint16_t *D, int dim, int64_t id_offset, float *out_scores, int64_t *out_ids,
                          uint32_t *flag_count, uint32_t *flag_list, unsigned long long *stat_cand, const uint32_t *out_rows,
                          hipStream_t s) {
    const size_t lds = select_fixed_lds(dim, ranges, rescore_cap) + (size_t)compact * 8;
    const bool wide = rescore_cap > 512 || compact > 8192 || ranges > 1024;
    auto go = [&](auto kernel, int threads) -> int {
        if (lds > 48 * 1024) {
            const int rc = ensure_dynamic_lds(reinterpret_cast<const void *>(kernel), SELECT_LDS_BUDGET + 8192);
            if (rc != CCR_OK) return rc;
        }
        hipLaunchKernelGGL(kernel, dim3(n_q), dim3(threads), lds, s, cand, cnt, ranges, sp, nq_pad, lay, k, rescore_cap, compact,
                           n_rows, thr, cq, tile_norm, row_norm, dmax_bits, Q, D, dim, id_offset, out_scores, out_ids, flag_count, flag_list, stat_cand,
                           out_rows);
        CCR_LAUNCH_CHECK();
        return CCR_OK;
    };
    if (wide) return go(&select_rescore_kernel<1024>, 1024);
    return go(&select_rescore_kernel<256>, 256);
}

}
```

crowd-coachable-recommendations_amd/csrc/ccr_index.h:

```cpp
#pragma once
#include "ccr_common.h"

namespace ccr {

struct Knobs {
    int qgroups;
    int progressive;
    int max_phases;
    int mfma16;
    int sample_div;
    int ranges;
    int optimistic;
    int opt_rank;
    int max_lists;
    int narrow;
    int narrow_grid;
    int wide;
    int narrow_groups;
};
Knobs read_knobs();

constexpr int FALLBACK_ROWS = 16;

Plan make_plan(int64_t n_rows, int dim, int n_q, int k, int flags, int num_cu, const Knobs &kn);

struct Bump {
    size_t off;
    size_t take(size_t bytes) { const size_t o = off; off = (off + bytes + 255) / 256 * 256; return o; }
};

struct SearchWs {
    float *qnorm, *thr, *cq, *gmax;
    uint32_t *cnt;
    uint2 *cand;
    uint32_t *flag_count, *flag_list;
    unsigned long long *stat_cand;
    uint32_t *top;
    float *thr_safe, *cq_safe, *dense;
    uint16_t *Q2;
    float *thr2, *cq2;
    uint32_t *retry_list, *dense_list, *counts, *flag2, *list_b, *list_c;
    size_t cand_bytes, dense_bytes, retry_bytes, total;
};
SearchWs search_ws(const Plan &p, int64_t n_rows, int dim, int n_q, int k, char *base);

enum MainKernel { MAIN_32X32, MAIN_16X16, MAIN_WIDE };
int launch_gemm(const GemmArgs &a, MainKernel kind, int epi, int grid, hipStream_t s);
int launch_shard_header(const ccr_shard_header &h, void *message, hipStream_t s);
int ensure_dynamic_lds(const void *kernel, size_t lds);
int launch_row_norms_bf16(const uint16_t *X, int64_t rows, int dim, float *norms, uint32_t *max_bits, uint32_t *tile_bits,
                          hipStream_t s);
int launch_tile_norms(const float *row_bounds, int64_t rows, uint32_t *tile_bits, uint32_t *max_bits, hipStream_t s);
int launch_threshold(const float *gmax, int64_t n_groups, int n_q, int nq_pad, int k, const float *qnorm,
                     const uint32_t *dmax_bits, int dim, const float *tile_norm, int64_t sample_stride, float *thr, float *cq,
                     hipStream_t s, uint32_t *zero_cnt = nullptr, int zero_per_query = 0);
int select_compact_entries(int dim, int ranges, int rescore_cap, int64_t want);
int launch_select_rescore(const uint2 *cand, const uint32_t *cnt, int ranges, int sp, int n_q, int nq_pad, const CandLayout &lay, int k,
                          int rescore_cap, int compact, int64_t n_rows, float *thr, const float *cq, const float *tile_norm, const float *row_norm,
                          const uint32_t *dmax_bits, const uint16_t *Q, const uint16_t *D, int dim, int64_t id_offset, float *out_scores, int64_t *out_ids,
                          uint32_t *flag_count, uint32_t *flag_list, unsigned long long *stat_cand, const uint32_t *out_rows,
                          hipStream_t s);
int launch_partition_flags(const uint32_t *flags, int begin, int n, uint32_t *retry_list, uint32_t *dense_list, uint32_t *counts,
                           hipStream_t s);
int launch_underfilled_to_retry(uint32_t *flags, int begin, int n, const float *thr_safe, float *thr, hipStream_t s);
int launch_scatter_thresholds(const uint32_t *list, int n, const float *thr2, float *thr, hipStream_t s);
int launch_gather_queries(const uint16_t *Q, int dim, const uint32_t *list, int n, const float *thr, const float *cq, uint16_t *Q2,
                          float *thr2, float *cq2, hipStream_t s);
int launch_threshold_update(const uint2 *cand, const uint32_t *cnt, int nsub, int nsub_part, int part_blocks, int prev_nsub, int prev_part,
                            int prev_blocks, int qb_per, int sp, int n_q, int nq_pad, const CandLayout &lay, int k, const float *cq,
                            const float *tile_norm, uint32_t *top, bool top_in, bool top_out, float *thr, hipStream_t s, int tile_q = TILE_Q);
int launch_dense_scores(const uint16_t *D, int64_t n_rows, int dim, const uint16_t *Q, const uint32_t *qlist,
                        int q_begin, int nq_chunk, const uint32_t *count_dev, float *out, hipStream_t s);
int launch_dense_select(const float *scores, int64_t n_rows, int k, const uint32_t *out_rows, int q_begin, int nq_chunk,
                        const uint32_t *count_dev, int64_t id_offset, float *out_scores, int64_t *out_ids, hipStream_t s,
                        bool aggregate = true, const uint32_t *in_rows = nullptr, bool in_rows_compact = false);

int launch_margin_select(const float *scores, int64_t pitch, int64_t n_rows, int k, int dim, const uint16_t *Q, const uint16_t *D,
                         const float *tile_norm, const float *row_norm, const uint32_t *dmax_bits, const float *hint, const uint32_t *out_rows,
                         int q_begin, int nq_chunk, int64_t id_offset, float *out_scores, int64_t *out_ids, uint32_t *flag_count, uint32_t *flag_list,
                         hipStream_t s);

enum SearchEvent { EV_BEGIN, EV_SAMPLE_BEGIN, EV_SAMPLE_END, EV_MAIN_BEGIN, EV_MAIN_END, EV_SELECT_END, EV_DONE, EV_ASYNC_END, EV_COUNT };

}

struct ccr_index {
    const uint16_t *D;
    int64_t n_rows;
    int dim;
    int64_t offset;
    int64_t id_out;
    uint32_t *dmax_bits;
    float *tile_norm;
    size_t tile_bytes;
    const float *row_norm;
    float *row_norm_own;
    size_t row_bytes;
    bool have_events;
    bool main_pass_recorded;
    int num_cu;
    int device;
    ccr::Knobs knobs;
    hipEvent_t ev[ccr::EV_COUNT];
    volatile uint32_t *host_flags;
    ccr::Plan plan;
    int plan_nq, plan_k, plan_flags;
    ccr_search_stats stats;
    struct {
        bool active;
        const uint16_t *Q;
        int n_q, k;
        float *out_scores;
        int64_t *out_ids;
        char *ws;
        hipStream_t stream;
    } pending;
};
```

include/ccr_retrieval.h:

```cpp
#ifndef CCR_RETRIEVAL_H
#define CCR_RETRIEVAL_H

#include <stddef.h>
#include <stdint.h>

#ifdef __cplusplus
extern "C" {
#endif

#define CCR_OK 0
#define CCR_ERR_INVALID (-1)
#define CCR_ERR_HIP (-2)
#define CCR_ERR_WORKSPACE (-3)
#define CCR_ERR_BLOCK_ID (-4)

#define CCR_DTYPE_F32 0
#define CCR_DTYPE_F16 1
#define CCR_DTYPE_BF16 2

#define CCR_SEARCH_DEFAULT 0
#define CCR_SEARCH_FORCE_DENSE 1
#define CCR_SEARCH_FORCE_FUSED 2
#define CCR_SEARCH_ASYNC 4

#define CCR_SCORES_CANONICAL 0
#define CCR_SCORES_MFMA 1

typedef struct ccr_index ccr_index;

typedef struct ccr_search_stats {
    int32_t path;
    int32_t n_fallback;
    int32_t sample_tiles;
    int32_t ranges;
    int32_t cap;
    int32_t sublists;
    int64_t n_candidates;
    float ms_sample;
    float ms_threshold;
    float ms_main;
    float ms_select;
    float ms_fallback;
    float ms_total;
    int32_t n_retried;
    int32_t n_dense;
    int32_t main_launches;
    int32_t opt_rank;
    int32_t main_tile_queries;
    int32_t reserved0;
} ccr_search_stats;

const char *ccr_last_error(void);
int ccr_version(void);

int ccr_pack_bf16(const float *src, uint16_t *dst, float *norms, int64_t rows, int dim, int normalize, void *stream);
int ccr_pack_bf16_ex(const float *src, uint16_t *dst, float *norms, float *row_norm_bounds, int64_t rows, int dim, int normalize,
                     void *stream);

int ccr_pack_bf16_padded(const float *src, int64_t rows, int src_dim, uint16_t *dst, int dst_dim, float *norms,
                         float *row_norm_bounds, int normalize, void *stream);

int ccr_meanpool_pack_bf16(const void *hidden, int hidden_dtype, const int64_t *mask, uint16_t *dst_bf16,
                           float *dst_f32, int B, int L, int dim, int normalize, void *stream);
int ccr_meanpool_pack_bf16_ex(const void *hidden, int hidden_dtype, const int64_t *mask, uint16_t *dst_bf16,
                              float *dst_f32, const int64_t *dst_rows, float *row_norm_bounds, int B, int L, int dim,
                              int normalize, void *stream);

int ccr_meanpool_pack_bf16_packed(const void *hidden, int hidden_dtype, const int32_t *seq_start, const int32_t *seq_len,
                                  uint16_t *dst_bf16, float *dst_f32, const int64_t *dst_rows, float *row_norm_bounds, int n_seq,
                                  int dim, int normalize, void *stream);

int ccr_meanpool_bwd(const float *grad, const int64_t *mask, void *dhidden, int hidden_dtype, int B, int L, int dim,
                     void *stream);

int ccr_embed_layernorm(const float *word_table, int64_t vocab, const float *position_table, int64_t n_positions,
                        const float *type_table, int64_t n_types, const int64_t *token_ids, const int64_t *positions,
                        const int64_t *token_types, const float *gamma, const float *beta, float eps, float *out_f32,
                        uint16_t *out_bf16, int64_t rows, int dim, void *stream);
int ccr_gelu_bf16(const uint16_t *x, uint16_t *y, int64_t n, void *stream);
int ccr_attention_bf16(const uint16_t *qkv, const int32_t *seq_start, const int32_t *seq_len, uint16_t *out, int n_seq,
                       int n_heads, int max_len, int pad_len, float scale, void *stream);
int ccr_add_layernorm(const uint16_t *x_bf16, const float *residual, const float *gamma, const float *beta, float eps,
                      float *out_f32, uint16_t *out_bf16, int64_t rows, int dim, void *stream);
int ccr_attention_half(const uint16_t *qkv, const int32_t *seq_start, const int32_t *seq_len, uint16_t *out, int n_seq, int n_heads,
                       int max_len, int pad_len, float scale, int half_dtype, void *stream);
int ccr_add_layernorm_half(const uint16_t *x_half, const float *residual, const float *gamma, const float *beta, float eps,
                           float *out_f32, uint16_t *out_half, int64_t rows, int dim, int half_dtype, void *stream);
int ccr_embed_layernorm_half(const float *word_table, int64_t vocab, const float *position_table, int64_t n_positions,
                             const float *type_table, int64_t n_types, const int64_t *token_ids, const int64_t *positions,
                             const int64_t *token_types, const float *gamma, const float *beta, float eps, float *out_f32,
                             uint16_t *out_half, int64_t rows, int dim, int half_dtype, void *stream);
int ccr_gelu_half(const uint16_t *x, uint16_t *y, int64_t n, int half_dtype, void *stream);

int ccr_index_create(const uint16_t *D_bf16, int64_t n_rows, int dim, int64_t global_row_offset, void *stream,
                     ccr_index **out);
int ccr_index_create_with_norms(const uint16_t *D_bf16, int64_t n_rows, int dim, int64_t global_row_offset,
                                const float *row_norm_bounds, void *stream, ccr_index **out);
int ccr_index_destroy(ccr_index *index);
int64_t ccr_index_rows(const ccr_index *index);
int ccr_index_dim(const ccr_index *index);

size_t ccr_search_workspace_bytes(const ccr_index *index, int n_q, int k);
int ccr_search(ccr_index *index, const uint16_t *Q_bf16, int n_q, int k, float *out_scores, int64_t *out_ids,
               void *workspace, size_t ws_bytes, int flags, void *stream);
int ccr_search_finish(ccr_index *index);
int ccr_search_last_stats(const ccr_index *index, ccr_search_stats *stats );
int ccr_search_stream_wait_main_pass(const ccr_index *index, void *stream);

int ccr_scores(const ccr_index *index, const uint16_t *Q_bf16, int n_q, int mode, float *out, void *stream);

size_t ccr_search_blocked_workspace_bytes(const ccr_index *index, int n_q, int k, const int64_t *block_ptr_host);
int ccr_search_blocked(ccr_index *index, const uint16_t *Q_bf16, int n_q, int k, const int64_t *block_ptr_host,
                       const int64_t *block_idx, float *out_scores, int64_t *out_ids, void *workspace, size_t ws_bytes,
                       int flags, void *stream);

size_t ccr_search_sparse_prior_workspace_bytes(const ccr_index *index, int n_q, int k, const int64_t *prior_ptr_host);
int ccr_search_sparse_prior(ccr_index *index, const uint16_t *Q_bf16, int n_q, int k, const int64_t *prior_ptr_host,
                            const int64_t *prior_idx, const double *prior_val, double *out_scores, int64_t *out_ids,
                            void *workspace, size_t ws_bytes, int flags, void *stream);

int ccr_colsum_bf16(const uint16_t *X, int64_t rows, int dim, double *out , void *stream);

int ccr_merge_topk(const float *scores, const int64_t *ids, int R, int n_q, int k, float *out_scores,
                   int64_t *out_ids, void *stream);
int ccr_merge_topk_strided(const float *scores, const int64_t *ids, int64_t score_rank_stride, int64_t id_rank_stride,
                           int R, int n_q, int k, float *out_scores, int64_t *out_ids, void *stream);

#define CCR_SHARD_MAGIC 0x4d524343u
typedef struct ccr_shard_header {
    uint32_t magic;
    uint32_t n_flagged;
    uint32_t k_valid;
    uint32_t n_covered;
    int64_t row_offset;
    int64_t n_rows;
} ccr_shard_header;
size_t ccr_shard_message_bytes(int n_q, int k);
int ccr_search_shard(ccr_index *index, const uint16_t *Q_bf16, int n_q, int k, void *message, void *workspace, size_t ws_bytes,
                     int flags, void *stream);
int ccr_shard_message_fill(void *message, int n_q, int k, int k_valid, const float *scores, const int64_t *ids, int64_t row_offset,
                           int64_t n_rows, void *stream);
int ccr_merge_shard_messages(const void *messages, int64_t message_stride_bytes, int R, int n_q, int k, float *out_scores,
                             int64_t *out_ids, void *stream);
int ccr_merge_short_lists(const void *messages, int64_t message_stride_bytes, int R, int n_q, int k_list, int k_out, float *out_scores,
                          int64_t *out_ids, uint32_t *flags, uint32_t *n_flagged, void *stream);

int ccr_apply_block(const float *in_scores, const int64_t *in_ids, int n_q, int k_in, const int64_t *block_ptr,
                    const int64_t *block_idx, int64_t n_rows_total, float *out_scores, int64_t *out_ids, int k_out,
                    void *stream);

size_t ccr_inbatch_ce_workspace_bytes(int B, int dim);
int ccr_inbatch_pack3_bf16(const float *q, const float *p, const float *n, int B, int dim, uint16_t *out, void *stream);
int ccr_inbatch_ce_fwd_f32(const float *q, const float *p, const float *n, int B, int dim, float inv_temperature, uint16_t *packed,
                           float *loss, float *lse, void *workspace, size_t ws_bytes, void *stream);
int ccr_inbatch_ce_fwd(const uint16_t *Qe, const uint16_t *Pe, const uint16_t *Ne, int B, int dim,
                       float inv_temperature, float *loss, float *lse, void *workspace, size_t ws_bytes, void *stream);
int ccr_inbatch_ce_bwd(const uint16_t *Qe, const uint16_t *Pe, const uint16_t *Ne, const float *lse, int B, int dim,
                       float inv_temperature, float grad_out, float *dQ, float *dP, float *dN, void *workspace,
                       size_t ws_bytes, void *stream);
int ccr_inbatch_ce_bwd_dev(const uint16_t *Qe, const uint16_t *Pe, const uint16_t *Ne, const float *lse, int B, int dim,
                           float inv_temperature, const float *grad_out_dev, float *dQ, float *dP, float *dN,
                           void *workspace, size_t ws_bytes, void *stream);

int ccr_rank_metrics(const int64_t *ids, int n_q, int k, const int64_t *qrel_ptr, const int64_t *qrel_idx,
                     const int32_t *k_values, int n_k, float *out_rr, int32_t *out_hits, void *stream);

typedef struct ccr_bm25_index ccr_bm25_index;
int ccr_bm25_index_create(const int64_t *indptr_host, const int32_t *doc_ids, const float *tf, const double *doc_k,
                          int64_t n_terms, int64_t n_docs, double k1, ccr_bm25_index **out);
int ccr_bm25_index_destroy(ccr_bm25_index *index);
int ccr_bm25_index_set_idf(ccr_bm25_index *index, const double *idf_host, double *contrib, void *stream);
size_t ccr_bm25_search_workspace_bytes(const ccr_bm25_index *index, int n_q, int max_terms_per_query);
size_t ccr_bm25_search_workspace_bytes_k(const ccr_bm25_index *index, int n_q, int max_terms_per_query, int k);
int ccr_bm25_search_last_stats(const ccr_bm25_index *index, int64_t *out4);
int ccr_bm25_search(const ccr_bm25_index *index, const int64_t *q_ptr_host, const int32_t *q_terms_host,
                    const double *q_idf_host, int n_q, int k, float *out_scores, int64_t *out_ids, void *workspace,
                    size_t ws_bytes, void *stream);

#ifdef __cplusplus
}
#endif
#endif
```

Baseline: 254,000.

## Skip sampled tiles in main pass and merge their candidates separately

```diff
diff --git a/crowd-coachable-recommendations_amd/ccrec_amd/_lib.py b/crowd-coachable-recommendations_amd/ccrec_amd/_lib.py
--- a/crowd-coachable-recommendations_amd/ccrec_amd/_lib.py
+++ b/crowd-coachable-recommendations_amd/ccrec_amd/_lib.py
@@ -40,7 +40,7 @@
                 ("ms_main", ctypes.c_float), ("ms_select", ctypes.c_float), ("ms_fallback", ctypes.c_float),
                 ("ms_total", ctypes.c_float), ("n_retried", ctypes.c_int32), ("n_dense", ctypes.c_int32),
                 ("main_launches", ctypes.c_int32), ("opt_rank", ctypes.c_int32), ("main_tile_queries", ctypes.c_int32),
-                ("reserved0", ctypes.c_int32)]
+                ("main_tiles_skipped", ctypes.c_int32)]
 
 
 class CcrError(RuntimeError):
diff --git a/crowd-coachable-recommendations_amd/csrc/ccr_api.hip b/crowd-coachable-recommendations_amd/csrc/ccr_api.hip
--- a/crowd-coachable-recommendations_amd/csrc/ccr_api.hip
+++ b/crowd-coachable-recommendations_amd/csrc/ccr_api.hip
@@ -107,8 +107,14 @@
     return r;
 }
 
+static bool skips_sample(const Plan &p, int k, int64_t sample) {
+    if (!p.fused || p.narrow || sample < 1 || sample * 4 > p.full_tiles) return false;
+    const int64_t stride = p.full_tiles / sample;
+    return (p.full_tiles - sample) * TILE_DOCS >= 8 * (int64_t)k && p.tiles < ((int64_t)1 << 24) && stride <= 65536;
+}
+
 static MainPassChoice choose_main_pass(const Plan &p, int k, int64_t sample_a, int64_t sample_b, int64_t sample_c, const Knobs &kn,
-                                       bool single_only = false) {
+                                       bool single_only = false, bool skip = false) {
     const int nrc = NUM_XCD / p.main_qgroups, qb_per = p.main_qblocks / p.main_qgroups, per_x = p.grid / NUM_XCD;
     const double tile_cost = p.tile_q == WIDE_Q ? 1.37 : 1.0;
     int64_t max_lists = p.rescore_cap > 512 ? 2048 : 1024;
@@ -130,6 +136,7 @@
         const int64_t smp = pass == 0 ? sample_a : (pass == 1 ? sample_b : sample_c);
         if ((pass >= 1 && smp == sample_a) || (pass == 2 && smp == sample_b)) continue;
         const double fs = (double)smp / (double)p.tiles;
+        const int64_t mt = skip ? p.tiles - smp : p.tiles;
         const double smp_cost = sample_cost(smp);
         auto survivors = [&](double fa, double fb) -> double {
             if (fa <= 0.0) return (double)k / fs;
@@ -140,7 +147,7 @@
         for (int64_t R = r_lo; R <= std::min(r_hi, target * 2); R += NUM_XCD) {
             if (kn.ranges > 0 && R != std::min<int64_t>(r_hi, std::max<int64_t>(r_lo, round_up(kn.ranges, NUM_XCD)))) continue;
             const int64_t items = R / nrc * qb_per;
-            const double item_cost = ((double)((p.tiles + R - 1) / R) + 0.15) * tile_cost;
+            const double item_cost = ((double)((mt + R - 1) / R) + 0.15) * tile_cost;
             auto rounds = [&](int64_t n) { return (double)((n + per_x - 1) / per_x); };
             const double common = smp_cost + select_per_range * (double)R + 1e-3 * std::abs((double)(R - target));
             const double single = rounds(items) * item_cost + hit_w * survivors(0.0, 0.0) + common;
@@ -149,7 +156,7 @@
                 best_choice = {smp, R, 0, 0, 0};
             }
             if (kn.optimistic != 0 && smp * GROUPS_PER_TILE >= 4 * 40) {
-                const int rank = optimistic_rank(k, smp, p.tiles, kn);
+                const int rank = optimistic_rank(k, smp, mt, kn);
                 if ((int64_t)rank * 4 <= smp * GROUPS_PER_TILE) {
                     const double pass = std::max((double)rank / fs, (double)k);
                     const double opt = rounds(items) * item_cost + hit_w * pass + common - (kn.optimistic == 1 ? 1e9 : 0.0);
@@ -159,7 +166,7 @@
                     }
                 }
             }
-            if (!(prog_on && items > per_x && (double)p.tiles / (double)R >= 8.0)) continue;
+            if (!(prog_on && items > per_x && (double)mt / (double)R >= 8.0)) continue;
             const double fa = (double)per_x / (double)items;
             const double two = (1.0 + rounds(items - per_x)) * item_cost + phase_w + hit_w * survivors(fa, 0.0) + common;
             if (two < best) {
@@ -256,12 +263,15 @@
             }
         }
         p.main_qgroups = pick_qgroups(p.main_qblocks, dim, kn, p.tile_q);
-        const MainPassChoice choice = choose_main_pass(p, k, sample, sample_alt, sample_big, kn, narrow);
+        MainPassChoice choice = choose_main_pass(p, k, sample, sample_alt, sample_big, kn, narrow);
         sample = choice.sample;
+        if (skips_sample(p, k, sample)) choice = choose_main_pass(p, k, sample, sample, sample, kn, narrow, true);
         const int64_t R = choice.ranges;
         p.sample_tiles = (int)sample;
         p.sample_stride = std::max<int64_t>(1, p.full_tiles / sample);
         p.sample_ranges = best_sample_ranges(sample, p.qblocks, p.qgroups, p.grid);
+        p.skip_sampled = skips_sample(p, k, sample) ? 1 : 0;
+        p.main_tiles = p.skip_sampled ? p.tiles - sample : p.tiles;
         p.ranges = (int)R;
         p.item_a = choice.item_a;
         p.item_b = choice.item_b;
@@ -334,6 +344,7 @@
         if (rows >= 64) rows = rows / 64 * 64;
         p.dense_rows_per_chunk = rows;
     }
+    if (!p.fused) p.main_tiles = p.tiles;
     const SearchWs w = search_ws(p, n_rows, dim, n_q, k, nullptr);
     p.off_qnorm = (size_t)w.qnorm, p.off_thr = (size_t)w.thr, p.off_gmax = (size_t)w.gmax, p.off_cnt = (size_t)w.cnt, p.off_cand = (size_t)w.cand;
     p.off_flag = (size_t)w.flag_count, p.off_dense = (size_t)w.dense, p.off_retry = (size_t)w.Q2, p.off_top = (size_t)w.top, p.off_safe = (size_t)w.thr_safe;
@@ -671,6 +682,10 @@
 
 static int run_main_pass(const ccr_index *ix, const Plan &p, const SearchWs &w, const uint16_t *Q, int n_q, int k, hipStream_t s) {
     GemmArgs gm = filter_args(ix, p, w, Q, n_q, p.nq_pad, p.main_qblocks, p.main_qgroups, w.thr, w.cq, p.cand);
+    if (p.skip_sampled) {
+        gm.n_vt = p.main_tiles;
+        gm.skip = make_tile_skip(p.sample_tiles, p.sample_stride);
+    }
     const int nrc = NUM_XCD / gm.qgroups, qb_per = gm.qblocks / gm.qgroups, items = p.ranges / nrc * qb_per;
     const int bounds[4] = {0, p.item_a, p.item_b, items};
     int done = 0, updates = 0, prev_full = 0, prev_part = 0, prev_blocks = 0;
@@ -748,6 +763,7 @@
     st.main_launches = 1 + (p.item_a ? 1 : 0) + (p.item_b ? 1 : 0);
     st.opt_rank = p.opt_rank;
     st.main_tile_queries = p.narrow ? 0 : p.tile_q;
+    st.main_tiles_skipped = (int32_t)(p.tiles - p.main_tiles);
     st.n_candidates = (int64_t)ncand;
     return CCR_OK;
 }
@@ -958,7 +974,7 @@
     if (!p.fused) return search_dense(ix, w, Q_bf16, n_q, k, out_scores, out_ids, flags, s);
 
     CCR_HIP_CHECK(hipMemsetAsync(w.flag_count, 0, 64, s));
-    if ((int64_t)p.ranges > p.tiles) CCR_HIP_CHECK(hipMemsetAsync(w.cnt, 0, (size_t)p.ranges * p.nq_pad * p.sublists * 4, s));
+    if ((int64_t)p.ranges > p.main_tiles) CCR_HIP_CHECK(hipMemsetAsync(w.cnt, 0, (size_t)p.ranges * p.nq_pad * p.sublists * 4, s));
     int rc = launch_row_norms_bf16(Q_bf16, n_q, ix->dim, w.qnorm, nullptr, nullptr, s);
     if (rc != CCR_OK) return rc;
 
@@ -985,6 +1001,11 @@
                                w.cq, ix->tile_norm, ix->row_norm, ix->dmax_bits, Q_bf16, ix->D, ix->dim, ix->id_out, out_scores, out_ids,
                                w.flag_count, w.flag_list, w.stat_cand, nullptr, s);
     if (rc != CCR_OK) return rc;
+    if (p.skip_sampled) {
+        rc = launch_sample_merge(w.gmax, p.sample_tiles, p.sample_stride, n_q, p.nq_pad, k, ix->n_rows, w.cq, ix->tile_norm, Q_bf16, ix->D, ix->dim,
+                                 ix->id_out, out_scores, out_ids, w.flag_count, w.flag_list, s);
+        if (rc != CCR_OK) return rc;
+    }
     CCR_HIP_CHECK(hipEventRecord(ix->ev[EV_SELECT_END], s));
 
     ix->pending = {false, Q_bf16, n_q, k, out_scores, out_ids, (char *)workspace, s};
diff --git a/crowd-coachable-recommendations_amd/csrc/ccr_common.h b/crowd-coachable-recommendations_amd/csrc/ccr_common.h
--- a/crowd-coachable-recommendations_amd/csrc/ccr_common.h
+++ b/crowd-coachable-recommendations_amd/csrc/ccr_common.h
@@ -64,6 +64,25 @@
     return L.base[g] + (((long long)(r - r0) * nq_pad + q) * sp) * (long long)cap + s;
 }
 
+struct TileSkip {
+    uint32_t n;
+    uint32_t period;
+    uint64_t magic;
+};
+__host__ __device__ __forceinline__ TileSkip make_tile_skip(int64_t n, int64_t stride) {
+    TileSkip s = {0u, 1u, 0ull};
+    if (n > 0 && stride >= 2) {
+        s.n = (uint32_t)n;
+        s.period = (uint32_t)(stride - 1);
+        s.magic = (1ull << 40) / s.period + 1ull;
+    }
+    return s;
+}
+__host__ __device__ __forceinline__ int64_t unsampled_tile(const TileSkip &s, int64_t v) {
+    const uint64_t u = (uint64_t)v;
+    return u < (uint64_t)s.n * s.period ? (int64_t)(u + ((u * s.magic) >> 40) + 1u) : v + (int64_t)s.n;
+}
+
 struct Plan {
     int fused;
     int nq_pad;
@@ -76,6 +95,8 @@
     int sample_tiles;
     int64_t sample_stride;
     int sample_ranges;
+    int skip_sampled;
+    int64_t main_tiles;
     int ranges;
     int item_a;
     int item_b;
@@ -110,6 +131,7 @@
     int qblocks;
     int64_t n_vt;
     int64_t tile_stride;
+    TileSkip skip;
     int ranges;
     int qgroups;
     int item_begin, item_end;
@@ -124,6 +146,10 @@
     int64_t store_pitch;
 };
 
+
+__device__ __forceinline__ int64_t physical_tile(const GemmArgs &a, int64_t vt) {
+    return a.skip.n ? unsampled_tile(a.skip, vt) : vt * a.tile_stride;
+}
 
 __device__ __forceinline__ float bf16_bits_to_f32(uint16_t h) { return __uint_as_float(((uint32_t)h) << 16); }
 
diff --git a/crowd-coachable-recommendations_amd/csrc/ccr_fused.hip b/crowd-coachable-recommendations_amd/csrc/ccr_fused.hip
--- a/crowd-coachable-recommendations_amd/csrc/ccr_fused.hip
+++ b/crowd-coachable-recommendations_amd/csrc/ccr_fused.hip
@@ -1,5 +1,6 @@
 #include <stdlib.h>
 
+#include <algorithm>
 #include <mutex>
 #include <set>
 #include <type_traits>
@@ -296,7 +297,7 @@
         int iks = 0;
         const uint16_t *dsrc[2];
         auto tile_ptrs = [&]() {
-            const int64_t row0 = (r + it * a.ranges) * a.tile_stride * TILE_DOCS;
+            const int64_t row0 = physical_tile(a, r + it * a.ranges) * TILE_DOCS;
 #pragma unroll
             for (int i = 0; i < 2; ++i) {
                 int64_t drow = row0 + (i * 128 + srow);
@@ -331,7 +332,7 @@
         };
 
         auto epilogue = [&](int64_t vt, float nt) {
-            const int64_t row_base = vt * a.tile_stride * TILE_DOCS + wd * 128 + 4 * lh;
+            const int64_t row_base = physical_tile(a, vt) * TILE_DOCS + wd * 128 + 4 * lh;
             if constexpr (EPI == EPI_GMAX) {
                 S::gmax(acc, a, vt, q0, wd, wq, lane);
             } else if constexpr (EPI == EPI_FILTER) {
@@ -395,7 +396,7 @@
             if (++cks == KS2) {
                 cks = 0;
                 const int64_t vt_done = r + ct * a.ranges;
-                const float nt_done = EPI == EPI_FILTER ? load_uniform_f32(a.tile_norm + vt_done * a.tile_stride) : 0.f;
+                const float nt_done = EPI == EPI_FILTER ? load_uniform_f32(a.tile_norm + physical_tile(a, vt_done)) : 0.f;
                 if (g1) {
                     epilogue(vt_done, nt_done);
                 } else {
@@ -504,7 +505,7 @@
         const char *dtile = nullptr;
         int dlimit = 0;
         auto tile_base = [&]() __attribute__((always_inline)) {
-            const int64_t row0 = (r + it * a.ranges) * a.tile_stride * TILE_DOCS;
+            const int64_t row0 = physical_tile(a, r + it * a.ranges) * TILE_DOCS;
             dlimit = (a.n_rows - 1 - row0 < TILE_DOCS - 1) ? (int)(a.n_rows - 1 - row0) : TILE_DOCS - 1;
             dtile = reinterpret_cast<const char *>(a.D) + row0 * pitch;
         };
@@ -560,7 +561,7 @@
             const uint32_t row_lo = (uint32_t)(wd * 128 + 4 * lqo);
             const uint32_t tc_addr = lds_offset(s_tc) + (uint32_t)l15o * 8u;
             const uint32_t cnt_addr = lds_offset(s_cnt) + (uint32_t)(lqo * 16 + l15o) * 4u;
-            const int64_t tile_row0 = vt * a.tile_stride * TILE_DOCS;
+            const int64_t tile_row0 = physical_tile(a, vt) * TILE_DOCS;
             const uint32_t rows_left = a.n_rows - tile_row0 < TILE_DOCS ? (uint32_t)(a.n_rows - tile_row0) : (uint32_t)TILE_DOCS;
 #pragma unroll
             for (int qt = 0; qt < WIDE_QT; ++qt) {
@@ -662,7 +663,7 @@
             if (++cks == KS2) {
                 cks = 0;
                 const int64_t vt_done = r + ct * a.ranges;
-                const float nt_done = load_uniform_f32(a.tile_norm + vt_done * a.tile_stride);
+                const float nt_done = load_uniform_f32(a.tile_norm + physical_tile(a, vt_done));
                 if (g1) {
                     epilogue(vt_done, nt_done);
                 } else {
@@ -990,6 +991,83 @@
     if (tid == 0) {
         const float t1 = orderable_to_f32(kth);
         if (t1 > thr[q]) thr[q] = t1;
+    }
+}
+
+template <int THREADS>
+__device__ __forceinline__ void canonical_rescore_keys(unsigned long long *s_keys, int ncoll, int np2, const uint16_t *s_q,
+                                                       const uint16_t *__restrict__ D, int dim, char *stage, size_t stage_bytes) {
+    const int tid = threadIdx.x;
+    int SB = (size_t)ncoll * 144 <= stage_bytes ? 128 : ((size_t)ncoll * 80 <= stage_bytes ? 64 : 0);
+    constexpr int PRE = 8;
+    if (SB == 128 && ncoll * 8 > PRE * THREADS) SB = 64;
+    if (SB != 0 && ncoll <= 2 * THREADS && ncoll * (SB / 16) <= PRE * THREADS) {
+        const int stride = SB + 16;
+        const int lpr = SB / 16;
+        const int row_bytes = dim * 2;
+        const char *Dbytes = reinterpret_cast<const char *>(D);
+        const int col = (tid % lpr) * 16;
+#define CCR_PIECES(X) X(0) X(1) X(2) X(3) X(4) X(5) X(6) X(7)
+        const int acol = col < row_bytes ? col : 0;
+        const char *Dcol = Dbytes + acol;
+        const int npiece = ncoll * lpr;
+#define CCR_DECL(j)                                                                                              \
+    const int idx##j = tid + j * THREADS;                                                                        \
+    const char *src##j = Dcol + (int64_t)(uint32_t)s_keys[idx##j < npiece ? idx##j / lpr : 0] * row_bytes;      \
+    uint4 pre##j = *reinterpret_cast<const uint4 *>(src##j);
+        CCR_PIECES(CCR_DECL)
+#undef CCR_DECL
+        double acc[2] = {0.0, 0.0};
+        for (int k0 = 0; k0 < row_bytes; k0 += SB) {
+            __syncthreads();
+            const bool col_in = k0 + col < row_bytes;
+#define CCR_PUT(j) \
+    if (col_in && idx##j < npiece) *reinterpret_cast<uint4 *>(stage + (idx##j / lpr) * stride + col) = pre##j;
+            CCR_PIECES(CCR_PUT)
+#undef CCR_PUT
+            __syncthreads();
+            {
+                const int kn = (k0 + SB + col < row_bytes) ? k0 + SB : -acol;
+#define CCR_GET(j) pre##j = *reinterpret_cast<const uint4 *>(src##j + kn);
+                CCR_PIECES(CCR_GET)
+#undef CCR_GET
+            }
+#undef CCR_PIECES
+#pragma unroll
+            for (int j = 0; j < 2; ++j) {
+                const int i = tid + j * THREADS;
+                if (i < ncoll) {
+                    double a = acc[j];
+                    for (int c = 0; c < lpr && k0 + c * 16 < row_bytes; ++c) {
+                        const uint4 dv = *reinterpret_cast<const uint4 *>(stage + (size_t)i * stride + c * 16);
+                        const uint4 qv = *reinterpret_cast<const uint4 *>(reinterpret_cast<const char *>(s_q) + k0 + c * 16);
+                        const uint32_t dw[4] = {dv.x, dv.y, dv.z, dv.w};
+                        const uint32_t qw[4] = {qv.x, qv.y, qv.z, qv.w};
+#pragma unroll
+                        for (int e = 0; e < 4; ++e) {
+                            a = fma((double)__uint_as_float(qw[e] << 16), (double)__uint_as_float(dw[e] << 16), a);
+                            a = fma((double)__uint_as_float(qw[e] & 0xffff0000u), (double)__uint_as_float(dw[e] & 0xffff0000u), a);
+                        }
+                    }
+                    acc[j] = a;
+                }
+            }
+        }
+        __syncthreads();
+#pragma unroll
+        for (int j = 0; j < 2; ++j) {
+            const int i = tid + j * THREADS;
+            if (i < np2) s_keys[i] = i < ncoll ? make_key((float)acc[j], (uint32_t)s_keys[i]) : 0ull;
+        }
+    } else {
+        for (int i = tid; i < np2; i += blockDim.x) {
+            unsigned long long key = 0ull;
+            if (i < ncoll) {
+                const uint32_t row = (uint32_t)s_keys[i];
+                key = make_key(canonical_dot(s_q, D + (int64_t)row * dim, dim), row);
+            }
+            s_keys[i] = key;
+        }
     }
 }
 
@@ -1206,85 +1284,138 @@
     }
     const int ncoll = (int)s_ncoll;
     const int np2 = pow2_ceil(ncoll);
-    const size_t stage_bytes = (size_t)compact * 8;
-    int SB = (size_t)ncoll * 144 <= stage_bytes ? 128 : ((size_t)ncoll * 80 <= stage_bytes ? 64 : 0);
-    constexpr int PRE = 8;
-    if (SB == 128 && ncoll * 8 > PRE * THREADS) SB = 64;
-    if (SB != 0 && ncoll <= 2 * THREADS && ncoll * (SB / 16) <= PRE * THREADS) {
-        char *stage = reinterpret_cast<char *>(s_comp);
-        const int stride = SB + 16;
-        const int lpr = SB / 16;
-        const int row_bytes = dim * 2;
-        const char *Dbytes = reinterpret_cast<const char *>(D);
-        const int col = (tid % lpr) * 16;
-#define CCR_PIECES(X) X(0) X(1) X(2) X(3) X(4) X(5) X(6) X(7)
-        const int acol = col < row_bytes ? col : 0;
-        const char *Dcol = Dbytes + acol;
-        const int npiece = ncoll * lpr;
-#define CCR_DECL(j)                                                                                              \
-    const int idx##j = tid + j * THREADS;                                                                        \
-    const char *src##j = Dcol + (int64_t)(uint32_t)s_keys[idx##j < npiece ? idx##j / lpr : 0] * row_bytes;      \
-    uint4 pre##j = *reinterpret_cast<const uint4 *>(src##j);
-        CCR_PIECES(CCR_DECL)
-#undef CCR_DECL
-        double acc[2] = {0.0, 0.0};
-        for (int k0 = 0; k0 < row_bytes; k0 += SB) {
-            __syncthreads();
-            const bool col_in = k0 + col < row_bytes;
-#define CCR_PUT(j) \
-    if (col_in && idx##j < npiece) *reinterpret_cast<uint4 *>(stage + (idx##j / lpr) * stride + col) = pre##j;
-            CCR_PIECES(CCR_PUT)
-#undef CCR_PUT
-            __syncthreads();
-            {
-                const int kn = (k0 + SB + col < row_bytes) ? k0 + SB : -acol;
-#define CCR_GET(j) pre##j = *reinterpret_cast<const uint4 *>(src##j + kn);
-                CCR_PIECES(CCR_GET)
-#undef CCR_GET
-            }
-#undef CCR_PIECES
-#pragma unroll
-            for (int j = 0; j < 2; ++j) {
-                const int i = tid + j * THREADS;
-                if (i < ncoll) {
-                    double a = acc[j];
-                    for (int c = 0; c < lpr && k0 + c * 16 < row_bytes; ++c) {
-                        const uint4 dv = *reinterpret_cast<const uint4 *>(stage + (size_t)i * stride + c * 16);
-                        const uint4 qv = *reinterpret_cast<const uint4 *>(reinterpret_cast<const char *>(s_q) + k0 + c * 16);
-                        const uint32_t dw[4] = {dv.x, dv.y, dv.z, dv.w};
-                        const uint32_t qw[4] = {qv.x, qv.y, qv.z, qv.w};
-#pragma unroll
-                        for (int e = 0; e < 4; ++e) {
-                            a = fma((double)__uint_as_float(qw[e] << 16), (double)__uint_as_float(dw[e] << 16), a);
-                            a = fma((double)__uint_as_float(qw[e] & 0xffff0000u), (double)__uint_as_float(dw[e] & 0xffff0000u), a);
-                        }
-                    }
-                    acc[j] = a;
-                }
-            }
-        }
-        __syncthreads();
-#pragma unroll
-        for (int j = 0; j < 2; ++j) {
-            const int i = tid + j * THREADS;
-            if (i < np2) s_keys[i] = i < ncoll ? make_key((float)acc[j], (uint32_t)s_keys[i]) : 0ull;
-        }
-    } else {
-        for (int i = tid; i < np2; i += blockDim.x) {
-            unsigned long long key = 0ull;
-            if (i < ncoll) {
-                const uint32_t row = (uint32_t)s_keys[i];
-                key = make_key(canonical_dot(s_q, D + (int64_t)row * dim, dim), row);
-            }
-            s_keys[i] = key;
-        }
-    }
+    canonical_rescore_keys<THREADS>(s_keys, ncoll, np2, s_q, D, dim, reinterpret_cast<char *>(s_comp), (size_t)compact * 8);
     block_bitonic_sort_desc(s_keys, np2);
     const int64_t orow = out_rows ? (int64_t)out_rows[q] : (int64_t)q;
     for (int i = tid; i < k; i += blockDim.x) {
         const unsigned long long key = s_keys[i];
         out_scores[orow * k + i] = key_score(key);
         store_id(out_ids, orow * k + i, id_offset, key_idx(key));
+    }
+}
+
+constexpr int MERGE_THREADS = 256;
+constexpr int MERGE_QUERIES = 16;
+constexpr int MERGE_STAGE_BYTES = 16 * 1024;
+static int merge_row_cap(int k) { return std::min(8192, std::max(1024, 4 * pow2_ceil(k))); }
+
+__global__ __launch_bounds__(MERGE_THREADS) void sample_merge_kernel(const float *__restrict__ gmax, int sample_tiles, int64_t sample_stride,
+                                                                    int n_q, int nq_pad, int k, int row_cap, int64_t n_rows,
+                                                                    const float *__restrict__ cq, const float *__restrict__ tile_norm,
+                                                                    const uint16_t *__restrict__ Q, const uint16_t *__restrict__ D, int dim,
+                                                                    int64_t id_offset, float *__restrict__ out_scores,
+                                                                    int64_t *__restrict__ out_ids, uint32_t *__restrict__ flag_count,
+                                                                    uint32_t *__restrict__ flag_list) {
+    extern __shared__ __attribute__((aligned(16))) char sm[];
+    const int group_cap = row_cap / 16;
+    uint16_t *s_q = reinterpret_cast<uint16_t *>(sm);
+    unsigned long long *s_old = reinterpret_cast<unsigned long long *>(sm + (((size_t)dim * 2 + 15) & ~(size_t)15));
+    unsigned long long *s_new = s_old + k;
+    char *stage = reinterpret_cast<char *>(s_new + row_cap);
+    uint32_t *s_grp = reinterpret_cast<uint32_t *>(stage + MERGE_STAGE_BYTES);
+    __shared__ uint32_t s_ngroup[MERGE_QUERIES], s_nnew;
+    __shared__ int s_flagged[MERGE_QUERIES];
+    const int tid = threadIdx.x;
+    const int q0 = blockIdx.x * MERGE_QUERIES;
+    const uint32_t n_flag = flag_count[0];
+    if (tid < MERGE_QUERIES) {
+        s_ngroup[tid] = 0;
+        s_flagged[tid] = q0 + tid >= n_q;
+    }
+    __syncthreads();
+    for (uint32_t i = tid; i < n_flag; i += MERGE_THREADS) {
+        const uint32_t f = flag_list[i] & ~FLAG_DENSE;
+        if (f >= (uint32_t)q0 && f < (uint32_t)(q0 + MERGE_QUERIES)) s_flagged[f - q0] = 1;
+    }
+    __syncthreads();
+    {
+        const int ql = tid & (MERGE_QUERIES - 1), ph = tid / MERGE_QUERIES, q = q0 + ql;
+        if (!s_flagged[ql]) {
+            const float s_k = out_scores[(int64_t)q * k + k - 1];
+            const float cut = s_k - fabsf(s_k) * 1.1920929e-7f;
+            const float c = cq[q];
+            const int n_groups = sample_tiles * GROUPS_PER_TILE, step = MERGE_THREADS / MERGE_QUERIES;
+            for (int g0 = ph; g0 < n_groups; g0 += step * 8) {
+                float m[8], nt[8];
+#pragma unroll
+                for (int u = 0; u < 8; ++u) {
+                    const int g = g0 + u * step < n_groups ? g0 + u * step : g0;
+                    m[u] = gmax[(int64_t)g * nq_pad + q];
+                    nt[u] = tile_norm[(int64_t)(g / GROUPS_PER_TILE) * sample_stride];
+                }
+#pragma unroll
+                for (int u = 0; u < 8; ++u) {
+                    const int g = g0 + u * step;
+                    if (g < n_groups && !(fmaf(c, nt[u], m[u]) < cut) &&
+                        ((int64_t)(g / GROUPS_PER_TILE) * sample_stride + 1) * TILE_DOCS <= n_rows) {
+                        const uint32_t p = atomicAdd(&s_ngroup[ql], 1u);
+                        if (p < (uint32_t)group_cap) s_grp[ql * group_cap + p] = (uint32_t)g;
+                    }
+                }
+            }
+        }
+    }
+    __syncthreads();
+    for (int ql = 0; ql < MERGE_QUERIES; ++ql) {
+        const int ngroup = (int)s_ngroup[ql];
+        if (s_flagged[ql] || ngroup == 0) continue;
+        const int q = q0 + ql;
+        if (ngroup > group_cap) {
+            if (tid == 0) flag_list[n_flag + atomicAdd(&flag_count[1], 1u)] = (uint32_t)q;
+            continue;
+        }
+        __syncthreads();
+        if (tid == 0) s_nnew = 0;
+        for (int c = tid; c < dim / 8; c += MERGE_THREADS)
+            reinterpret_cast<uint4 *>(s_q)[c] = reinterpret_cast<const uint4 *>(Q + (int64_t)q * dim)[c];
+        const int ncoll = ngroup * 16, np2 = pow2_ceil(ncoll);
+        for (int i = tid; i < ncoll; i += MERGE_THREADS) {
+            const int g = (int)s_grp[ql * group_cap + (i >> 4)], gi = g % GROUPS_PER_TILE, x = i & 15;
+            const uint32_t first = (uint32_t)((int64_t)(g / GROUPS_PER_TILE) * sample_stride * TILE_DOCS) +
+                                   (uint32_t)((gi >> 3) * 128 + ((gi >> 1) & 3) * 32 + (gi & 1) * 4);
+            s_new[i] = (unsigned long long)(first + 8 * (x >> 2) + (x & 3));
+        }
+        const int64_t out0 = (int64_t)q * k;
+        auto old_row = [&](int i) -> uint32_t {
+            return id_offset == ID_LOCAL_U32 ? reinterpret_cast<const uint32_t *>(out_ids)[out0 + i] : (uint32_t)(out_ids[out0 + i] - id_offset);
+        };
+        for (int i = tid; i < k; i += MERGE_THREADS) s_old[i] = make_key(out_scores[out0 + i], old_row(i));
+        const unsigned long long last = make_key(out_scores[out0 + k - 1], old_row(k - 1));
+        __syncthreads();
+        canonical_rescore_keys<MERGE_THREADS>(s_new, ncoll, np2, s_q, D, dim, stage, MERGE_STAGE_BYTES);
+        __syncthreads();
+        for (int i = tid; i < np2; i += MERGE_THREADS)
+            if (s_new[i] <= last) s_new[i] = 0ull;
+        block_bitonic_sort_desc(s_new, np2);
+        for (int i = tid; i < np2; i += MERGE_THREADS)
+            if (s_new[i] != 0ull && (i + 1 == np2 || s_new[i + 1] == 0ull)) s_nnew = (uint32_t)(i + 1);
+        __syncthreads();
+        const int n_new = (int)s_nnew;
+        auto above = [](const unsigned long long *a, int n, unsigned long long key) {
+            int lo = 0, hi = n;
+            while (lo < hi) {
+                const int mid = (lo + hi) >> 1;
+                if (a[mid] > key)
+                    lo = mid + 1;
+                else
+                    hi = mid;
+            }
+            return lo;
+        };
+        auto put = [&](int pos, unsigned long long key) {
+            if (pos < k) {
+                out_scores[out0 + pos] = key_score(key);
+                store_id(out_ids, out0 + pos, id_offset, key_idx(key));
+            }
+        };
+        if (n_new > 0) {
+            for (int i = tid; i < k; i += MERGE_THREADS) put(i + above(s_new, n_new, s_old[i]), s_old[i]);
+            for (int j = tid; j < n_new; j += MERGE_THREADS) put(j + above(s_old, k, s_new[j]), s_new[j]);
+        }
+    }
+    if (tid == 0) {
+        __threadfence();
+        if (atomicAdd(&flag_count[4], 1u) == gridDim.x - 1) flag_count[0] = n_flag + atomicAdd(&flag_count[1], 0u);
     }
 }
 
@@ -1493,6 +1624,21 @@
     return (int)std::min<int64_t>(std::max<int64_t>(want, 2048), fit) / 256 * 256;
 }
 
+int launch_sample_merge(const float *gmax, int sample_tiles, int64_t sample_stride, int n_q, int nq_pad, int k, int64_t n_rows, const float *cq,
+                        const float *tile_norm, const uint16_t *Q, const uint16_t *D, int dim, int64_t id_offset, float *out_scores,
+                        int64_t *out_ids, uint32_t *flag_count, uint32_t *flag_list, hipStream_t s) {
+    const int row_cap = merge_row_cap(k);
+    const size_t lds = (((size_t)dim * 2 + 15) & ~(size_t)15) + ((size_t)k + row_cap) * 8 + MERGE_STAGE_BYTES + (size_t)MERGE_QUERIES * (row_cap / 16) * 4;
+    if (lds > 48 * 1024) {
+        const int rc = ensure_dynamic_lds(reinterpret_cast<const void *>(&sample_merge_kernel), SELECT_LDS_BUDGET);
+        if (rc != CCR_OK) return rc;
+    }
+    hipLaunchKernelGGL(sample_merge_kernel, dim3((n_q + MERGE_QUERIES - 1) / MERGE_QUERIES), dim3(MERGE_THREADS), lds, s, gmax, sample_tiles, sample_stride, n_q, nq_pad, k, row_cap, n_rows, cq,
+                       tile_norm, Q, D, dim, id_offset, out_scores, out_ids, flag_count, flag_list);
+    CCR_LAUNCH_CHECK();
+    return CCR_OK;
+}
+
 int launch_partition_flags(const uint32_t *flags, int begin, int n, uint32_t *retry_list, uint32_t *dense_list, uint32_t *counts,
                            hipStream_t s) {
     hipLaunchKernelGGL(partition_flags_kernel, dim3(1), dim3(256), 0, s, flags, begin, n, retry_list, dense_list, counts);
diff --git a/crowd-coachable-recommendations_amd/csrc/ccr_index.h b/crowd-coachable-recommendations_amd/csrc/ccr_index.h
--- a/crowd-coachable-recommendations_amd/csrc/ccr_index.h
+++ b/crowd-coachable-recommendations_amd/csrc/ccr_index.h
@@ -60,6 +60,9 @@
                           const uint32_t *dmax_bits, const uint16_t *Q, const uint16_t *D, int dim, int64_t id_offset, float *out_scores, int64_t *out_ids,
                           uint32_t *flag_count, uint32_t *flag_list, unsigned long long *stat_cand, const uint32_t *out_rows,
                           hipStream_t s);
+int launch_sample_merge(const float *gmax, int sample_tiles, int64_t sample_stride, int n_q, int nq_pad, int k, int64_t n_rows, const float *cq,
+                        const float *tile_norm, const uint16_t *Q, const uint16_t *D, int dim, int64_t id_offset, float *out_scores,
+                        int64_t *out_ids, uint32_t *flag_count, uint32_t *flag_list, hipStream_t s);
 int launch_partition_flags(const uint32_t *flags, int begin, int n, uint32_t *retry_list, uint32_t *dense_list, uint32_t *counts,
                            hipStream_t s);
 int launch_underfilled_to_retry(uint32_t *flags, int begin, int n, const float *thr_safe, float *thr, hipStream_t s);
diff --git a/include/ccr_retrieval.h b/include/ccr_retrieval.h
--- a/include/ccr_retrieval.h
+++ b/include/ccr_retrieval.h
@@ -47,7 +47,7 @@
     int32_t main_launches;
     int32_t opt_rank;
     int32_t main_tile_queries;
-    int32_t reserved0;
+    int32_t main_tiles_skipped;
 } ccr_search_stats;
 
 const char *ccr_last_error(void);
```

Result: no change. 256,100 (median of 6 runs) (+0.8%).
